# maxjaritz/mvpnet

Hardware: AMD Instinct MI355X
Metric: chunks/sec (8192 pts, 3x160x120 views) fwd+bwd (higher is better)
Workload: dtype f32; 1 GPU; configs[2]: MVPNet lifting (unproject + pixel k-NN + gather) + FeatureAggregation + PN2SSG full train step (fwd+loss+bwd+Adam), 2D CNN replaced by a resident 64-ch feature map; cfg=mvpnet_3d_unet_resnet34_pn2ssg.yaml, chunks_per_gpu=32, points=8192, views=3x160x120, feature_channels=64, k=3, parallelism=dp1 (one process per GPU, 1 grad all-reduce/step), launch=eager, cpu_affinity=32 logical cpus of 256 (0 .. 183)

## Files before the change

include/mvp_hip.h:

```cpp
#ifndef MVP_HIP_H_
#define MVP_HIP_H_

#include <stdint.h>

#ifdef __cplusplus
extern "C" {
#endif

typedef void* mvp_stream_t;

#define MVP_OK 0
#define MVP_EINVAL (-1)
#define MVP_EUNSUPPORTED (-2)
#define MVP_ENULL (-3)

const char* mvp_version(void);
const char* mvp_strerror(int code);

int mvp_set_fps_mode(int mode);

int mvp_fps_f32(const float* points, int64_t B, int64_t N, int64_t D, int64_t M, int64_t* index, mvp_stream_t stream);
int mvp_fps_f64(const double* points, int64_t B, int64_t N, int64_t D, int64_t M, int64_t* index, mvp_stream_t stream);
int mvp_fps_shape_f32(const float* points, int64_t B, int64_t N, int64_t D, int64_t M, int64_t* index, int shape, mvp_stream_t stream);
int mvp_fps_shape_f64(const double* points, int64_t B, int64_t N, int64_t D, int64_t M, int64_t* index, int shape, mvp_stream_t stream);
// ... 232 lines not shown
                                      const float* beta_i, const double* stat_i, float* dgamma_i, float* dbeta_i, int training, int mode,
                                      float drop_p, uint64_t drop_seed, const float* X, int64_t ldx, const float* act_mean,
                                      const float* act_invstd, const float* act_gamma, const float* act_beta, const float* W, int64_t ldw,
                                      int64_t R, int64_t C, int64_t Cp, float* dW, int64_t lddw, float* dZ, double* stat_prev, int* ticket,
                                      float* workspace, int64_t workspace_floats, int precision, int precision_backward, mvp_stream_t stream);
int mvp_mlp_layer_backward_wide_pooled_p_f32(const float* G, const float* Yi, const float* mean_i, const float* invstd_i, const float* gamma_i,
                                             const float* beta_i, const double* stat_i, float* dgamma_i, float* dbeta_i, int training, int mode,
                                             int64_t pool_k, float drop_p, uint64_t drop_seed, const float* X, int64_t ldx, const float* act_mean,
                                             const float* act_invstd, const float* act_gamma, const float* act_beta, const float* W, int64_t ldw,
                                             int64_t R, int64_t C, int64_t Cp, float* dW, int64_t lddw, float* dZ, double* stat_prev, int* ticket,
                                             float* workspace, int64_t workspace_floats, int precision, int precision_backward, mvp_stream_t stream);
int mvp_mlp_weight_grad_finish_p_f32(const float* dZ, const float* Y, const float* mean, const float* invstd, const float* gamma, const double* stat,
                                     int training, const float* X, int64_t R, int64_t Cout, int64_t Cin, int64_t ldx, float* dW, int64_t lddw,
                                     float* workspace, int64_t workspace_floats, int precision, int precision_backward, mvp_stream_t stream);
int mvp_mlp_weight_grad_finish_rel_p_f32(const float* dZ, const float* Y, const float* mean, const float* invstd, const float* gamma, const double* stat,
                                         int training, const float* X, int64_t R, int64_t Cout, int64_t Cin, int64_t ldx, const float* REL, float* dW,
                                         float* dWrel, int64_t lddw, int precision, int precision_backward, mvp_stream_t stream);
int mvp_mlp_weight_grad_finish_act_p_f32(const float* dZ, const float* Y, const float* mean, const float* invstd, const float* gamma, const double* stat,
                                         int training, const float* X, int64_t R, int64_t Cout, int64_t Cin, int64_t ldx, const float* act_mean,
                                         const float* act_invstd, const float* act_gamma, const float* act_beta, float* dW, int64_t lddw,
                                         float* workspace, int64_t workspace_floats, int precision, int precision_backward, mvp_stream_t stream);
int64_t mvp_mlp_input_grad_wide_workspace_bytes(int64_t C, int64_t Cp);
int mvp_mlp_input_grad_wide_p_f32(const float* G, const float* Yi, const float* mean_i, const float* invstd_i, const float* gamma_i,
                                  const double* stat_i, float* dgamma_i, float* dbeta_i, int training, const float* X, int64_t ldx,
                                  const float* act_mean, const float* act_invstd, const float* act_gamma, const float* act_beta, const float* W,
                                  int64_t ldw, int64_t R, int64_t C, int64_t Cp, float* dZ, double* stat_prev, void* workspace,
                                  int64_t workspace_bytes, int precision, int precision_backward, mvp_stream_t stream);
int mvp_mlp_weight_grad_f32(const float* dY, const float* X, int64_t R, int64_t Cout, int64_t Cin, int64_t ldx,
                            const float* act_mean, const float* act_invstd, const float* act_gamma, const float* act_beta,
                            float* dW, int64_t lddw, mvp_stream_t stream);
int64_t mvp_mlp_weight_grad_workspace_floats(void);
int mvp_mlp_weight_grad_ws_f32(const float* dY, const float* X, int64_t R, int64_t Cout, int64_t Cin, int64_t ldx,
                               const float* act_mean, const float* act_invstd, const float* act_gamma, const float* act_beta,
                               float* dW, int64_t lddw, float* workspace, int64_t workspace_floats, mvp_stream_t stream);

int mvp_sa_train_forward_f32(int stage, const float* zf, const float* xyz, const float* centre, const int64_t* index, const float* wxyz,
                             int64_t B, int64_t N, int64_t M, int64_t K, int64_t C1, const float* bn1_mean, const float* bn1_invstd,
                             const float* bn1_gamma, const float* bn1_beta, const float* W2, int64_t C2, const float* bn2_mean,
                             const float* bn2_invstd, const float* bn2_gamma, const float* bn2_beta, const float* W3, int64_t C3,
                             double* stat, float eps, float momentum, float* mean, float* invstd, float* running_mean,
                             float* running_var, int64_t* num_batches_tracked, float* ymax, float* ymin, uint8_t* amax, uint8_t* amin,
                             mvp_stream_t stream);
int mvp_sa_train_backward_f32(int layer, const float* zf, const float* xyz, const float* centre, const int64_t* index, const float* wxyz,
                              int64_t B, int64_t N, int64_t M, int64_t K, int64_t C1, const float* bn1_mean, const float* bn1_invstd,
                              const float* bn1_gamma, const float* bn1_beta, const float* W2, int64_t C2, const float* bn2_mean,
                              const float* bn2_invstd, const float* bn2_gamma, const float* bn2_beta, const float* W3, int64_t C3,
                              const float* mean_i, const float* invstd_i, const float* gamma_i, const double* stat_i, float* dgamma_i,
                              float* dbeta_i, int training, const float* G, const float* pool_dout, const float* pool_out,
                              const uint8_t* pool_arg, float* dW, int64_t lddw, float* dZ, double* stat_prev, float* tsum, mvp_stream_t stream);
int mvp_sa_train_backward1_f32(const float* dz1, const int32_t* offsets, const int32_t* slots, const float* zf, const float* dsum,
                               const float* wxyz, const float* tsum, const double* zsum, const double* gsum, int64_t B, int64_t N, int64_t M,
                               int64_t K, int64_t C1, const float* mean, const float* invstd, const float* gamma, const double* stat,
                               int training, float* dgamma, float* dbeta, float* gz, float* dWxyz, int64_t lddw, mvp_stream_t stream);
int mvp_sa_geom_sums_f32(const int32_t* offsets, const int32_t* slots, const float* xyz, const float* centre, int64_t B, int64_t N, int64_t M,
                         int64_t K, float* dsum, double* gsum, mvp_stream_t stream);
int mvp_sa_train_stats1_f32(const float* zf, const float* dsum, const float* wxyz, const double* gsum, int64_t B, int64_t N, int64_t M, int64_t K,
                            int64_t C1, double* stat, double* zsum, float eps, float momentum, float* mean, float* invstd, float* running_mean,
                            float* running_var, int64_t* num_batches_tracked, mvp_stream_t stream);
int mvp_sa_train_stats1_ws_f32(const float* zf, const float* dsum, const float* wxyz, const double* gsum, int64_t B, int64_t N, int64_t M, int64_t K,
                               int64_t C1, double* stat, double* zsum, float eps, float momentum, float* mean, float* invstd, float* running_mean,
                               float* running_var, int64_t* num_batches_tracked, double* scratch, int64_t scratch_doubles, mvp_stream_t stream);

int mvp_mlp_forward_p_f32(const float* X, int64_t R, int64_t Cin, int64_t ldx, const float* W, int64_t ldw, int64_t Cout, const
    float* act_mean, const float* act_invstd, const float* act_gamma, const float* act_beta, const float* bias, float* Y,
    double* stat, double* partial, int precision, int precision_backward, mvp_stream_t stream);
int mvp_mlp_forward_bn_p_f32(const float* X, int64_t R, int64_t Cin, int64_t ldx, const float* W, int64_t ldw, int64_t Cout,
    const float* act_mean, const float* act_invstd, const float* act_gamma, const float* act_beta, float* Y, double* stat,
    double* partial, float eps, float momentum, float* mean, float* invstd, float* running_mean, float* running_var, int64_t*
    num_batches_tracked, int precision, int precision_backward, mvp_stream_t stream);
int mvp_mlp_forward_rel_bn_p_f32(const float* X, int64_t R, int64_t Cin, int64_t ldx, const float* W, int64_t ldw, int64_t Cout,
    const float* rel, const float* wrel, float* Y, double* stat, double* partial, float eps, float momentum, float* mean, float*
    invstd, float* running_mean, float* running_var, int64_t* num_batches_tracked, int precision, int precision_backward,
    mvp_stream_t stream);
int mvp_mlp_forward_pool_p_f32(const float* X, int64_t R, int64_t Cin, int64_t ldx, const float* W, int64_t ldw, int64_t Cout,
    const float* act_mean, const float* act_invstd, const float* act_gamma, const float* act_beta, float* ymax, float* ymin,
    uint8_t* amax, uint8_t* amin, double* stat, double* partial, float eps, float momentum, float* mean, float* invstd, float*
    running_mean, float* running_var, int64_t* num_batches_tracked, int precision, int precision_backward, mvp_stream_t stream);
int mvp_mlp_input_grad_p_f32(const float* dY, int64_t R, int64_t Cout, const float* W, int64_t Cin, const float* y_prev, const
    float* mean, const float* invstd, const float* gamma, const float* beta, float* dZ, double* stat, double* partial, int
    precision, int precision_backward, mvp_stream_t stream);
int mvp_mlp_input_grad_dropout_p_f32(const float* dY, int64_t R, int64_t Cout, const float* W, int64_t Cin, const float* y_prev, const
    float* mean, const float* invstd, const float* gamma, const float* beta, float drop_p, uint64_t drop_seed, float* dZ, double* stat,
    double* partial, int precision, int precision_backward, mvp_stream_t stream);
int mvp_mlp_weight_grad_p_f32(const float* dY, const float* X, int64_t R, int64_t Cout, int64_t Cin, int64_t ldx, const float*
    act_mean, const float* act_invstd, const float* act_gamma, const float* act_beta, float* dW, int64_t lddw, int precision,
    int precision_backward, mvp_stream_t stream);
int mvp_mlp_weight_grad_ws_p_f32(const float* dY, const float* X, int64_t R, int64_t Cout, int64_t Cin, int64_t ldx, const
    float* act_mean, const float* act_invstd, const float* act_gamma, const float* act_beta, float* dW, int64_t lddw, float*
    workspace, int64_t workspace_floats, int precision, int precision_backward, mvp_stream_t stream);
int mvp_mlp_layer_backward_p_f32(const float* G, const float* Yi, const float* mean_i, const float* invstd_i, const float*
    gamma_i, const double* stat_i, float* dgamma_i, float* dbeta_i, int training, const float* X, int64_t ldx, const float*
    act_mean, const float* act_invstd, const float* act_gamma, const float* act_beta, const float* W, int64_t ldw, int64_t R,
    int64_t C, int64_t Cp, float* dW, int64_t lddw, float* dZ, double* stat_prev, double* partial, const float* pool_dout, const
    float* pool_out, const uint8_t* pool_arg, int precision, int precision_backward, mvp_stream_t stream);
int mvp_mlp_layer_backward_ws_p_f32(const float* G, const float* Yi, const float* mean_i, const float* invstd_i, const float*
    gamma_i, const double* stat_i, float* dgamma_i, float* dbeta_i, int training, const float* X, int64_t ldx, const float*
    act_mean, const float* act_invstd, const float* act_gamma, const float* act_beta, const float* W, int64_t ldw, int64_t R,
    int64_t C, int64_t Cp, float* dW, int64_t lddw, float* dZ, double* stat_prev, double* partial, const float* pool_dout, const
    float* pool_out, const uint8_t* pool_arg, float* workspace, int64_t workspace_floats, int precision, int precision_backward,
    mvp_stream_t stream);
int mvp_sa_fused_forward_p_f32(const float* zf, const float* xyz, const float* centre, const int64_t* index, const float* wxyz,
    int64_t B, int64_t N, int64_t M, int64_t K, int64_t C1, const float* bn1_mean, const float* bn1_invstd, const float*
    bn1_gamma, const float* bn1_beta, const float* W2, int64_t C2, const float* bn2_mean, const float* bn2_invstd, const float*
    bn2_gamma, const float* bn2_beta, const float* W3, int64_t C3, const float* bn3_mean, const float* bn3_invstd, const float*
    bn3_gamma, const float* bn3_beta, float* out, uint8_t* arg, int precision, int precision_backward, mvp_stream_t stream);

int mvp_sa_train_forward_p_f32(int stage, const float* zf, const float* xyz, const float* centre, const int64_t* index, const
    float* wxyz, int64_t B, int64_t N, int64_t M, int64_t K, int64_t C1, const float* bn1_mean, const float* bn1_invstd, const
    float* bn1_gamma, const float* bn1_beta, const float* W2, int64_t C2, const float* bn2_mean, const float* bn2_invstd, const
    float* bn2_gamma, const float* bn2_beta, const float* W3, int64_t C3, double* stat, float eps, float momentum, float* mean,
    float* invstd, float* running_mean, float* running_var, int64_t* num_batches_tracked, float* ymax, float* ymin, uint8_t*
    amax, uint8_t* amin, int precision, int precision_backward, mvp_stream_t stream);
int mvp_sa_train_backward_p_f32(int layer, const float* zf, const float* xyz, const float* centre, const int64_t* index, const
    float* wxyz, int64_t B, int64_t N, int64_t M, int64_t K, int64_t C1, const float* bn1_mean, const float* bn1_invstd, const
    float* bn1_gamma, const float* bn1_beta, const float* W2, int64_t C2, const float* bn2_mean, const float* bn2_invstd, const
    float* bn2_gamma, const float* bn2_beta, const float* W3, int64_t C3, const float* mean_i, const float* invstd_i, const
    float* gamma_i, const double* stat_i, float* dgamma_i, float* dbeta_i, int training, const float* G, const float* pool_dout,
    const float* pool_out, const uint8_t* pool_arg, float* dW, int64_t lddw, float* dZ, double* stat_prev, float* tsum, int precision, int
    precision_backward, mvp_stream_t stream);

int mvp_pn2_plan_f32(const float* xyz, int64_t B, int64_t N, int64_t levels, const int64_t* centroids, const float* radius,
                     const int64_t* neighbours, const int32_t* geom, int fps_shape, int flags, float knn_eps, void* const* buffers,
                     int64_t n_buffers, void* const* events, int* fps_status, mvp_stream_t stream);

int mvp_vote_accumulate_f32(const float* logit, int64_t ld_r, int64_t ld_c, const int64_t* chunk_ind, int64_t n,
                            int64_t C, float* sum, int32_t* count, mvp_stream_t stream);
int mvp_vote_gather_f32(const float* logit, int64_t ld_chunk, int64_t ld_r, int64_t ld_c, const int64_t* chunk_offsets, int64_t num_chunks,
                        const int32_t* point_offsets, const int32_t* point_slots, int64_t n_pts, int64_t C, float* sum, int32_t* count,
                        mvp_stream_t stream);
int mvp_vote_finish_f32(const float* sum, const int32_t* count, int64_t n_pts, int64_t C, float* mean, int64_t* label,
                        mvp_stream_t stream);

int mvp_seg_loss_f32(const float* logit, int64_t B, int64_t C, int64_t N, int64_t ld_b, int64_t ld_c, int64_t ld_n,
                     const int64_t* label, const float* weight, int64_t ignore_index, double* acc, float* loss, mvp_stream_t stream);
int mvp_seg_loss_backward_f32(const float* logit, int64_t B, int64_t C, int64_t N, int64_t ld_b, int64_t ld_c, int64_t ld_n,
                              const int64_t* label, const float* weight, int64_t ignore_index, const double* acc,
                              const float* grad_out, float* grad_logit, int64_t gld_b, int64_t gld_c, int64_t gld_n,
                              mvp_stream_t stream);
int mvp_seg_confusion_f32(const float* logit, int64_t B, int64_t C, int64_t N, int64_t ld_b, int64_t ld_c, int64_t ld_n,
                          const int64_t* label, int64_t ignore_index, int64_t* mat, mvp_stream_t stream);

#ifdef __cplusplus
}
#endif
#endif
```

mvpnet_amd/_lib.py:

```python
import ctypes
import os

import torch

_HERE = os.path.dirname(os.path.abspath(__file__))
LIB_PATH = os.environ.get('MVP_LIBRARY') or os.path.join(_HERE, 'libmvp_hip.so')
_lib = None
MLP_PRECISIONS = {'fp32': 0, 'bf16': 1, 'bf16x3': 3, 'bf16x6': 6}

_i64 = ctypes.c_int64
_ptr = ctypes.c_void_p
_f32 = ctypes.c_float

_SIGNATURES = {
    'mvp_fps_f32': [_ptr, _i64, _i64, _i64, _i64, _ptr, _ptr],
    'mvp_fps_f64': [_ptr, _i64, _i64, _i64, _i64, _ptr, _ptr],
    'mvp_fps_shape_f32': [_ptr, _i64, _i64, _i64, _i64, _ptr, ctypes.c_int, _ptr],
    'mvp_fps_shape_f64': [_ptr, _i64, _i64, _i64, _i64, _ptr, ctypes.c_int, _ptr],
    'mvp_fps_checked_f32': [_ptr, _i64, _i64, _i64, _i64, _ptr, ctypes.c_int, _ptr, _ptr],
    'mvp_fps_centroid_levels_f32': [_ptr, _ptr, _i64, _i64, _i64, _i64, _i64, _ptr, _ptr, _ptr],
    'mvp_ball_query_f32': [_ptr, _ptr, _i64, _i64, _i64, _f32, _i64, _ptr, _ptr],
    'mvp_ball_query_f64': [_ptr, _ptr, _i64, _i64, _i64, _f32, _i64, _ptr, _ptr],
    'mvp_ball_query_distance_f32': [_ptr, _ptr, _i64, _i64, _i64, _f32, _i64, _ptr, _ptr, _ptr],
    'mvp_ball_query_distance_f64': [_ptr, _ptr, _i64, _i64, _i64, _f32, _i64, _ptr, _ptr, _ptr],
# ... 25 lines not shown
    'mvp_interpolate_forward_bf16': [_ptr, _ptr, _ptr, _i64, _i64, _i64, _i64, _ptr, _ptr],
    'mvp_interpolate_backward_f32': [_ptr, _ptr, _ptr, _i64, _i64, _i64, _i64, _ptr, _ptr],
    'mvp_interpolate_backward_f64': [_ptr, _ptr, _ptr, _i64, _i64, _i64, _i64, _ptr, _ptr],
    'mvp_interpolate_backward_bf16': [_ptr, _ptr, _ptr, _i64, _i64, _i64, _i64, _ptr, _ptr],
    'mvp_unproject_f32': [_ptr, _ptr, _ptr, _ptr, _i64, _i64, _i64, _i64, _ptr, _ptr, _ptr],
    'mvp_unproject_u16': [_ptr, _ptr, _ptr, _ptr, _i64, _i64, _i64, _i64, _ptr, _ptr, _ptr],
    'mvp_pixel_knn_bruteforce_f32': [_ptr, _ptr, _ptr, _i64, _i64, _i64, _i64, _ptr, _ptr, _ptr],
    'mvp_pixel_knn_projective_f32': [_ptr, _ptr, _ptr, _ptr, _ptr, _i64, _i64, _i64, _i64, _i64, _i64, _ptr, _ptr, _ptr],
    'mvp_lift_gather_f32': [_ptr, _ptr, _ptr, _i64, _i64, _i64, _i64, _i64, _ptr, _ptr, _ptr],
    'mvp_lift_gather_backward_f32': [_ptr, _ptr, _i64, _i64, _i64, _i64, _i64, _ptr, _ptr],
    'mvp_lift_f32': [_ptr, ctypes.c_int, _ptr, _ptr, _ptr, _ptr, _ptr, _ptr, _i64, _i64, _i64, _i64, _i64, _i64, _i64, _ptr,
                     _ptr, _ptr, _ptr, _ptr, _ptr, _ptr],
    'mvp_lift_aug_f32': [_ptr, ctypes.c_int, _ptr, _ptr, _ptr, _ptr, _ptr, _ptr, _i64, _i64, _i64, _i64, _i64, _i64, _i64, _ptr,
                         _ptr, _ptr, _ptr, _ptr, _ptr, _ptr, _ptr, _ptr, _ptr],
    'mvp_rotate_rows_f32': [_ptr, _ptr, _i64, _i64, _ptr, _ptr],
    'mvp_copy_slices_f32': [_ptr, _i64, _ptr],
    'mvp_group_rows_f32': [_ptr, _ptr, _ptr, _ptr, _i64, _i64, _i64, _i64, _i64, _i64, _ptr, _ptr],
    'mvp_group_rows_backward_f32': [_ptr, _ptr, _i64, _i64, _i64, _i64, _i64, _i64, _ptr, _ptr],
    'mvp_group_lin_rows_f32': [_ptr, _ptr, _ptr, _ptr, _ptr, _i64, _i64, _i64, _i64, _i64, _ptr, _ptr, _ptr, _ptr, _ptr],
    'mvp_group_lin_rows_bn_f32': [_ptr, _ptr, _ptr, _ptr, _ptr, _i64, _i64, _i64, _i64, _i64, _ptr, _ptr, _ptr, _ptr, _f32, _f32, _ptr, _ptr, _ptr, _ptr, _ptr, _ptr],
    'mvp_colstats_f32': [_ptr, _i64, _i64, _ptr, _ptr, _ptr],
    'mvp_relation_rows_f32': [_ptr, _ptr, _ptr, _i64, _i64, _i64, _ptr, _ptr],
    'mvp_interp_rows_f32': [_ptr, _ptr, _ptr, _i64, _i64, _i64, _i64, _i64, _ptr, _ptr],
    'mvp_mlp_forward_bf16': [_ptr, _i64, _i64, _i64, _ptr, _i64, _i64, _ptr, _ptr, _ptr, ctypes.c_int, _ptr, _i64, _ptr],
    'mvp_adam_step_f32': [_ptr, _ptr, _ptr, _ptr, _ptr, _i64] + [ctypes.c_double] * 6 + [_ptr],
    'mvp_csr_build_i64': [_ptr, _i64, _i64, _i64, _ptr, _ptr, _ptr, _ptr],
    'mvp_csr_build_sorted_i64': [_ptr, _i64, _i64, _i64, _ptr, _ptr, _ptr, _ptr],
    'mvp_gather_rows_backward_csr_f32': [_ptr, _ptr, _ptr, _ptr, _i64, _i64, _i64, _i64, _i64, _i64, _ptr, _ptr],
    'mvp_gather_rows_backward_csr_finish_f32': [_ptr, _ptr, _ptr, _ptr, _ptr, _ptr, ctypes.c_int, _ptr, _ptr, _ptr, _i64, _i64, _i64, _i64, _i64, _i64, _ptr, _ptr],
    'mvp_interp_add_rows_f32': [_ptr, _ptr, _ptr, _ptr, _i64, _i64, _i64, _i64, _ptr, _ptr, _ptr, _ptr],
    'mvp_interp_add_rows_bn_f32': [_ptr, _ptr, _ptr, _ptr, _i64, _i64, _i64, _i64, _ptr, _ptr, _ptr, _f32, _f32, _ptr, _ptr, _ptr, _ptr, _ptr, _ptr],
    'mvp_interp_rows_backward_f32': [_ptr, _ptr, _ptr, _i64, _i64, _i64, _i64, _i64, _ptr, _ptr],
    'mvp_bn_rows_forward_f32': [_ptr, _ptr, _ptr, _i64, _i64, _i64, ctypes.c_int, _f32, _f32, ctypes.c_int, _ptr, _ptr, _ptr, _ptr,
                                _ptr, _ptr, _ptr, _ptr, _ptr],
    'mvp_bn_rows_backward_f32': [_ptr, _ptr, _ptr, _ptr, _ptr, _ptr, _ptr, _ptr, _i64, _i64, _i64, ctypes.c_int, ctypes.c_int, _ptr,
                                 _ptr, _ptr, _ptr, _ptr, _ptr],
    'mvp_bn_rows_forward_dropout_f32': [_ptr, _ptr, _ptr, _i64, _i64, ctypes.c_int, _f32, _f32, ctypes.c_int, _ptr, _ptr, _ptr, _ptr, _ptr, _ptr,
                                        _ptr, _f32, ctypes.c_uint64, _ptr],
    'mvp_bn_rows_backward_dropout_f32': [_ptr, _ptr, _ptr, _ptr, _ptr, _ptr, _i64, _i64, ctypes.c_int, ctypes.c_int, _ptr, _ptr, _ptr, _ptr,
                                         _ptr, _f32, ctypes.c_uint64, _ptr],
    'mvp_bn_rows_backward_finish_f32': [_ptr, _ptr, _ptr, _ptr, _ptr, _ptr, _i64, _i64, ctypes.c_int, _ptr, _ptr, _ptr, _ptr, _ptr],
    'mvp_bn_finalize_f32': [_ptr, _i64, _i64, _f32, _f32, _ptr, _ptr, _ptr, _ptr, _ptr, _ptr],
    'mvp_mlp_weight_grad_f32': [_ptr, _ptr, _i64, _i64, _i64, _i64, _ptr, _ptr, _ptr, _ptr, _ptr, _i64, _ptr],
    'mvp_mlp_weight_grad_ws_f32': [_ptr, _ptr, _i64, _i64, _i64, _i64, _ptr, _ptr, _ptr, _ptr, _ptr, _i64, _ptr, _i64, _ptr],
    'mvp_mlp_input_grad_f32': [_ptr, _i64, _i64, _ptr, _i64, _ptr, _ptr, _ptr, _ptr, _ptr, _ptr, _ptr, _ptr, _ptr],
    'mvp_mlp_input_grad_dropout_f32': [_ptr, _i64, _i64, _ptr, _i64, _ptr, _ptr, _ptr, _ptr, _ptr, _f32, ctypes.c_uint64, _ptr, _ptr, _ptr, _ptr],
    'mvp_mlp_layer_backward_f32': [_ptr, _ptr, _ptr, _ptr, _ptr, _ptr, _ptr, _ptr, ctypes.c_int, _ptr, _i64, _ptr, _ptr, _ptr, _ptr, _ptr, _i64,
                                   _i64, _i64, _i64, _ptr, _i64, _ptr, _ptr, _ptr, _ptr, _ptr, _ptr, _ptr],
    'mvp_mlp_layer_backward_ws_f32': [_ptr, _ptr, _ptr, _ptr, _ptr, _ptr, _ptr, _ptr, ctypes.c_int, _ptr, _i64, _ptr, _ptr, _ptr, _ptr, _ptr, _i64,
                                   _i64, _i64, _i64, _ptr, _i64, _ptr, _ptr, _ptr, _ptr, _ptr, _ptr, _ptr, _i64, _ptr],
    'mvp_mlp_forward_pool_f32': [_ptr, _i64, _i64, _i64, _ptr, _i64, _i64, _ptr, _ptr, _ptr, _ptr, _ptr, _ptr, _ptr, _ptr, _ptr, _ptr, _f32, _f32,
                                 _ptr, _ptr, _ptr, _ptr, _ptr, _ptr],
    'mvp_pool_finalize_f32': [_ptr, _ptr, _ptr, _ptr, _ptr, _ptr, _ptr, _ptr, _i64, _i64, ctypes.c_int, _ptr, _ptr, _ptr, _ptr],
    'mvp_pool_backward_stats_f32': [_ptr, _ptr, _ptr, _ptr, _ptr, _i64, _i64, ctypes.c_int, _ptr, _ptr, _ptr],
    'mvp_sa_fused_forward_f32': [_ptr, _ptr, _ptr, _ptr, _ptr, _i64, _i64, _i64, _i64, _i64, _ptr, _ptr, _ptr, _ptr, _ptr, _i64, _ptr, _ptr, _ptr,
                                 _ptr, _ptr, _i64, _ptr, _ptr, _ptr, _ptr, _ptr, _ptr, _ptr],
    'mvp_sa_train_forward_f32': [ctypes.c_int, _ptr, _ptr, _ptr, _ptr, _ptr, _i64, _i64, _i64, _i64, _i64, _ptr, _ptr, _ptr, _ptr, _ptr, _i64, _ptr, _ptr,
                                 _ptr, _ptr, _ptr, _i64, _ptr, _f32, _f32, _ptr, _ptr, _ptr, _ptr, _ptr, _ptr, _ptr, _ptr, _ptr, _ptr],
    'mvp_sa_train_backward_f32': [ctypes.c_int, _ptr, _ptr, _ptr, _ptr, _ptr, _i64, _i64, _i64, _i64, _i64, _ptr, _ptr, _ptr, _ptr, _ptr, _i64, _ptr, _ptr,
                                  _ptr, _ptr, _ptr, _i64, _ptr, _ptr, _ptr, _ptr, _ptr, _ptr, ctypes.c_int, _ptr, _ptr, _ptr, _ptr, _ptr, _i64, _ptr, _ptr,
                                  _ptr, _ptr],
    'mvp_sa_train_backward1_f32': [_ptr, _ptr, _ptr, _ptr, _ptr, _ptr, _ptr, _ptr, _ptr, _i64, _i64, _i64, _i64, _i64, _ptr, _ptr, _ptr, _ptr,
                                   ctypes.c_int, _ptr, _ptr, _ptr, _ptr, _i64, _ptr],
    'mvp_pn2_plan_f32': [_ptr, _i64, _i64, _i64, _ptr, _ptr, _ptr, _ptr, ctypes.c_int, ctypes.c_int, _f32, _ptr, _i64, _ptr, _ptr, _ptr],
    'mvp_sa_geom_sums_f32': [_ptr, _ptr, _ptr, _ptr, _i64, _i64, _i64, _i64, _ptr, _ptr, _ptr],
    'mvp_sa_train_stats1_f32': [_ptr, _ptr, _ptr, _ptr, _i64, _i64, _i64, _i64, _i64, _ptr, _ptr, _f32, _f32, _ptr, _ptr, _ptr, _ptr, _ptr, _ptr],
    'mvp_sa_train_stats1_ws_f32': [_ptr, _ptr, _ptr, _ptr, _i64, _i64, _i64, _i64, _i64, _ptr, _ptr, _f32, _f32, _ptr, _ptr, _ptr, _ptr, _ptr, _ptr, _i64, _ptr],
    'mvp_mlp_forward_bn_f32': [_ptr, _i64, _i64, _i64, _ptr, _i64, _i64, _ptr, _ptr, _ptr, _ptr, _ptr, _ptr, _ptr, _f32, _f32, _ptr, _ptr, _ptr,
                               _ptr, _ptr, _ptr],
    'mvp_mlp_forward_rel_bn_f32': [_ptr, _i64, _i64, _i64, _ptr, _i64, _i64, _ptr, _ptr, _ptr, _ptr, _ptr, _f32, _f32, _ptr, _ptr, _ptr, _ptr, _ptr, _ptr],
    'mvp_relation4_rows_f32': [_ptr, _ptr, _i64, _i64, _ptr, _ptr],
    'mvp_mlp_forward_f32': [_ptr, _i64, _i64, _i64, _ptr, _i64, _i64, _ptr, _ptr, _ptr, _ptr, _ptr, _ptr, _ptr, _ptr, _ptr],
    'mvp_vote_accumulate_f32': [_ptr, _i64, _i64, _ptr, _i64, _i64, _ptr, _ptr, _ptr],
    'mvp_vote_gather_f32': [_ptr, _i64, _i64, _i64, _ptr, _i64, _ptr, _ptr, _i64, _i64, _ptr, _ptr, _ptr],
    'mvp_vote_finish_f32': [_ptr, _ptr, _i64, _i64, _ptr, _ptr, _ptr],
    'mvp_seg_loss_f32': [_ptr, _i64, _i64, _i64, _i64, _i64, _i64, _ptr, _ptr, _i64, _ptr, _ptr, _ptr],
    'mvp_seg_loss_backward_f32': [_ptr, _i64, _i64, _i64, _i64, _i64, _i64, _ptr, _ptr, _i64, _ptr, _ptr, _ptr, _i64, _i64, _i64, _ptr],
    'mvp_seg_confusion_f32': [_ptr, _i64, _i64, _i64, _i64, _i64, _i64, _ptr, _i64, _ptr, _ptr],
}
for _n in ['mvp_mlp_forward_f32', 'mvp_mlp_forward_bn_f32', 'mvp_mlp_forward_rel_bn_f32', 'mvp_mlp_forward_pool_f32', 'mvp_mlp_input_grad_f32', 'mvp_mlp_input_grad_dropout_f32',
           'mvp_mlp_weight_grad_f32', 'mvp_mlp_weight_grad_ws_f32', 'mvp_mlp_layer_backward_f32', 'mvp_mlp_layer_backward_ws_f32',
           'mvp_sa_fused_forward_f32', 'mvp_sa_train_forward_f32', 'mvp_sa_train_backward_f32']:
    _SIGNATURES[_n[:-4] + '_p_f32'] = _SIGNATURES[_n][:-1] + [ctypes.c_int, ctypes.c_int, _ptr]
_SIGNATURES['mvp_mlp_layer_backward_wide_p_f32'] = [_ptr] * 9 + [ctypes.c_int, ctypes.c_int, _f32, ctypes.c_uint64, _ptr, _i64, _ptr, _ptr, _ptr, _ptr, _ptr, _i64,
                                                    _i64, _i64, _i64, _ptr, _i64, _ptr, _ptr, _ptr, _ptr, _i64, ctypes.c_int, ctypes.c_int, _ptr]
_SIGNATURES['mvp_mlp_layer_backward_wide_pooled_p_f32'] = [_ptr] * 9 + [ctypes.c_int, ctypes.c_int, _i64, _f32, ctypes.c_uint64, _ptr, _i64, _ptr, _ptr, _ptr, _ptr, _ptr, _i64,
                                                           _i64, _i64, _i64, _ptr, _i64, _ptr, _ptr, _ptr, _ptr, _i64, ctypes.c_int, ctypes.c_int, _ptr]
_SIGNATURES['mvp_mlp_weight_grad_finish_p_f32'] = [_ptr] * 6 + [ctypes.c_int, _ptr, _i64, _i64, _i64, _i64, _ptr, _i64, _ptr, _i64, ctypes.c_int, ctypes.c_int, _ptr]
_SIGNATURES['mvp_mlp_weight_grad_finish_rel_p_f32'] = [_ptr] * 6 + [ctypes.c_int, _ptr, _i64, _i64, _i64, _i64, _ptr, _ptr, _ptr, _i64, ctypes.c_int, ctypes.c_int, _ptr]
_SIGNATURES['mvp_mlp_weight_grad_finish_act_p_f32'] = [_ptr] * 6 + [ctypes.c_int, _ptr, _i64, _i64, _i64, _i64, _ptr, _ptr, _ptr, _ptr, _ptr, _i64, _ptr, _i64, ctypes.c_int,
                                                        ctypes.c_int, _ptr]
_SIGNATURES['mvp_mlp_input_grad_wide_p_f32'] = [_ptr] * 8 + [ctypes.c_int, _ptr, _i64, _ptr, _ptr, _ptr, _ptr, _ptr, _i64, _i64, _i64, _i64, _ptr, _ptr, _ptr, _i64,
                                                 ctypes.c_int, ctypes.c_int, _ptr]
EXPORTS = ['mvp_version', 'mvp_strerror', 'mvp_lift_workspace_bytes', 'mvp_ball_query_grid_workspace', 'mvp_knn3_grid_workspace', 'mvp_mlp_weight_grad_workspace_floats', 'mvp_mlp_input_grad_wide_workspace_bytes', 'mvp_group_lin_partial_count', 'mvp_colstats_partial_count',
           'mvp_set_mlp_precision', 'mvp_get_mlp_precision', 'mvp_mlp_layer_backward_partial_count', 'mvp_set_mlp_stream', 'mvp_set_mlp_precision_backward', 'mvp_get_mlp_precision_backward', 'mvp_mlp_precision_scope', 'mvp_set_fps_mode', 'mvp_fps_debug_spin_limit', 'mvp_fps_last_kernel'] + sorted(_SIGNATURES)


def lib():
    global _lib
    if _lib is None:
        if not os.path.exists(LIB_PATH):
            raise RuntimeError('libmvp_hip.so is not built: run `python -c "import __graft_entry__ as g; g.build()"` '
                               'or `make -C mvpnet_amd/csrc` ({})'.format(LIB_PATH))
        handle = ctypes.CDLL(LIB_PATH)
        handle.mvp_version.restype = ctypes.c_char_p
        handle.mvp_strerror.restype = ctypes.c_char_p
        handle.mvp_strerror.argtypes = [ctypes.c_int]
        handle.mvp_lift_workspace_bytes.restype = ctypes.c_int64
        handle.mvp_lift_workspace_bytes.argtypes = [_i64, _i64, _i64, _i64, _i64]
        handle.mvp_ball_query_grid_workspace.restype = ctypes.c_int64
        handle.mvp_ball_query_grid_workspace.argtypes = [_i64, _i64, _i64]
        handle.mvp_knn3_grid_workspace.restype = ctypes.c_int64
        handle.mvp_knn3_grid_workspace.argtypes = [_i64, _i64, _i64]
        handle.mvp_group_lin_partial_count.restype = ctypes.c_int64
        handle.mvp_group_lin_partial_count.argtypes = [_i64, _i64, _i64, _i64]
        handle.mvp_mlp_weight_grad_workspace_floats.restype = ctypes.c_int64
        handle.mvp_mlp_weight_grad_workspace_floats.argtypes = []
        handle.mvp_mlp_input_grad_wide_workspace_bytes.restype = ctypes.c_int64
        handle.mvp_mlp_input_grad_wide_workspace_bytes.argtypes = [ctypes.c_int64, ctypes.c_int64]
        handle.mvp_colstats_partial_count.restype = ctypes.c_int64
        handle.mvp_colstats_partial_count.argtypes = [_i64, _i64]
        handle.mvp_set_mlp_precision.restype = ctypes.c_int
        handle.mvp_set_mlp_precision.argtypes = [ctypes.c_int, ctypes.c_int]
        handle.mvp_get_mlp_precision.restype = ctypes.c_int
        handle.mvp_get_mlp_precision.argtypes = []
        handle.mvp_mlp_layer_backward_partial_count.restype = ctypes.c_int64
        handle.mvp_mlp_layer_backward_partial_count.argtypes = [_i64, _i64]
        for name, argtypes in _SIGNATURES.items():
            fn = getattr(handle, name)
            fn.argtypes = argtypes
            fn.restype = ctypes.c_int
        _lib = handle
        handle.mvp_set_mlp_stream.restype = ctypes.c_int
        handle.mvp_set_mlp_stream.argtypes = [ctypes.c_int]
        handle.mvp_set_fps_mode.restype = ctypes.c_int
        handle.mvp_set_fps_mode.argtypes = [ctypes.c_int]
        handle.mvp_fps_debug_spin_limit.restype = ctypes.c_int
        handle.mvp_fps_debug_spin_limit.argtypes = [ctypes.c_int]
        handle.mvp_fps_last_kernel.restype = ctypes.c_int
        handle.mvp_fps_last_kernel.argtypes = []
        if os.environ.get('MVP_MLP_STREAM') is not None:
            handle.mvp_set_mlp_stream(int(os.environ['MVP_MLP_STREAM']))
        handle.mvp_set_mlp_precision_backward.restype = ctypes.c_int
        handle.mvp_set_mlp_precision_backward.argtypes = [ctypes.c_int]
        handle.mvp_get_mlp_precision_backward.restype = ctypes.c_int
        handle.mvp_get_mlp_precision_backward.argtypes = []
        handle.mvp_mlp_precision_scope.restype = ctypes.c_int
        handle.mvp_mlp_precision_scope.argtypes = [ctypes.c_int, ctypes.c_int]
        if os.environ.get('MVP_MLP_PRECISION_BWD'):
            check(handle.mvp_set_mlp_precision_backward(MLP_PRECISIONS[os.environ['MVP_MLP_PRECISION_BWD']]), 'mvp_set_mlp_precision_backward')
        env = os.environ.get('MVP_MLP_PRECISION')
        if env:
            set_mlp_precision(env, int(os.environ.get('MVP_MLP_MIN_WIDTH', '0')))
    return _lib




def set_mlp_precision(name, min_width=0):
    if name not in MLP_PRECISIONS:
        raise ValueError('mlp precision must be one of {}'.format(sorted(MLP_PRECISIONS)))
    check(lib().mvp_set_mlp_precision(MLP_PRECISIONS[name], int(min_width)), 'mvp_set_mlp_precision')
    global _mlp_min_width
    _mlp_min_width = int(min_width)


_mlp_min_width = 0


def mlp_min_width():
    return _mlp_min_width


def set_mlp_precision_backward(name):
    if name not in ('bf16', 'bf16x3', 'bf16x6'):
        raise ValueError("backward mlp precision must be 'bf16', 'bf16x3' or 'bf16x6'")
    check(lib().mvp_set_mlp_precision_backward(MLP_PRECISIONS[name]), 'mvp_set_mlp_precision_backward')


class mlp_precision:

    def __init__(self, forward=None, backward=None):
        self.terms = -1 if forward is None else MLP_PRECISIONS[forward]
        self.bwd = -1 if backward is None else MLP_PRECISIONS[backward]
        if self.bwd == 0:
            raise ValueError("backward mlp precision must be 'bf16', 'bf16x3' or 'bf16x6'")

    def __enter__(self):
        old = lib().mvp_mlp_precision_scope(self.terms, self.bwd)
        if old < 0:
            check(old, 'mvp_mlp_precision_scope')
        self.old = (old // 16 - 1, old % 16 - 1)
        return self

    def __exit__(self, *exc):
        lib().mvp_mlp_precision_scope(*self.old)


def current_precision():
    h = lib()
    return (h.mvp_get_mlp_precision(), h.mvp_get_mlp_precision_backward())

# ... 30 lines not shown


def stream_of(t):
    return ctypes.c_void_p(torch.cuda.current_stream(t.device).cuda_stream)


def ptr(t):
    return None if t is None else t.data_ptr()


def ptr_at(t, element_offset):
    return t.data_ptr() + int(element_offset) * t.element_size()


def require_gpu(*tensors):
    for t in tensors:
        if t is None:
            continue
        if not t.is_cuda:
            raise RuntimeError('mvpnet_amd ops run on the GPU only (got a {} tensor); there is no CPU fallback'.format(t.device))
        if not t.is_contiguous():
            raise RuntimeError('tensor must be contiguous')


def suffix(t):
    if t.dtype == torch.float32:
        return 'f32'
    if t.dtype == torch.float64:
        return 'f64'
    raise RuntimeError('expected a float32 or float64 tensor, got {}'.format(t.dtype))


def value_suffix(t):
    return 'bf16' if t.dtype == torch.bfloat16 else suffix(t)


_FN = {}
_raw_stream = getattr(torch._C, '_cuda_getCurrentRawStream', None)
_raw_device = getattr(torch._C, '_cuda_getDevice', None)


def _fn(name):
    f = _FN.get(name)
    if f is None:
        f = _FN[name] = getattr(_lib if _lib is not None else lib(), name)
    return f


DW_WORKSPACE = os.environ.get('MVP_DETERMINISTIC', '0') == '1'


def set_deterministic(flag):
    global DW_WORKSPACE
    old, DW_WORKSPACE = DW_WORKSPACE, bool(flag)
    return old


_DW_WS = {}
_DW_WS_NAMES = {'mvp_mlp_weight_grad_f32': 'mvp_mlp_weight_grad_ws_f32', 'mvp_mlp_layer_backward_f32': 'mvp_mlp_layer_backward_ws_f32'}


def dw_workspace(index, stream_handle):
    ws = _DW_WS.get((index, stream_handle))
    if ws is None:
        ws = _DW_WS[(index, stream_handle)] = torch.empty(lib().mvp_mlp_weight_grad_workspace_floats(), dtype=torch.float32,
                                                          device=torch.device('cuda', index))
    return ws


def current_dw_workspace(device):
    if not DW_WORKSPACE:
        return None, 0
    index = device.index
    handle = _raw_stream(index) if (_raw_stream is not None and index == _raw_device()) else torch.cuda.current_stream(device).cuda_stream
    ws = dw_workspace(index, handle)
    return ws.data_ptr(), ws.numel()


def _with_dw_workspace(index, stream_handle, args):
    ws = dw_workspace(index, stream_handle)
    return args + (ws.data_ptr(), ws.numel())


def call_on(stream, name, *args, prec=None):
    if DW_WORKSPACE and name in _DW_WS_NAMES:
        name, args = _DW_WS_NAMES[name], _with_dw_workspace(stream.device.index, stream.cuda_stream, args)
    if prec is not None:
        name, args = name[:-4] + '_p_f32', args + prec
    code = _fn(name)(*args, stream.cuda_stream)
    if code != 0:
        check(code, name)


def call(name, tensor_for_device, *args, prec=None):
    index = tensor_for_device.device.index
    if DW_WORKSPACE and name in _DW_WS_NAMES:
        handle = _raw_stream(index) if _raw_stream is not None else torch.cuda.current_stream(tensor_for_device.device).cuda_stream
        name, args = _DW_WS_NAMES[name], _with_dw_workspace(index, handle, args)
    if prec is not None:
        name, args = name[:-4] + '_p_f32', args + prec
    if _raw_stream is not None and index == _raw_device():
        code = _fn(name)(*args, _raw_stream(index))
    elif index == torch.cuda.current_device():
        code = _fn(name)(*args, torch.cuda.current_stream(tensor_for_device.device).cuda_stream)
    else:
        with torch.cuda.device(tensor_for_device.device):
            code = _fn(name)(*args, stream_of(tensor_for_device))
    if code != 0:
        check(code, name)
```

mvpnet_amd/csrc/mlp.hip:

```cpp
#include "common.h"
#include "stats_reduce.h"
#include "mlp_common.h"
#include "dropout.h"
#include <algorithm>

int mvp_mlp_stream_forward(const float* X, int64_t R, int Cin, int ldx, const float* W, int ldw, int Cout, const float* act_mean,
                           const float* act_invstd, const float* act_gamma, const float* act_beta, const float* bias, float* Y,
                           double* stat, double* partial, int ns, float bn_eps, float bn_momentum, float* bn_mean, float* bn_invstd,
                           float* bn_running_mean, float* bn_running_var, int64_t* bn_num_batches, float* ymax, float* ymin,
                           uint8_t* amax, uint8_t* amin, hipStream_t s);

int g_mlp_terms = 6;
int g_mlp_terms_bwd = 3;
int g_mlp_min_width = 0;
thread_local int tl_mlp_terms = -1;
thread_local int tl_mlp_terms_bwd = -1;
int g_mlp_stream = 1;

namespace {


constexpr int kMT = 256;
constexpr int kBM = 128;


struct EpiBwd {
  const float* y;
  const float* mean;
  const float* invstd;
  const float* gamma;
  const float* beta;
  const float* rel;
  const float* wrel;
  Dropout drop;
};

#ifndef MVP_MFMA_PRIO
#define MVP_MFMA_PRIO 2
#endif
#ifndef MVP_DW_PRIO
#define MVP_DW_PRIO 2
#endif
constexpr int kMaxActCin = 512;

#ifndef MVP_MLP_WAVES128
#define MVP_MLP_WAVES128 3
#endif
template <int BN, int BK, bool WT, bool VEC, int ACT, int NS>
__global__ __launch_bounds__(kMT, (BN == 128 && VEC && WT && NS == 0) ? MVP_MLP_WAVES128 : (NS != 0 && BN == 128) ? 2 : 1) void mlp_fwd_kernel(const float* __restrict__ X, int64_t R, int Cin, int ldx,
                                                      const float* __restrict__ W, int ldw, int Cout,
                                                      InAct act, const float* __restrict__ bias, EpiBwd epi,
                                                      float* __restrict__ Y , double* __restrict__ stat,
                                                      double* __restrict__ partial) {
  static_assert(NS == 0 || (VEC && BK == 32), "split-bf16 needs the vector path and 32-wide slabs");
  constexpr int kLdB = BK + 4;
  constexpr int NT = BK / 8;
  constexpr int kColB = 80;
  constexpr int kPieceB = BN * kColB;
  constexpr int kBufB = NS == 0 ? BN * kLdB * 4 : NS * kPieceB;
  __shared__ __attribute__((aligned(16))) unsigned char BsRaw[2 * kBufB];
  float* const Bs0 = reinterpret_cast<float*>(BsRaw);
  __shared__ __attribute__((aligned(16))) float Ps[4][kMaxActCin];
  constexpr int kLdS = 36;
  constexpr int kSsFloats = 4 * 32 * kLdS;
  constexpr bool kAliasS = sizeof(float) * kSsFloats + sizeof(double) * 2 * 4 * BN <= (size_t)2 * kBufB;
  __shared__ __attribute__((aligned(16))) float Ss_own[kAliasS ? 4 : kSsFloats];
  float (*Ss)[32 * kLdS] = reinterpret_cast<float (*)[32 * kLdS]>(kAliasS ? Bs0 : &Ss_own[0]);
  static_assert(sizeof(double) * 2 * 4 * BN <= (size_t)2 * kBufB, "sred must fit in Bs");
  double (*sred)[4][BN] = reinterpret_cast<double (*)[4][BN]>(Bs0 + (kAliasS ? kSsFloats : 0));
  constexpr int NB = BN / 32;
  const int tid = threadIdx.x, lane = tid & 63, wave = tid >> 6;
  const int64_t row0 = (int64_t)blockIdx.x * kBM;
  const int col0 = blockIdx.y * BN;
  const int li = lane & 31, lh = lane >> 5;

  f32x16 acc[NB];
#pragma unroll
  for (int j = 0; j < NB; ++j)
#pragma unroll
    for (int i = 0; i < 16; ++i) acc[j][i] = 0.f;

  constexpr bool has_act = ACT != 0;
  constexpr bool act_lds = ACT == 1;
  if constexpr (act_lds) {
    for (int k = tid; k < min(kMaxActCin, (Cin + BK - 1) / BK * BK); k += kMT) {
      const int kc = min(k, Cin - 1);
      Ps[0][k] = act.mean[kc];
      Ps[1][k] = act.invstd[kc];
      Ps[2][k] = act.gamma[kc];
      Ps[3][k] = act.beta[kc];
    }
  }

  const int64_t arow = row0 + wave * 32 + li;
  const bool arow_ok = arow < R;
  const float* xrow = X + (size_t)(arow_ok ? arow : 0) * ldx;
  float4 an[NT];
  auto load_a = [&](int k0) {
#pragma unroll
    for (int t = 0; t < NT; ++t) {
      const int k = k0 + 8 * t + 4 * lh;
      if constexpr (VEC) {
        an[t] = *reinterpret_cast<const float4*>(xrow + min(k, Cin - 4));
      } else {
        an[t].x = xrow[min(k + 0, Cin - 1)];
        an[t].y = xrow[min(k + 1, Cin - 1)];
        an[t].z = xrow[min(k + 2, Cin - 1)];
        an[t].w = xrow[min(k + 3, Cin - 1)];
      }
    }
  };
  float ac[NT][4];
  auto activate = [&](int k0) {
#pragma unroll
    for (int t = 0; t < NT; ++t) {
      const int k = k0 + 8 * t + 4 * lh;
      float v[4] = {an[t].x, an[t].y, an[t].z, an[t].w};
      if constexpr (has_act) {
        float pm[4], pi[4], pg[4], pb[4];
        if constexpr (act_lds) {
          const float4 m4 = *reinterpret_cast<const float4*>(&Ps[0][k]), i4 = *reinterpret_cast<const float4*>(&Ps[1][k]);
          const float4 g4 = *reinterpret_cast<const float4*>(&Ps[2][k]), b4 = *reinterpret_cast<const float4*>(&Ps[3][k]);
          pm[0] = m4.x; pm[1] = m4.y; pm[2] = m4.z; pm[3] = m4.w;
          pi[0] = i4.x; pi[1] = i4.y; pi[2] = i4.z; pi[3] = i4.w;
          pg[0] = g4.x; pg[1] = g4.y; pg[2] = g4.z; pg[3] = g4.w;
          pb[0] = b4.x; pb[1] = b4.y; pb[2] = b4.z; pb[3] = b4.w;
        } else {
#pragma unroll
          for (int e = 0; e < 4; ++e) {
            const int kc = min(k + e, Cin - 1);
            pm[e] = act.mean[kc];
            pi[e] = act.invstd[kc];
            pg[e] = act.gamma[kc];
            pb[e] = act.beta[kc];
          }
        }
#pragma unroll
        for (int e = 0; e < 4; ++e) {
          const float a = ((v[e] - pm[e]) * pi[e]) * pg[e] + pb[e];
          v[e] = a > 0.f ? a : 0.f;
        }
      }
#pragma unroll
      for (int e = 0; e < 4; ++e) ac[t][e] = v[e];
    }
  };

  constexpr int LPC = BK / 4;
  constexpr int CPP = kMT / LPC;
  constexpr int NV = BN / CPP;
  constexpr int KH = BK / 32;
  float4 bn[WT ? NB * KH : NV];
  auto load_b = [&](int k0) {
    if constexpr (WT && NS != 0) {
      const int c = tid & 31, kq = (tid >> 5) * 4;
#pragma unroll
      for (int u = 0; u < NB; ++u) {
        const int co = min(col0 + u * 32 + c, Cout - 1);
        bn[u].x = W[(size_t)min(k0 + kq + 0, Cin - 1) * ldw + co];
        bn[u].y = W[(size_t)min(k0 + kq + 1, Cin - 1) * ldw + co];
        bn[u].z = W[(size_t)min(k0 + kq + 2, Cin - 1) * ldw + co];
        bn[u].w = W[(size_t)min(k0 + kq + 3, Cin - 1) * ldw + co];
      }
    } else if constexpr (!WT) {
      const int c = tid / LPC, k = k0 + (tid % LPC) * 4;
#pragma unroll
      for (int u = 0; u < NV; ++u) {
        const float* src = W + (size_t)min(col0 + u * CPP + c, Cout - 1) * ldw;
        if constexpr (VEC) {
          bn[u] = *reinterpret_cast<const float4*>(src + min(k, Cin - 4));
        } else {
          bn[u].x = src[min(k + 0, Cin - 1)];
          bn[u].y = src[min(k + 1, Cin - 1)];
          bn[u].z = src[min(k + 2, Cin - 1)];
          bn[u].w = src[min(k + 3, Cin - 1)];
        }
      }
    } else {
#pragma unroll
      for (int g = 0; g < KH; ++g) {
        const float* src = W + (size_t)min(k0 + 32 * g + (tid & 31), Cin - 1) * ldw;
#pragma unroll
        for (int p = 0; p < NB; ++p) {
          const int co = col0 + p * 32 + (tid >> 5) * 4;
          if constexpr (VEC) {
            bn[g * NB + p] = *reinterpret_cast<const float4*>(src + min(co, Cout - 4));
          } else {
            bn[g * NB + p].x = src[min(co + 0, Cout - 1)];
            bn[g * NB + p].y = src[min(co + 1, Cout - 1)];
            bn[g * NB + p].z = src[min(co + 2, Cout - 1)];
            bn[g * NB + p].w = src[min(co + 3, Cout - 1)];
          }
        }
      }
    }
  };
  auto store_b = [&](int buf, int k0) {
    if constexpr (NS != 0) {
      const int c = WT ? (tid & 31) : (tid / LPC), kq = WT ? (tid >> 5) * 4 : (tid % LPC) * 4;
      const int t = kq >> 3, unit = 2 * (t >> 1) + ((kq >> 2) & 1);
      unsigned char* base = BsRaw + (size_t)buf * kBufB + unit * 16 + (t & 1) * 8;
      const int k = k0 + kq;
      constexpr int PASSES = WT ? NB : NV;
#pragma unroll
      for (int u = 0; u < PASSES; ++u) {
        const int cl = u * 32 + c;
        const bool cok = col0 + cl < Cout;
        float4 v = bn[u];
        v.x = (cok && k + 0 < Cin) ? v.x : 0.f;
        v.y = (cok && k + 1 < Cin) ? v.y : 0.f;
        v.z = (cok && k + 2 < Cin) ? v.z : 0.f;
        v.w = (cok && k + 3 < Cin) ? v.w : 0.f;
        unsigned lo[NS], hi[NS];
        split_pair<NS>(v.x, v.y, lo);
        split_pair<NS>(v.z, v.w, hi);
#pragma unroll
        for (int pc = 0; pc < NS; ++pc)
          *reinterpret_cast<uint2*>(base + (size_t)pc * kPieceB + (size_t)cl * kColB) = make_uint2(lo[pc], hi[pc]);
      }
      return;
    }
    float* dst = Bs0 + (size_t)buf * (kBufB / 4);
    if constexpr (!WT) {
      const int c = tid / LPC, kq = (tid % LPC) * 4, k = k0 + kq;
#pragma unroll
      for (int u = 0; u < NV; ++u) {
        const bool cok = col0 + u * CPP + c < Cout;
        float4 v = bn[u];
        v.x = (cok && k + 0 < Cin) ? v.x : 0.f;
        v.y = (cok && k + 1 < Cin) ? v.y : 0.f;
        v.z = (cok && k + 2 < Cin) ? v.z : 0.f;
        v.w = (cok && k + 3 < Cin) ? v.w : 0.f;
        *reinterpret_cast<float4*>(dst + (u * CPP + c) * kLdB + kq) = v;
      }
    } else {
#pragma unroll
      for (int g = 0; g < KH; ++g) {
        const int kl = 32 * g + (tid & 31);
        const bool kok = k0 + kl < Cin;
#pragma unroll
        for (int p = 0; p < NB; ++p) {
          const int c = p * 32 + (tid >> 5) * 4;
          const int co = col0 + c;
          dst[(c + 0) * kLdB + kl] = (kok && co + 0 < Cout) ? bn[g * NB + p].x : 0.f;
          dst[(c + 1) * kLdB + kl] = (kok && co + 1 < Cout) ? bn[g * NB + p].y : 0.f;
          dst[(c + 2) * kLdB + kl] = (kok && co + 2 < Cout) ? bn[g * NB + p].z : 0.f;
          dst[(c + 3) * kLdB + kl] = (kok && co + 3 < Cout) ? bn[g * NB + p].w : 0.f;
        }
      }
    }
  };

  u32x4 af[NS == 0 ? 1 : 2][NS == 0 ? 1 : NS];
  auto split_a = [&]() {
    if constexpr (NS != 0) {
#pragma unroll
      for (int sI = 0; sI < 2; ++sI) {
        unsigned q0[NS], q1[NS], q2[NS], q3[NS];
        split_pair<NS>(ac[2 * sI][0], ac[2 * sI][1], q0);
        split_pair<NS>(ac[2 * sI][2], ac[2 * sI][3], q1);
        split_pair<NS>(ac[2 * sI + 1][0], ac[2 * sI + 1][1], q2);
        split_pair<NS>(ac[2 * sI + 1][2], ac[2 * sI + 1][3], q3);
#pragma unroll
        for (int pc = 0; pc < NS; ++pc) af[sI][pc] = u32x4{q0[pc], q1[pc], q2[pc], q3[pc]};
      }
    }
  };
  f32x16 acc1;
#pragma unroll
  for (int i = 0; i < 16; ++i) acc1[i] = 0.f;

  load_a(0);
  load_b(0);
  __syncthreads();
  store_b(0, 0);
  activate(0);
  split_a();
  __syncthreads();
  int buf = 0;
  for (int k0 = 0; k0 < Cin; k0 += BK) {
    const bool more = k0 + BK < Cin;
    if (more) {
      load_a(k0 + BK);
      load_b(k0 + BK);
    }
    __builtin_amdgcn_sched_barrier(0);
    __builtin_amdgcn_s_setprio(MVP_MFMA_PRIO);
    if constexpr (NS == 0) {
      const float* bp = Bs0 + (size_t)buf * (kBufB / 4) + li * kLdB + 4 * lh;
#pragma unroll
      for (int t = 0; t < NT; ++t) {
        float4 bf[NB];
#pragma unroll
        for (int j = 0; j < NB; ++j) bf[j] = *reinterpret_cast<const float4*>(bp + j * 32 * kLdB + 8 * t);
#pragma unroll
        for (int j = 0; j < NB; ++j) acc[j] = __builtin_amdgcn_mfma_f32_32x32x2f32(ac[t][0], bf[j].x, acc[j], 0, 0, 0);
#pragma unroll
        for (int j = 0; j < NB; ++j) acc[j] = __builtin_amdgcn_mfma_f32_32x32x2f32(ac[t][1], bf[j].y, acc[j], 0, 0, 0);
#pragma unroll
        for (int j = 0; j < NB; ++j) acc[j] = __builtin_amdgcn_mfma_f32_32x32x2f32(ac[t][2], bf[j].z, acc[j], 0, 0, 0);
#pragma unroll
        for (int j = 0; j < NB; ++j) acc[j] = __builtin_amdgcn_mfma_f32_32x32x2f32(ac[t][3], bf[j].w, acc[j], 0, 0, 0);
      }
    } else {
      using SP = SplitPairs<NS == 0 ? 2 : NS>;
      const unsigned char* bp = BsRaw + (size_t)buf * kBufB + (size_t)li * kColB + lh * 16;
      constexpr int JG = NB >= 2 ? 2 : 1;
#pragma unroll
      for (int sI = 0; sI < 2; ++sI) {
#pragma unroll
        for (int j0 = 0; j0 < NB; j0 += JG) {
          u32x4 bfr[JG][NS == 0 ? 1 : NS];
#pragma unroll
          for (int jj = 0; jj < JG; ++jj)
#pragma unroll
            for (int pc = 0; pc < NS; ++pc)
              bfr[jj][pc] = *reinterpret_cast<const u32x4*>(bp + (size_t)pc * kPieceB + (size_t)(j0 + jj) * 32 * kColB + sI * 32);
#pragma unroll
          for (int q = 0; q < SP::N; ++q)
#pragma unroll
            for (int jj = 0; jj < JG; ++jj) {
              const bf16x8 a8 = __builtin_bit_cast(bf16x8, af[sI][SP::A[q]]);
              const bf16x8 b8 = __builtin_bit_cast(bf16x8, bfr[jj][SP::B[q]]);
              if (NB == 1 && sI == 1)
                acc1 = __builtin_amdgcn_mfma_f32_32x32x16_bf16(a8, b8, acc1, 0, 0, 0);
              else
                acc[j0 + jj] = __builtin_amdgcn_mfma_f32_32x32x16_bf16(a8, b8, acc[j0 + jj], 0, 0, 0);
            }
        }
      }
    }
    __builtin_amdgcn_s_setprio(0);
    __builtin_amdgcn_sched_barrier(0);
    if (more) {
      store_b(buf ^ 1, k0 + BK);
      activate(k0 + BK);
      split_a();
    }
    __syncthreads();
    buf ^= 1;
  }
  if constexpr (NS != 0 && NB == 1) {
#pragma unroll
    for (int i = 0; i < 16; ++i) acc[0][i] += acc1[i];
  }

  const int cl = lane & 31, rh = (lane >> 5) * 4;
  const bool has_rel = VEC && !WT && epi.rel != nullptr;
  if constexpr (VEC && !WT) {
    if (has_rel) {
      if (lane < 32) {
        const int64_t r = row0 + wave * 32 + lane;
        f32x4 v = {0.f, 0.f, 0.f, 0.f};
        if (r < R) v = *reinterpret_cast<const f32x4*>(epi.rel + (size_t)r * 4);
        *reinterpret_cast<f32x4*>(Ss[wave] + lane * kLdS + 32) = v;
      }
      __builtin_amdgcn_wave_barrier();
    }
  }
  f32x4 ypv[VEC ? NB : 1][4];
  if constexpr (VEC) {
    if (epi.y) {
#pragma unroll
      for (int j = 0; j < NB; ++j)
#pragma unroll
        for (int pp = 0; pp < 4; ++pp) {
          const int row = pp * 8 + (lane >> 3), c4 = (lane & 7) * 4;
// ... 20 lines not shown
    if (has_rel && co < Cout) wr = *reinterpret_cast<const f32x4*>(epi.wrel + (size_t)co * 4);
    float yst[16];
    if constexpr (VEC) {
      if (epi.y) {
        float* st = Ss[wave];
#pragma unroll
        for (int pp = 0; pp < 4; ++pp) {
          const int row = pp * 8 + (lane >> 3), c4 = (lane & 7) * 4;
          *reinterpret_cast<f32x4*>(st + row * kLdS + c4) = ypv[j][pp];
        }
        __builtin_amdgcn_wave_barrier();
      }
    }
#pragma unroll
    for (int i = 0; i < 16; ++i) {
      const int m = wave * 32 + (i & 3) + 8 * (i >> 2) + rh;
      const int64_t r = row0 + m;
      yst[i] = 0.f;
      if (r < R && co < Cout) {
        float y = acc[j][i] + bv;
        if constexpr (VEC && !WT) {
          if (has_rel) {
            const f32x4 rv = *reinterpret_cast<const f32x4*>(Ss[wave] + ((i & 3) + 8 * (i >> 2) + rh) * kLdS + 32);
            y += (rv[0] * wr[0] + rv[1] * wr[1]) + (rv[2] * wr[2] + rv[3] * wr[3]);
          }
        }
        if (epi.y) {
          const float yp = VEC ? Ss[wave][((i & 3) + 8 * (i >> 2) + rh) * kLdS + cl] : epi.y[(size_t)r * Cout + co];
          const float xh = (yp - em) * ei;
          if (epi.drop.thresh) y *= epi.drop.factor((unsigned)((size_t)r * Cout + co));
          y = (xh * eg + eb > 0.f) ? y : 0.f;
          s += y;
          q += y * xh;
        } else {
          s += y;
          q += y * y;
        }
        if constexpr (!VEC) __builtin_nontemporal_store(y, Y + (size_t)r * Cout + co);
        yst[i] = y;
      }
    }
    if constexpr (VEC) {
      if (epi.y) __builtin_amdgcn_wave_barrier();
      float* st = Ss[wave];
#pragma unroll
      for (int i = 0; i < 16; ++i) st[((i & 3) + 8 * (i >> 2) + rh) * kLdS + cl] = yst[i];
      __builtin_amdgcn_wave_barrier();
#pragma unroll
      for (int pp = 0; pp < 4; ++pp) {
        const int row = pp * 8 + (lane >> 3), c4 = (lane & 7) * 4;
        const f32x4 v = *reinterpret_cast<const f32x4*>(st + row * kLdS + c4);
        const int64_t r = row0 + wave * 32 + row;
        const int cc = col0 + j * 32 + c4;
        if (r < R && cc < Cout)
          __builtin_nontemporal_store(v, reinterpret_cast<f32x4*>(Y + (size_t)r * Cout + cc));
      }
      __builtin_amdgcn_wave_barrier();
    }
    if (stat) {
      s += __shfl_xor(s, 32, kWave);
      q += __shfl_xor(q, 32, kWave);
      if (lane < 32) {
        sred[0][wave][j * 32 + cl] = (double)s;
        sred[1][wave][j * 32 + cl] = (double)q;
      }
    }
  }
  if (stat) {
    __syncthreads();
    for (int c = tid; c < BN; c += kMT) {
      const int co = col0 + c;
      if (co < Cout) {
        const double s0 = sred[0][0][c] + sred[0][1][c] + sred[0][2][c] + sred[0][3][c];
        const double s1 = sred[1][0][c] + sred[1][1][c] + sred[1][2][c] + sred[1][3][c];
        if (partial) {
          partial[((size_t)blockIdx.x * 2 + 0) * Cout + co] = s0;
          partial[((size_t)blockIdx.x * 2 + 1) * Cout + co] = s1;
        } else {
          atomicAdd(stat + co, s0);
          atomicAdd(stat + Cout + co, s1);
        }
      }
    }
  }
}

template <int TM, int TN, bool VEC, bool FIN = false>
__global__ __launch_bounds__(kMT) void mlp_dw_kernel(const float* __restrict__ dY, const float* __restrict__ X, int64_t R,
                                                     int Cout, int Cin, int ldx, InAct act, int64_t rows_per_block,
                                                     float* __restrict__ dW, int lddw, float* __restrict__ ws, DyFinish fin = DyFinish{}) {
  static_assert(!FIN || VEC, "the finish on load takes whole quadruples");
  constexpr int NBLK = (TM / 32) * (TN / 32);
  constexpr int RS = 4 / NBLK;
  constexpr int BR = 32 * RS;
  __shared__ __attribute__((aligned(16))) float Ds[2][BR * TM];
  __shared__ __attribute__((aligned(16))) float As[2][BR * TN];
  const int tid = threadIdx.x, lane = tid & 63, wave = tid >> 6;
  const int co0 = blockIdx.x * TM, ci0 = blockIdx.y * TN;
  const int64_t r_begin = (int64_t)blockIdx.z * rows_per_block;
  const int64_t r_end = min(R, r_begin + rows_per_block);
  const int blk = wave % NBLK, rs = wave / NBLK;
  const int wco = (blk / (TN / 32)) * 32, wci = (blk % (TN / 32)) * 32;
  f32x16 acc;
#pragma unroll
  for (int i = 0; i < 16; ++i) acc[i] = 0.f;

  constexpr int LD = TM / 4, RD = kMT / LD, PD = BR / RD;
  constexpr int LA = TN / 4, RA = kMT / LA, PA = BR / RA;
  const int dq = (tid % LD) * 4, dr = tid / LD;
  const int aq = (tid % LA) * 4, ar = tid / LA;
  float pm[4], pi[4], pg[4], pb[4];
  const bool has_act = act.mean != nullptr;
  if (has_act) {
#pragma unroll
    for (int i = 0; i < 4; ++i) {
      const int k = min(ci0 + aq + i, Cin - 1);
      pm[i] = act.mean[k];
      pi[i] = act.invstd[k];
      pg[i] = act.gamma[k];
      pb[i] = act.beta[k];
    }
  }
  float4 dn[PD], an[PA];
  float4 yn[FIN ? PD : 1];
  float fmu[4], fis[4], fsc[4], fdb[4], fdg[4];
  if constexpr (FIN) {
#pragma unroll
    for (int i = 0; i < 4; ++i) {
      const int k = min(co0 + dq, Cout - 4) + i;
      fmu[i] = fin.mean[k];
      fis[i] = fin.invstd[k];
      fsc[i] = fin.gamma[k] * fis[i];
      fdb[i] = (float)fin.stat[k] * fin.inv_rows;
      fdg[i] = (float)fin.stat[Cout + k] * fin.inv_rows;
    }
  }
  auto load = [&](int64_t r0) {
#pragma unroll
    for (int p = 0; p < PD; ++p) {
      const float* src = dY + (size_t)min(r0 + dr + p * RD, R - 1) * Cout;
      const int c = co0 + dq;
      if constexpr (FIN) yn[p] = *reinterpret_cast<const float4*>(fin.Y + (size_t)min(r0 + dr + p * RD, R - 1) * Cout + min(c, Cout - 4));
      if constexpr (VEC) {
        dn[p] = *reinterpret_cast<const float4*>(src + min(c, Cout - 4));
      } else {
        dn[p].x = src[min(c + 0, Cout - 1)];
        dn[p].y = src[min(c + 1, Cout - 1)];
        dn[p].z = src[min(c + 2, Cout - 1)];
        dn[p].w = src[min(c + 3, Cout - 1)];
      }
    }
#pragma unroll
    for (int p = 0; p < PA; ++p) {
      const float* src = X + (size_t)min(r0 + ar + p * RA, R - 1) * ldx;
      const int c = ci0 + aq;
      if constexpr (VEC) {
        an[p] = *reinterpret_cast<const float4*>(src + min(c, Cin - 4));
      } else {
        an[p].x = src[min(c + 0, Cin - 1)];
        an[p].y = src[min(c + 1, Cin - 1)];
        an[p].z = src[min(c + 2, Cin - 1)];
        an[p].w = src[min(c + 3, Cin - 1)];
      }
    }
  };
  auto store = [&](int buf, int64_t r0) {
// ... 243 lines not shown
                                                           accr[a], 0, 0, 0);
    }
    __builtin_amdgcn_s_setprio(0);
    __builtin_amdgcn_sched_barrier(0);
  }
  constexpr int NBLK = TMB * TNB;
  auto publish = [&](int slot) {
#pragma unroll
    for (int a = 0; a < TMB; ++a)
#pragma unroll
      for (int b = 0; b < TNB; ++b)
#pragma unroll
        for (int i = 0; i < 16; ++i) red[slot][((a * TNB + b) * 16 + i) * 64 + lane] = acc[a][b][i];
    if constexpr (REL) {
#pragma unroll
      for (int a = 0; a < TMB; ++a)
#pragma unroll
        for (int i = 0; i < 16; ++i) red[slot][((TMB * TNB + a) * 16 + i) * 64 + lane] = accr[a][i];
    }
  };
  auto absorb = [&](int slot) {
#pragma unroll
    for (int a = 0; a < TMB; ++a)
#pragma unroll
      for (int b = 0; b < TNB; ++b)
#pragma unroll
        for (int i = 0; i < 16; ++i) acc[a][b][i] += red[slot][((a * TNB + b) * 16 + i) * 64 + lane];
    if constexpr (REL) {
#pragma unroll
      for (int a = 0; a < TMB; ++a)
#pragma unroll
        for (int i = 0; i < 16; ++i) accr[a][i] += red[slot][((TMB * TNB + a) * 16 + i) * 64 + lane];
    }
  };
  static_assert(NBLK <= 4, "tile");
  static_assert(!REL || sizeof(red) <= 64 * 1024, "LDS");
  if (wave >= 2) publish(wave - 2);
  __syncthreads();
  if (wave < 2) absorb(wave);
  __syncthreads();
  if (wave == 1) publish(0);
  __syncthreads();
  if (wave == 0) {
    absorb(0);
    if (ws) {
      float* t = ws + (((size_t)blockIdx.z * gridDim.x + blockIdx.x) * gridDim.y + blockIdx.y) * (size_t)(NBLK * 1024);
#pragma unroll
      for (int a = 0; a < TMB; ++a)
#pragma unroll
        for (int b = 0; b < TNB; ++b)
#pragma unroll
          for (int i = 0; i < 16; ++i) __builtin_nontemporal_store(acc[a][b][i], t + ((a * TNB + b) * 16 + i) * 64 + lane);
      return;
    }
#pragma unroll
    for (int a = 0; a < TMB; ++a)
#pragma unroll
      for (int b = 0; b < TNB; ++b) {
        const int ci = ci0 + 32 * b + c;
#pragma unroll
        for (int i = 0; i < 16; ++i) {
          const int co = co0 + 32 * a + (i & 3) + 8 * (i >> 2) + 4 * g;
#ifdef MVP_EXP_DW_STORE
          if (co < Cout && ci < Cin) *(dW + (size_t)co * lddw + ci) = acc[a][b][i];
#else
          if (co < Cout && ci < Cin) atomicAdd(dW + (size_t)co * lddw + ci, acc[a][b][i]);
#endif
        }
      }
    if constexpr (REL) {
#pragma unroll
      for (int a = 0; a < TMB; ++a)
#pragma unroll
        for (int i = 0; i < 16; ++i) {
          const int co = co0 + 32 * a + (i & 3) + 8 * (i >> 2) + 4 * g;
          if (co < Cout && c < 4) atomicAdd(dW2 + (size_t)co * lddw + c, accr[a][i]);
        }
    }
  }
}

template <bool WT>
void launch_mlp(const float* X, int64_t R, int K, int ldx, const float* W, int ldw, int N, InAct act, const float* bias, EpiBwd epi,
                float* Y, double* stat, double* partial, hipStream_t s) {
  const unsigned gx = (unsigned)cdiv(R, kBM);
  const bool vec = ldx % 4 == 0 && ldw % 4 == 0 && K % 4 == 0 && N % 4 == 0 && ((uintptr_t)X) % 16 == 0 && ((uintptr_t)W) % 16 == 0 &&
                   K >= 4 && N >= 4;
#define MVP_MLP_LAUNCH(BN, VEC, NS_)                                                                                              \
                                  \
  do {                                                                                                                             \
    if (WT || act.mean == nullptr)                                                                                                 \
      hipLaunchKernelGGL((mlp_fwd_kernel<BN, 32, WT, VEC, 0, NS_>), dim3(gx, (unsigned)cdiv(N, BN)), dim3(kMT), 0, s, X, R, K, ldx, W, ldw, N, \
                         act, bias, epi, Y, stat, partial);                                                                        \
    else if (K <= kMaxActCin)                                                                                                      \
      hipLaunchKernelGGL((mlp_fwd_kernel<BN, 32, WT, VEC, WT ? 0 : 1, NS_>), dim3(gx, (unsigned)cdiv(N, BN)), dim3(kMT), 0, s, X, R, K, ldx, W, \
                         ldw, N, act, bias, epi, Y, stat, partial);                                                                \
    else                                                                                                                           \
      hipLaunchKernelGGL((mlp_fwd_kernel<BN, 32, WT, VEC, WT ? 0 : 2, NS_>), dim3(gx, (unsigned)cdiv(N, BN)), dim3(kMT), 0, s, X, R, K, ldx, W, \
                         ldw, N, act, bias, epi, Y, stat, partial);                                                                \
  } while (0)
  int bn = N <= 32 ? 32 : N <= 64 ? 64 : 128;
  while (bn > 32 && (int64_t)gx * cdiv(N, bn) < 256) bn >>= 1;
  const int fwd_pieces = mlp_fwd_pieces();
  const int ns = (vec && std::max(K, N) >= g_mlp_min_width) ? (WT ? mlp_bwd_pieces() : fwd_pieces) : 0;
#define MVP_MLP_BY_NS(BN)                                                                                                          \
  do {                                                                                                                             \
    if (!vec) MVP_MLP_LAUNCH(BN, false, 0);                                                                                        \
    else if (ns == 1) MVP_MLP_LAUNCH(BN, true, 1);                                                                                 \
    else if (ns == 2) MVP_MLP_LAUNCH(BN, true, 2);                                                                                 \
    else if (ns == 3) MVP_MLP_LAUNCH(BN, true, 3);                                                                                 \
    else MVP_MLP_LAUNCH(BN, true, 0);                                                                                              \
  } while (0)
  if (bn == 32) MVP_MLP_BY_NS(32);
  else if (bn == 64) MVP_MLP_BY_NS(64);
  else MVP_MLP_BY_NS(128);
#undef MVP_MLP_BY_NS
#undef MVP_MLP_LAUNCH
}

}

namespace {
int mlp_forward_impl(const float* X, int64_t R, int64_t Cin, int64_t ldx, const float* W, int64_t ldw, int64_t Cout, const float* act_mean,
                     const float* act_invstd, const float* act_gamma, const float* act_beta, const float* bias, float* Y, double* stat,
                     double* partial, float bn_eps, float bn_momentum, float* bn_mean, float* bn_invstd, float* bn_running_mean,
                     float* bn_running_var, int64_t* bn_num_batches, hipStream_t s, const float* rel = nullptr, const float* wrel = nullptr) {
  InAct act{act_mean, act_invstd, act_gamma, act_beta};
  const unsigned gx = (unsigned)cdiv(R, kBM);
  const BnFinalize fin{R, bn_eps, bn_momentum, bn_mean, bn_invstd, bn_running_mean, bn_running_var, bn_num_batches};
  if (g_mlp_stream && !rel && std::max(Cin, Cout) >= g_mlp_min_width) {
    const int rc = mvp_mlp_stream_forward(X, R, (int)Cin, (int)ldx, W, (int)ldw, (int)Cout, act_mean, act_invstd, act_gamma, act_beta, bias, Y,
                                          stat, partial, mlp_fwd_pieces(), bn_eps, bn_momentum, bn_mean,
                                          bn_invstd, bn_running_mean, bn_running_var, bn_num_batches, nullptr, nullptr, nullptr, nullptr, s);
    if (rc != MVP_EUNSUPPORTED) return rc;
  }
  launch_mlp<false>(X, R, (int)Cin, (int)ldx, W, (int)ldw, (int)Cout, act, bias, EpiBwd{nullptr, nullptr, nullptr, nullptr, nullptr, rel, wrel}, Y, stat,
                    stat ? partial : nullptr, s);
  if (stat && bn_mean)
    launch_stats_reduce_finalize(partial, partial ? (int64_t)gx : 0, (int)(2 * Cout), stat, fin, s);
  else if (stat && partial)
    launch_stats_reduce(partial, (int64_t)gx, (int)(2 * Cout), stat, s);
  return mvp_launch_status();
}
}

MVP_API int mvp_mlp_forward_f32(const float* X, int64_t R, int64_t Cin, int64_t ldx, const float* W, int64_t ldw,
                                int64_t Cout, const float* act_mean, const float* act_invstd, const float* act_gamma,
                                const float* act_beta, const float* bias, float* Y, double* stat, double* partial,
                                mvp_stream_t stream) {
  MVP_NONNULL(X);
  MVP_NONNULL(W);
  MVP_NONNULL(Y);
  MVP_REQUIRE(R >= 0 && Cin > 0 && Cout > 0 && ldx >= Cin && ldw >= Cin && Cin < (1 << 20) && Cout < (1 << 20));
  if (act_mean) {
    MVP_NONNULL(act_invstd);
    MVP_NONNULL(act_gamma);
    MVP_NONNULL(act_beta);
  }
  if (R == 0) return MVP_OK;
  return mlp_forward_impl(X, R, Cin, ldx, W, ldw, Cout, act_mean, act_invstd, act_gamma, act_beta, bias, Y, stat, partial, 0.f, 0.f, nullptr,
                          nullptr, nullptr, nullptr, nullptr, static_cast<hipStream_t>(stream));
}

MVP_API int mvp_mlp_forward_bn_f32(const float* X, int64_t R, int64_t Cin, int64_t ldx, const float* W, int64_t ldw, int64_t Cout,
                                   const float* act_mean, const float* act_invstd, const float* act_gamma, const float* act_beta, float* Y,
                                   double* stat, double* partial, float eps, float momentum, float* mean, float* invstd,
                                   float* running_mean, float* running_var, int64_t* num_batches_tracked, mvp_stream_t stream) {
  MVP_NONNULL(X);
  MVP_NONNULL(W);
  MVP_NONNULL(Y);
  MVP_NONNULL(stat);
  MVP_NONNULL(mean);
  MVP_NONNULL(invstd);
  MVP_REQUIRE(R > 0 && Cin > 0 && Cout > 0 && ldx >= Cin && ldw >= Cin && Cin < (1 << 20) && Cout < (1 << 20));
  if (act_mean) {
    MVP_NONNULL(act_invstd);
    MVP_NONNULL(act_gamma);
    MVP_NONNULL(act_beta);
  }
  if (running_mean) MVP_NONNULL(running_var);
  return mlp_forward_impl(X, R, Cin, ldx, W, ldw, Cout, act_mean, act_invstd, act_gamma, act_beta, nullptr, Y, stat, partial, eps, momentum,
                          mean, invstd, running_mean, running_var, num_batches_tracked, static_cast<hipStream_t>(stream));
}

MVP_API int mvp_mlp_forward_rel_bn_f32(const float* X, int64_t R, int64_t Cin, int64_t ldx, const float* W, int64_t ldw, int64_t Cout,
                                       const float* rel, const float* wrel, float* Y, double* stat, double* partial, float eps, float momentum,
                                       float* mean, float* invstd, float* running_mean, float* running_var, int64_t* num_batches_tracked,
                                       mvp_stream_t stream) {
  MVP_NONNULL(X);
  MVP_NONNULL(W);
  MVP_NONNULL(Y);
  MVP_NONNULL(rel);
  MVP_NONNULL(wrel);
  MVP_REQUIRE(R > 0 && Cin >= 4 && Cout >= 4 && ldx >= Cin && ldw >= Cin && Cin < (1 << 20) && Cout < (1 << 20));
  MVP_REQUIRE(ldx % 4 == 0 && ldw % 4 == 0 && Cin % 4 == 0 && Cout % 4 == 0 && ((uintptr_t)X) % 16 == 0 && ((uintptr_t)W) % 16 == 0 &&
              ((uintptr_t)rel) % 16 == 0 && ((uintptr_t)wrel) % 16 == 0);
  if (mean) {
    MVP_NONNULL(stat);
    MVP_NONNULL(invstd);
  }
  if (running_mean) MVP_NONNULL(running_var);
  return mlp_forward_impl(X, R, Cin, ldx, W, ldw, Cout, nullptr, nullptr, nullptr, nullptr, nullptr, Y, stat, partial, eps, momentum, mean, invstd,
                          running_mean, running_var, num_batches_tracked, static_cast<hipStream_t>(stream), rel, wrel);
}

MVP_API int mvp_mlp_forward_pool_f32(const float* X, int64_t R, int64_t Cin, int64_t ldx, const float* W, int64_t ldw, int64_t Cout,
                                     const float* act_mean, const float* act_invstd, const float* act_gamma, const float* act_beta,
                                     float* ymax, float* ymin, uint8_t* amax, uint8_t* amin, double* stat, double* partial, float eps,
                                     float momentum, float* mean, float* invstd, float* running_mean, float* running_var,
                                     int64_t* num_batches_tracked, mvp_stream_t stream) {
  MVP_NONNULL(X);
  MVP_NONNULL(W);
  MVP_NONNULL(ymax);
  MVP_NONNULL(ymin);
  MVP_NONNULL(amax);
  MVP_NONNULL(amin);
  MVP_NONNULL(stat);
  MVP_NONNULL(partial);
  MVP_NONNULL(mean);
  MVP_NONNULL(invstd);
// ... 158 lines not shown
                                                 const float* REL, float* dW, float* dWrel, int64_t lddw, int precision, int precision_backward,
                                                 mvp_stream_t stream) {
  MVP_NONNULL(dZ);
  MVP_NONNULL(Y);
  MVP_NONNULL(mean);
  MVP_NONNULL(invstd);
  MVP_NONNULL(gamma);
  MVP_NONNULL(stat);
  MVP_NONNULL(X);
  MVP_NONNULL(REL);
  MVP_NONNULL(dW);
  MVP_NONNULL(dWrel);
  MVP_REQUIRE(R >= 0 && Cin > 0 && Cout > 0 && ldx >= Cin && lddw >= Cin && lddw >= 4 && lddw < (1 << 24) && Cout < (1 << 20));
  MVP_REQUIRE((precision == -1 || precision == 0 || precision == 1 || precision == 3 || precision == 6) &&
              (precision_backward == -1 || precision_backward == 1 || precision_backward == 3 || precision_backward == 6));
  const int terms = precision >= 0 ? precision : mlp_terms();
  const int bwd = precision_backward >= 0 ? precision_backward : mlp_terms_bwd();
  const int ns = terms == 0 ? 0 : (bwd == 6 ? 3 : bwd == 1 ? 1 : 2);
  if ((ns != 1 && ns != 2) || Cout <= 32 || Cin <= 32 || Cin > 64 || std::max(Cin, Cout) < g_mlp_min_width) return MVP_EUNSUPPORTED;
  if (R == 0) return MVP_OK;
  hipStream_t s = static_cast<hipStream_t>(stream);
  static const int64_t wg_target = []() { const char* e = getenv("MVP_DW_WORKGROUPS"); return e ? (int64_t)atoi(e) : (int64_t)1024; }();
  const int64_t tiles = cdiv(Cout, 64);
  int64_t splits = std::min<int64_t>(cdiv(wg_target, tiles), 512);
  int64_t rows_per_block = cdiv(cdiv(R, splits), 64) * 64;
  if (rows_per_block < 256) rows_per_block = 256;
  splits = cdiv(R, rows_per_block);
  const DyFinish fin{Y, mean, invstd, gamma, stat, training ? 1.0f / (float)R : 0.f};
  const InAct act{nullptr, nullptr, nullptr, nullptr};
  dim3 grid((unsigned)tiles, 1, (unsigned)splits);
  if (ns == 1)
    hipLaunchKernelGGL((mlp_dw_bf_kernel<2, 2, 1, true, true>), grid, dim3(kMT), 0, s, dZ, X, R, (int)Cout, (int)Cin, (int)ldx, act, rows_per_block, dW,
                       (int)lddw, nullptr, fin, REL, dWrel);
  else
    hipLaunchKernelGGL((mlp_dw_bf_kernel<2, 2, 2, true, true>), grid, dim3(kMT), 0, s, dZ, X, R, (int)Cout, (int)Cin, (int)ldx, act, rows_per_block, dW,
                       (int)lddw, nullptr, fin, REL, dWrel);
  return mvp_launch_status();
}

MVP_API int mvp_mlp_weight_grad_finish_act_p_f32(const float* dZ, const float* Y, const float* mean, const float* invstd, const float* gamma,
                                                 const double* stat, int training, const float* X, int64_t R, int64_t Cout, int64_t Cin, int64_t ldx,
                                                 const float* act_mean, const float* act_invstd, const float* act_gamma, const float* act_beta,
                                                 float* dW, int64_t lddw, float* workspace, int64_t workspace_floats, int precision,
                                                 int precision_backward, mvp_stream_t stream) {
  MVP_NONNULL(Y);
  MVP_NONNULL(mean);
  MVP_NONNULL(invstd);
  MVP_NONNULL(gamma);
  MVP_NONNULL(stat);
  MVP_REQUIRE((precision == -1 || precision == 0 || precision == 1 || precision == 3 || precision == 6) &&
              (precision_backward == -1 || precision_backward == 1 || precision_backward == 3 || precision_backward == 6));
  if (Cout % 4 != 0 || Cout <= 32 || ((uintptr_t)dZ | (uintptr_t)Y) % 16 != 0 || (act_mean && Cin <= 32)) return MVP_EUNSUPPORTED;
  const int old_terms = tl_mlp_terms, old_bwd = tl_mlp_terms_bwd;
  if (precision >= 0) tl_mlp_terms = precision;
  if (precision_backward >= 0) tl_mlp_terms_bwd = precision_backward;
  const DyFinish fin{Y, mean, invstd, gamma, stat, (training && R > 0) ? 1.0f / (float)R : 0.f};
  const int rc = weight_grad_impl(dZ, X, R, Cout, Cin, ldx, act_mean, act_invstd, act_gamma, act_beta, dW, lddw, workspace, workspace_floats, stream, &fin);
  tl_mlp_terms = old_terms;
  tl_mlp_terms_bwd = old_bwd;
  return rc;
}

namespace {
int input_grad_impl(const float* dY, int64_t R, int64_t Cout, const float* W, int64_t Cin, const float* y_prev, const float* mean, const float* invstd,
                    const float* gamma, const float* beta, float drop_p, uint64_t drop_seed, float* dZ, double* stat, double* partial, mvp_stream_t stream) {
  MVP_NONNULL(dY);
  MVP_NONNULL(W);
  MVP_NONNULL(dZ);
  MVP_REQUIRE(R >= 0 && Cin > 0 && Cout > 0 && Cin < (1 << 20) && Cout < (1 << 20));
  if (y_prev) {
    MVP_NONNULL(mean);
    MVP_NONNULL(invstd);
    MVP_NONNULL(gamma);
    MVP_NONNULL(beta);
    MVP_NONNULL(stat);
  }
  hipStream_t s = static_cast<hipStream_t>(stream);
  if (R == 0) return MVP_OK;
  InAct act{nullptr, nullptr, nullptr, nullptr};
  EpiBwd epi{y_prev, mean, invstd, gamma, beta};
  if (make_dropout(y_prev ? drop_p : 0.f, drop_seed, R, Cin, 1, &epi.drop) != MVP_OK) return MVP_EINVAL;
  double* st = y_prev ? stat : nullptr;
  const unsigned gx = (unsigned)cdiv(R, kBM);
  launch_mlp<true>(dY, R, (int)Cout, (int)Cout, W, (int)Cin, (int)Cin, act, nullptr, epi, dZ, st, st ? partial : nullptr, s);
  if (st && partial)
    launch_stats_reduce(partial, (int64_t)gx, (int)(2 * Cin), stat, s);
  return mvp_launch_status();
}
}

MVP_API int mvp_mlp_input_grad_f32(const float* dY, int64_t R, int64_t Cout, const float* W, int64_t Cin,
                                   const float* y_prev, const float* mean, const float* invstd, const float* gamma,
                                   const float* beta, float* dZ, double* stat, double* partial, mvp_stream_t stream) {
  return input_grad_impl(dY, R, Cout, W, Cin, y_prev, mean, invstd, gamma, beta, 0.f, 0, dZ, stat, partial, stream);
}

MVP_API int mvp_mlp_input_grad_dropout_f32(const float* dY, int64_t R, int64_t Cout, const float* W, int64_t Cin, const float* y_prev, const float* mean,
                                           const float* invstd, const float* gamma, const float* beta, float drop_p, uint64_t drop_seed, float* dZ,
                                           double* stat, double* partial, mvp_stream_t stream) {
  MVP_NONNULL(y_prev);
  return input_grad_impl(dY, R, Cout, W, Cin, y_prev, mean, invstd, gamma, beta, drop_p, drop_seed, dZ, stat, partial, stream);
}

MVP_API int mvp_set_mlp_precision(int terms, int min_width) {
  MVP_REQUIRE(terms == 0 || terms == 1 || terms == 3 || terms == 6);
  MVP_REQUIRE(min_width >= 0);
  g_mlp_terms = terms;
  g_mlp_min_width = min_width;
  return MVP_OK;
}
MVP_API int mvp_get_mlp_precision(void) { return mlp_terms(); }
MVP_API int mvp_set_mlp_precision_backward(int terms) {
  MVP_REQUIRE(terms == 1 || terms == 3 || terms == 6);
  g_mlp_terms_bwd = terms;
  return MVP_OK;
}
MVP_API int mvp_get_mlp_precision_backward(void) { return mlp_terms_bwd(); }
MVP_API int mvp_mlp_precision_scope(int terms, int terms_backward) {
  if (!(terms == -1 || terms == 0 || terms == 1 || terms == 3 || terms == 6) ||
      !(terms_backward == -1 || terms_backward == 1 || terms_backward == 3 || terms_backward == 6))
    return MVP_EINVAL;
  const int old = (tl_mlp_terms + 1) * 16 + (tl_mlp_terms_bwd + 1);
  tl_mlp_terms = terms;
  tl_mlp_terms_bwd = terms_backward;
  return old;
}
MVP_API int mvp_set_mlp_stream(int on) {
  const int old = g_mlp_stream;
  g_mlp_stream = on ? 1 : 0;
  return old;
}
```

mvpnet_amd/csrc/mlp_common.h:

```cpp
#pragma once
#include "common.h"

extern int g_mlp_terms;
extern int g_mlp_terms_bwd;
extern int g_mlp_min_width;

extern thread_local int tl_mlp_terms;
extern thread_local int tl_mlp_terms_bwd;
static inline int mlp_terms() { return tl_mlp_terms >= 0 ? tl_mlp_terms : g_mlp_terms; }
static inline int mlp_terms_bwd() { return tl_mlp_terms_bwd >= 0 ? tl_mlp_terms_bwd : g_mlp_terms_bwd; }
static inline int mlp_fwd_pieces() { return mlp_terms() == 1 ? 1 : mlp_terms() == 3 ? 2 : mlp_terms() == 6 ? 3 : 0; }
static inline int mlp_bwd_pieces() { return mlp_terms() == 0 ? 0 : (mlp_terms_bwd() == 6 ? 3 : mlp_terms_bwd() == 1 ? 1 : 2); }

int mlp_dw_wide_launch(const float* G, const float* Yi, const float* mean_i, const float* invstd_i, const float* gamma_i, const double* stat_i,
                       float inv_rows, const float* X, int64_t ldx, const float* act_mean, const float* act_invstd, const float* act_gamma,
                       const float* act_beta, int64_t R, int64_t C, int64_t Cp, float* dW, int64_t lddw, int ns, hipStream_t s);

namespace {

struct InAct {
  const float* mean;
  const float* invstd;
  const float* gamma;
  const float* beta;
};

struct DyFinish {
  const float* Y;
  const float* mean;
  const float* invstd;
  const float* gamma;
  const double* stat;
  float inv_rows;
};

typedef float f32x16 __attribute__((ext_vector_type(16)));
typedef float f32x4 __attribute__((ext_vector_type(4)));
typedef __bf16 bf16x8 __attribute__((ext_vector_type(8)));
typedef __bf16 bf16x2 __attribute__((ext_vector_type(2)));
typedef unsigned u32x4 __attribute__((ext_vector_type(4)));

__device__ __forceinline__ unsigned pack_bf16(float x, float y) {
  bf16x2 p = {(__bf16)x, (__bf16)y};
  return __builtin_bit_cast(unsigned, p);
}
template <int NS>
__device__ __forceinline__ void split_pair(float x, float y, unsigned (&pc)[NS]) {
  pc[0] = pack_bf16(x, y);
  if constexpr (NS == 1) return;
  float rx = x - __uint_as_float(pc[0] << 16), ry = y - __uint_as_float(pc[0] & 0xffff0000u);
  pc[1] = pack_bf16(rx, ry);
  if constexpr (NS == 3) {
    rx -= __uint_as_float(pc[1] << 16);
    ry -= __uint_as_float(pc[1] & 0xffff0000u);
    pc[2] = pack_bf16(rx, ry);
  }
}
template <int NS> struct SplitPairs;
template <> struct SplitPairs<1> { static constexpr int N = 1; static constexpr int A[1] = {0}; static constexpr int B[1] = {0}; };
template <> struct SplitPairs<2> { static constexpr int N = 3; static constexpr int A[3] = {1, 0, 0}; static constexpr int B[3] = {0, 1, 0}; };
template <> struct SplitPairs<3> { static constexpr int N = 6; static constexpr int A[6] = {2, 0, 1, 1, 0, 0}; static constexpr int B[6] = {0, 2, 1, 0, 1, 0}; };


template <int TMB, int TNB>
__global__ __launch_bounds__(256) void dw_reduce_kernel(const float* __restrict__ ws, int splits, int tiles_x, int tiles_y, int Cout, int Cin,
                                                        float* __restrict__ dW, int lddw) {
  constexpr int NBLK = TMB * TNB;
  __shared__ float part[4][64];
  const int lane = threadIdx.x & 63, wave = threadIdx.x >> 6;
  const int e = blockIdx.x;
  const int i = e & 15, ab = (e >> 4) % NBLK, tile = (e >> 4) / NBLK;
  const int a = ab / TNB, b = ab % TNB;
  const int tx = tile / tiles_y, ty = tile % tiles_y;
  const size_t stride = (size_t)tiles_x * tiles_y * NBLK * 1024;
  const float* p = ws + (size_t)tile * (NBLK * 1024) + (size_t)(ab * 16 + i) * 64 + lane;
  float v0 = 0.f, v1 = 0.f, v2 = 0.f, v3 = 0.f;
  int sI = wave;
  for (; sI + 12 < splits; sI += 16) {
    v0 += p[(size_t)sI * stride];
    v1 += p[(size_t)(sI + 4) * stride];
    v2 += p[(size_t)(sI + 8) * stride];
    v3 += p[(size_t)(sI + 12) * stride];
  }
  for (; sI < splits; sI += 4) v0 += p[(size_t)sI * stride];
  part[wave][lane] = (v0 + v1) + (v2 + v3);
  __syncthreads();
  if (wave == 0) {
    const float sum = (part[0][lane] + part[1][lane]) + (part[2][lane] + part[3][lane]);
    const int co = tx * (32 * TMB) + 32 * a + (i & 3) + 8 * (i >> 2) + 4 * (lane >> 5);
    const int ci = ty * (32 * TNB) + 32 * b + (lane & 31);
    if (co < Cout && ci < Cin) dW[(size_t)co * lddw + ci] += sum;
// ... 6 lines not shown
```

mvpnet_amd/csrc/mlp_prec.hip:

```cpp
#include "mlp_common.h"

namespace {
struct PrecisionArg {
  int old_terms, old_bwd;
  bool ok;
  PrecisionArg(int terms, int bwd) : old_terms(tl_mlp_terms), old_bwd(tl_mlp_terms_bwd) {
    ok = (terms == -1 || terms == 0 || terms == 1 || terms == 3 || terms == 6) && (bwd == -1 || bwd == 1 || bwd == 3 || bwd == 6);
    if (ok && terms >= 0) tl_mlp_terms = terms;
    if (ok && bwd >= 0) tl_mlp_terms_bwd = bwd;
  }
  ~PrecisionArg() {
    tl_mlp_terms = old_terms;
    tl_mlp_terms_bwd = old_bwd;
  }
};
}

#define MVP_WITH_PRECISION(call)             \
  PrecisionArg scope(precision, precision_backward); \
  if (!scope.ok) return MVP_EINVAL;          \
  return call

MVP_API int mvp_mlp_forward_p_f32(const float* X, int64_t R, int64_t Cin, int64_t ldx, const float* W, int64_t ldw, int64_t Cout,
                                  const float* act_mean, const float* act_invstd, const float* act_gamma, const float* act_beta,
                                  const float* bias, float* Y, double* stat, double* partial, int precision, int precision_backward,
                                  mvp_stream_t stream) {
  MVP_WITH_PRECISION(mvp_mlp_forward_f32(X, R, Cin, ldx, W, ldw, Cout, act_mean, act_invstd, act_gamma, act_beta, bias, Y, stat, partial, stream));
}
MVP_API int mvp_mlp_forward_bn_p_f32(const float* X, int64_t R, int64_t Cin, int64_t ldx, const float* W, int64_t ldw, int64_t Cout,
                                     const float* act_mean, const float* act_invstd, const float* act_gamma, const float* act_beta, float* Y,
                                     double* stat, double* partial, float eps, float momentum, float* mean, float* invstd,
                                     float* running_mean, float* running_var, int64_t* num_batches_tracked, int precision,
                                     int precision_backward, mvp_stream_t stream) {
  MVP_WITH_PRECISION(mvp_mlp_forward_bn_f32(X, R, Cin, ldx, W, ldw, Cout, act_mean, act_invstd, act_gamma, act_beta, Y, stat, partial, eps, momentum,
                                            mean, invstd, running_mean, running_var, num_batches_tracked, stream));
}
MVP_API int mvp_mlp_forward_rel_bn_p_f32(const float* X, int64_t R, int64_t Cin, int64_t ldx, const float* W, int64_t ldw, int64_t Cout,
                                         const float* rel, const float* wrel, float* Y, double* stat, double* partial, float eps, float momentum,
                                         float* mean, float* invstd, float* running_mean, float* running_var, int64_t* num_batches_tracked,
                                         int precision, int precision_backward, mvp_stream_t stream) {
  MVP_WITH_PRECISION(mvp_mlp_forward_rel_bn_f32(X, R, Cin, ldx, W, ldw, Cout, rel, wrel, Y, stat, partial, eps, momentum, mean, invstd, running_mean,
                                                running_var, num_batches_tracked, stream));
}
MVP_API int mvp_mlp_forward_pool_p_f32(const float* X, int64_t R, int64_t Cin, int64_t ldx, const float* W, int64_t ldw, int64_t Cout,
                                       const float* act_mean, const float* act_invstd, const float* act_gamma, const float* act_beta,
                                       float* ymax, float* ymin, uint8_t* amax, uint8_t* amin, double* stat, double* partial, float eps,
                                       float momentum, float* mean, float* invstd, float* running_mean, float* running_var,
                                       int64_t* num_batches_tracked, int precision, int precision_backward, mvp_stream_t stream) {
  MVP_WITH_PRECISION(mvp_mlp_forward_pool_f32(X, R, Cin, ldx, W, ldw, Cout, act_mean, act_invstd, act_gamma, act_beta, ymax, ymin, amax, amin, stat,
                                              partial, eps, momentum, mean, invstd, running_mean, running_var, num_batches_tracked, stream));
}
MVP_API int mvp_mlp_input_grad_p_f32(const float* dY, int64_t R, int64_t Cout, const float* W, int64_t Cin, const float* y_prev,
                                     const float* mean, const float* invstd, const float* gamma, const float* beta, float* dZ, double* stat,
                                     double* partial, int precision, int precision_backward, mvp_stream_t stream) {
  MVP_WITH_PRECISION(mvp_mlp_input_grad_f32(dY, R, Cout, W, Cin, y_prev, mean, invstd, gamma, beta, dZ, stat, partial, stream));
}
MVP_API int mvp_mlp_input_grad_dropout_p_f32(const float* dY, int64_t R, int64_t Cout, const float* W, int64_t Cin, const float* y_prev,
                                             const float* mean, const float* invstd, const float* gamma, const float* beta, float drop_p,
                                             uint64_t drop_seed, float* dZ, double* stat, double* partial, int precision, int precision_backward,
                                             mvp_stream_t stream) {
  MVP_WITH_PRECISION(mvp_mlp_input_grad_dropout_f32(dY, R, Cout, W, Cin, y_prev, mean, invstd, gamma, beta, drop_p, drop_seed, dZ, stat, partial, stream));
}
MVP_API int mvp_mlp_weight_grad_p_f32(const float* dY, const float* X, int64_t R, int64_t Cout, int64_t Cin, int64_t ldx,
                                      const float* act_mean, const float* act_invstd, const float* act_gamma, const float* act_beta,
                                      float* dW, int64_t lddw, int precision, int precision_backward, mvp_stream_t stream) {
  MVP_WITH_PRECISION(mvp_mlp_weight_grad_f32(dY, X, R, Cout, Cin, ldx, act_mean, act_invstd, act_gamma, act_beta, dW, lddw, stream));
}
MVP_API int mvp_mlp_weight_grad_ws_p_f32(const float* dY, const float* X, int64_t R, int64_t Cout, int64_t Cin, int64_t ldx,
                                         const float* act_mean, const float* act_invstd, const float* act_gamma, const float* act_beta,
                                         float* dW, int64_t lddw, float* workspace, int64_t workspace_floats, int precision,
                                         int precision_backward, mvp_stream_t stream) {
  MVP_WITH_PRECISION(mvp_mlp_weight_grad_ws_f32(dY, X, R, Cout, Cin, ldx, act_mean, act_invstd, act_gamma, act_beta, dW, lddw, workspace,
                                                workspace_floats, stream));
}
MVP_API int mvp_mlp_layer_backward_p_f32(const float* G, const float* Yi, const float* mean_i, const float* invstd_i, const float* gamma_i,
                                         const double* stat_i, float* dgamma_i, float* dbeta_i, int training, const float* X, int64_t ldx,
                                         const float* act_mean, const float* act_invstd, const float* act_gamma, const float* act_beta,
                                         const float* W, int64_t ldw, int64_t R, int64_t C, int64_t Cp, float* dW, int64_t lddw, float* dZ,
                                         double* stat_prev, double* partial, const float* pool_dout, const float* pool_out,
                                         const uint8_t* pool_arg, int precision, int precision_backward, mvp_stream_t stream) {
  MVP_WITH_PRECISION(mvp_mlp_layer_backward_f32(G, Yi, mean_i, invstd_i, gamma_i, stat_i, dgamma_i, dbeta_i, training, X, ldx, act_mean, act_invstd,
                                                act_gamma, act_beta, W, ldw, R, C, Cp, dW, lddw, dZ, stat_prev, partial, pool_dout,
                                                    pool_out, pool_arg,
                                                stream));
}
MVP_API int mvp_mlp_layer_backward_ws_p_f32(const float* G, const float* Yi, const float* mean_i, const float* invstd_i, const float* gamma_i,
                                            const double* stat_i, float* dgamma_i, float* dbeta_i, int training, const float* X, int64_t ldx,
                                            const float* act_mean, const float* act_invstd, const float* act_gamma, const float* act_beta,
                                            const float* W, int64_t ldw, int64_t R, int64_t C, int64_t Cp, float* dW, int64_t lddw, float* dZ,
                                            double* stat_prev, double* partial, const float* pool_dout, const float* pool_out,
                                            const uint8_t* pool_arg, float* workspace, int64_t workspace_floats, int precision,
                                            int precision_backward, mvp_stream_t stream) {
  MVP_WITH_PRECISION(mvp_mlp_layer_backward_ws_f32(G, Yi, mean_i, invstd_i, gamma_i, stat_i, dgamma_i, dbeta_i, training, X, ldx, act_mean,
      act_invstd,
                                                   act_gamma, act_beta, W, ldw, R, C, Cp, dW, lddw, dZ, stat_prev, partial, pool_dout, pool_out,
                                                   pool_arg, workspace, workspace_floats, stream));
}
MVP_API int mvp_sa_fused_forward_p_f32(const float* zf, const float* xyz, const float* centre, const int64_t* index, const float* wxyz,
                                       int64_t B, int64_t N, int64_t M, int64_t K, int64_t C1, const float* bn1_mean, const float* bn1_invstd,
                                       const float* bn1_gamma, const float* bn1_beta, const float* W2, int64_t C2, const float* bn2_mean,
                                       const float* bn2_invstd, const float* bn2_gamma, const float* bn2_beta, const float* W3, int64_t C3,
                                       const float* bn3_mean, const float* bn3_invstd, const float* bn3_gamma, const float* bn3_beta,
                                       float* out, uint8_t* arg, int precision, int precision_backward, mvp_stream_t stream) {
  MVP_WITH_PRECISION(mvp_sa_fused_forward_f32(zf, xyz, centre, index, wxyz, B, N, M, K, C1, bn1_mean, bn1_invstd, bn1_gamma, bn1_beta, W2,
      C2, bn2_mean,
                                              bn2_invstd, bn2_gamma, bn2_beta, W3, C3, bn3_mean, bn3_invstd, bn3_gamma, bn3_beta, out, arg, stream));
}
MVP_API int mvp_sa_train_forward_p_f32(int stage, const float* zf, const float* xyz, const float* centre, const int64_t* index, const float*
    wxyz, int64_t B, int64_t N, int64_t M, int64_t K, int64_t C1, const float* bn1_mean, const float* bn1_invstd, const float* bn1_gamma,
    const float* bn1_beta, const float* W2, int64_t C2, const float* bn2_mean, const float* bn2_invstd, const float* bn2_gamma, const float*
    bn2_beta, const float* W3, int64_t C3, double* stat, float eps, float momentum, float* mean, float* invstd, float* running_mean, float*
    running_var, int64_t* num_batches_tracked, float* ymax, float* ymin, uint8_t* amax, uint8_t* amin, int precision, int
    precision_backward, mvp_stream_t stream) {
  MVP_WITH_PRECISION(mvp_sa_train_forward_f32(stage, zf, xyz, centre, index, wxyz, B, N, M, K, C1, bn1_mean, bn1_invstd, bn1_gamma,
      bn1_beta, W2, C2, bn2_mean, bn2_invstd, bn2_gamma, bn2_beta, W3, C3, stat, eps, momentum, mean, invstd, running_mean, running_var,
      num_batches_tracked, ymax, ymin, amax, amin, stream));
}

MVP_API int mvp_sa_train_backward_p_f32(int layer, const float* zf, const float* xyz, const float* centre, const int64_t* index, const
    float* wxyz, int64_t B, int64_t N, int64_t M, int64_t K, int64_t C1, const float* bn1_mean, const float* bn1_invstd, const float*
    bn1_gamma, const float* bn1_beta, const float* W2, int64_t C2, const float* bn2_mean, const float* bn2_invstd, const float* bn2_gamma,
    const float* bn2_beta, const float* W3, int64_t C3, const float* mean_i, const float* invstd_i, const float* gamma_i, const double*
    stat_i, float* dgamma_i, float* dbeta_i, int training, const float* G, const float* pool_dout, const float* pool_out, const uint8_t*
    pool_arg, float* dW, int64_t lddw, float* dZ, double* stat_prev, float* tsum, int precision, int precision_backward, mvp_stream_t stream) {
  MVP_WITH_PRECISION(mvp_sa_train_backward_f32(layer, zf, xyz, centre, index, wxyz, B, N, M, K, C1, bn1_mean, bn1_invstd, bn1_gamma,
      bn1_beta, W2, C2, bn2_mean, bn2_invstd, bn2_gamma, bn2_beta, W3, C3, mean_i, invstd_i, gamma_i, stat_i, dgamma_i, dbeta_i, training,
      G, pool_dout, pool_out, pool_arg, dW, lddw, dZ, stat_prev, tsum, stream));
}
```

mvpnet_amd/optim.py:

```python
import ctypes

import torch

from . import _lib as L


class FusedAdam(torch.optim.Adam):
    def __init__(self, params, lr=1e-3, betas=(0.9, 0.999), eps=1e-8, weight_decay=0.0, amsgrad=False, **kwargs):
        if amsgrad or kwargs.get('maximize') or kwargs.get('capturable') or kwargs.get('differentiable'):
            raise ValueError('FusedAdam covers plain Adam (no amsgrad / maximize / capturable / differentiable)')
        kwargs.pop('fused', None)
        kwargs.pop('foreach', None)
        super().__init__(params, lr=lr, betas=betas, eps=eps, weight_decay=weight_decay, amsgrad=False, foreach=False, fused=False, **kwargs)
        self._plans = {}
        self._step_bufs = {}

    def _plan(self, gi, plist):
        key = tuple(id(p) for p in plist)
        plan = self._plans.get(gi)
        if plan is not None and plan['key'] == key and all(p.data_ptr() == q for p, q in zip(plist, plan['pptr'])) \
                and all(self.state[p]['exp_avg'] is m and self.state[p]['exp_avg_sq'] is v for p, m, v in zip(plist, *plan['keep'])):
            return plan
        n = len(plist)
        arr = lambda vals: (ctypes.c_void_p * n)(*vals)
        moments1 = [self.state[p]['exp_avg'] for p in plist]
        moments2 = [self.state[p]['exp_avg_sq'] for p in plist]
        plan = {'key': key, 'pptr': [p.data_ptr() for p in plist], 'p': arr([p.data_ptr() for p in plist]),
                'm': arr([t.data_ptr() for t in moments1]), 'v': arr([t.data_ptr() for t in moments2]), 'g': (ctypes.c_void_p * n)(),
                'numel': (ctypes.c_int64 * n)(*[p.numel() for p in plist]), 'keep': (moments1, moments2)}
        self._plans[gi] = plan
        return plan

    def _advance_steps(self, gi, plist):
        cache = self._step_bufs.get(gi)
        state = self.state
        if cache is None or len(cache[1]) != len(plist) or any(state[p]['step'] is not v for p, v in zip(plist, cache[1])):
            base = torch.tensor([float(state[p]['step']) for p in plist], dtype=torch.float32)
            views = [base[i] for i in range(len(plist))]
            for p, v in zip(plist, views):
                state[p]['step'] = v
            cache = self._step_bufs[gi] = (base, views)
        cache[0].add_(1.0)
        return cache[0].tolist()

    @torch.no_grad()
    def step(self, closure=None):
        loss = None
        if closure is not None:
            with torch.enable_grad():
                loss = closure()
        for gi, group in enumerate(self.param_groups):
            plist = [p for p in group['params'] if p.grad is not None]
            if not plist:
                continue
            for p in plist:
                if not (p.is_cuda and p.dtype == torch.float32 and p.is_contiguous()) or p.grad.is_sparse:
                    raise RuntimeError('FusedAdam: parameters must be dense contiguous float32 tensors on the GPU (use torch.optim.Adam otherwise)')
                st = self.state[p]
                if len(st) == 0:
                    st['step'] = torch.tensor(0.0, dtype=torch.float32)
                    st['exp_avg'] = torch.zeros_like(p, memory_format=torch.preserve_format)
                    st['exp_avg_sq'] = torch.zeros_like(p, memory_format=torch.preserve_format)
            counts = self._advance_steps(gi, plist)
            plan = self._plan(gi, plist)
            grads = []
            g_arr = plan['g']
            for i, p in enumerate(plist):
                g = p.grad
                if g.dtype != torch.float32 or not g.is_contiguous():
                    g = g.float().contiguous()
                grads.append(g)
                g_arr[i] = g.data_ptr()
            beta1, beta2 = group['betas']
            dev = plist[0].device
            if any(p.device != dev for p in plist):
                raise RuntimeError('FusedAdam: the parameters of a group must live on one device')
            if all(c == counts[0] for c in counts):
                buckets = [(counts[0], plan['p'], g_arr, plan['m'], plan['v'], plan['numel'], len(plist))]
            else:
                buckets = []
                for c in sorted(set(counts)):
                    ids = [i for i, ci in enumerate(counts) if ci == c]
                    sub = lambda arr, typ: (typ * len(ids))(*[arr[i] for i in ids])
                    buckets.append((c, sub(plan['p'], ctypes.c_void_p), sub(g_arr, ctypes.c_void_p), sub(plan['m'], ctypes.c_void_p),
                                    sub(plan['v'], ctypes.c_void_p), sub(plan['numel'], ctypes.c_int64), len(ids)))
            with torch.cuda.device(dev):
                for count, p_arr, gg_arr, m_arr, v_arr, n_arr, n in buckets:
                    code = L._fn('mvp_adam_step_f32')(p_arr, gg_arr, m_arr, v_arr, n_arr, n, float(group['lr']), float(beta1), float(beta2),
                                                      float(group['eps']), float(group['weight_decay']), count,
                                                      torch.cuda.current_stream(dev).cuda_stream)
                    if code != 0:
                        L.check(code, 'mvp_adam_step_f32')
            del grads
        return loss
```

mvpnet_amd/rows.py:

```python
import os
import weakref

import torch
import torch.nn.functional as F
from torch.autograd.function import once_differentiable

from . import _lib as L


FUSE_BWD_MAX_COUT = int(os.environ.get('MVP_BWD_FUSE_MAXC', '64'))
FUSE_BWD_MAX_CIN = int(os.environ.get('MVP_BWD_FUSE_MAXCIN', '96'))
PARTIAL_MIN_ROWS = int(os.environ.get('MVP_PARTIAL_MIN_ROWS', '65536'))
WIDE_BWD = os.environ.get('MVP_BWD_WIDE', '1') != '0'
WIDE_BWD_MIN_ROWS = int(os.environ.get('MVP_BWD_WIDE_MIN_ROWS', '16384'))


WIDE_BWD_64 = os.environ.get('MVP_BWD_WIDE64', '1') != '0'
WIDE_BWD_POOLED = os.environ.get('MVP_BWD_WIDE_POOLED', '1') != '0'
WIDE_BWD_64_MIN_ROWS = int(os.environ.get('MVP_BWD_WIDE64_MIN_ROWS', '262144'))


DX_WIDE = os.environ.get('MVP_DX_WIDE', '0') == '1'
DX_WIDE_MIN_ROWS = int(os.environ.get('MVP_DX_WIDE_MIN_ROWS', '16384'))
DX_WIDE_MAX_COUT = int(os.environ.get('MVP_DX_WIDE_MAXC', '512'))
# ... 93 lines not shown
        self.demand = 0
        self.capacity = 0
        self.depth = 0

    class _Step:
        def __init__(self, pool, dev):
            self.pool, self.dev = pool, dev

        def __enter__(self):
            p = self.pool
            if p.depth == 0:
                p.capacity = max(p.demand, p.cursor)
                p.buf = torch.zeros(p.capacity // 8, dtype=torch.float64, device=self.dev) if p.capacity else None
                p.cursor = p.demand = 0
                if self.dev.type == 'cuda':
                    weight_slices.refresh(self.dev)
            p.depth += 1

        def __exit__(self, *exc):
            self.pool.depth -= 1

    def step(self, dev):
        return ZeroPool._Step(self, dev)

    def zeros(self, shape, dtype, dev):
        if isinstance(shape, int):
            shape = (shape,)
        numel = 1
        for d in shape:
            numel *= int(d)
        nbytes = (numel * torch.empty(0, dtype=dtype).element_size() + 255) // 256 * 256
        self.demand += nbytes
        buf = self.buf
        if buf is None or buf.device != dev or self.cursor + nbytes > self.capacity or numel == 0:
            return torch.zeros(shape, dtype=dtype, device=dev)
        view = buf[self.cursor // 8:(self.cursor + nbytes) // 8].view(dtype)[:numel].view(shape)
        self.cursor += nbytes
        return view


zero_pool = ZeroPool()


class WeightSlices:

    ENABLED = os.environ.get('MVP_WEIGHT_SLICES', '1') != '0'

    class Entry:
        __slots__ = ('weight', 'c0', 'cols', 'bufs', 'cur', 'version', 'ptr')

    def __init__(self):
        self.entries = {}
        self.tables = {}
        self.retired = []

    @staticmethod
    def _src(e):
        return e.weight.detach().reshape(e.weight.size(0), -1)[:, e.c0:e.c0 + e.cols]

    def get(self, weight, c0, c1, ld):
        if not WeightSlices.ENABLED:
            w = weight.detach().reshape(weight.size(0), -1)[:, c0:c1]
            return (F.pad(w, (0, ld - (c1 - c0))) if ld != c1 - c0 else w).contiguous()
        key = (id(weight), c0, c1, ld)
        e = self.entries.get(key)
        if e is None or e.weight is not weight or e.bufs[0].device != weight.device:
            e = WeightSlices.Entry()
            e.weight, e.c0, e.cols, e.cur, e.version, e.ptr = weight, c0, c1 - c0, 0, None, None
            e.bufs = [torch.zeros((weight.size(0), ld), dtype=torch.float32, device=weight.device) for _ in range(2)]
            if not torch.cuda.is_current_stream_capturing():
                self.entries[key] = e
                old = self.tables.pop(weight.device, None)
                if old is not None:
                    self.retired.append(old[0])
        if e.version != weight._version or e.ptr != weight.data_ptr():
            e.cur ^= 1
            e.bufs[e.cur][:, :e.cols].copy_(self._src(e))
            e.version, e.ptr = weight._version, weight.data_ptr()
        return e.bufs[e.cur]

    def invalidate(self):
        for e in self.entries.values():
            e.version = None

    def refresh(self, dev):
        if not WeightSlices.ENABLED:
            return
        mine = [e for e in self.entries.values() if e.bufs[0].device == dev]
        if not mine:
            return
        capturing = torch.cuda.is_current_stream_capturing()
        tab = self.tables.get(dev)
        if (tab is None or any(e.weight.data_ptr() != p for e, p in zip(tab[1], tab[2]))) and not capturing:
            rows = [[], []]
            for e in mine:
                w2 = e.weight.detach().reshape(e.weight.size(0), -1)
                for par in (0, 1):
                    rows[par].append([w2.data_ptr() + 4 * e.c0, e.bufs[par].data_ptr(), w2.stride(0), e.bufs[par].stride(0), w2.size(0), e.cols])
            if tab is not None:
                self.retired.append(tab[0])
            tab = self.tables[dev] = ([torch.tensor(r, dtype=torch.int64).to(dev) for r in rows], mine, [e.weight.data_ptr() for e in mine])
        if tab is None:
            return
        stale = [e.version != e.weight._version or e.ptr != e.weight.data_ptr() for e in tab[1]]
        if not capturing and not any(stale):
            return
        par = tab[1][0].cur ^ 1
        L.call('mvp_copy_slices_f32', tab[0][par], L.ptr(tab[0][par]), len(tab[1]))
        for e in tab[1]:
            e.cur, e.version, e.ptr = par, e.weight._version, e.weight.data_ptr()


weight_slices = WeightSlices()


DW_SIDE_STREAM = os.environ.get('MVP_DW_SIDE_STREAM', '1') != '0'
LINEAR_ASIDE = os.environ.get('MVP_LINEAR_ASIDE', '1') != '0'
DW_FINISH_ON_LOAD = os.environ.get('MVP_DW_FINISH_ON_LOAD', '1') != '0'
REL_DW_FUSED = os.environ.get('MVP_REL_DW_FUSED', '1') != '0'
REL_DW_SPLIT = os.environ.get('MVP_REL_DW_SPLIT', '1') != '0'
_EXP_SKIP_DW = os.environ.get('MVP_EXP_SKIP_DW', '0') == '1'


class WeightUse:
    __slots__ = ('weights', 'shared', 'done', '__weakref__')

    def __init__(self, weights):
        self.weights = list(weights)
        self.shared = False
        self.done = False
        me = weakref.ref(self)
        for w in self.weights:
            live = [r for r in w.__dict__.get('_mvp_uses', ()) if r() is not None and not r().done]
            for r in live:
                r().shared = True
            if live:
                self.shared = True
            live.append(me)
            w.__dict__['_mvp_uses'] = live

    def aside_ok(self):
        return not self.shared and all(w.is_leaf and w.grad is None and not w._backward_hooks and not w._post_accumulate_grad_hooks
                                       for w in self.weights)


class SideStream:
    def __init__(self):
        self.streams = {}
        self.open = set()
        self.keep = []
        self.task = None

    def _join(self):
        for dev in list(self.open):
            torch.cuda.current_stream(dev).wait_stream(self.streams[dev][0])
        self.open.clear()
        self.keep.clear()

    def run(self, dev, name, args, tensors, prec=None):
        st = self.streams.get(dev)
        if st is None:
            st = self.streams[dev] = (torch.cuda.Stream(device=dev), torch.cuda.Event())
        task = torch._C._current_graph_task_id()
        if task != self.task or not self.open:
            torch.autograd.Variable._execution_engine.queue_callback(self._join)
            self.task = task
        self.open.add(dev)
        side, fork = st
        fork.record(torch.cuda.current_stream(dev))
        side.wait_event(fork)
        if dev.index == torch.cuda.current_device():
            L.call_on(side, name, *args, prec=prec)
        else:
            with torch.cuda.stream(side):
                L.call(name, tensors[0], *args, prec=prec)
        self.keep.extend(tensors)


side_stream = SideStream()


class WeightGradSink:

    def __init__(self, weight, users):
        self.shape = tuple(weight.shape)
        self.numel = weight.numel()
        self.users = self.left = users
        self.buf = None
        self.use = WeightUse([weight]) if DW_SIDE_STREAM else None
        self.aside = None

    def buffer(self, dev):
        if self.buf is None:
            self.buf = zero_pool.zeros(self.numel + 4, torch.float32, dev)
        return self.buf

# ... 336 lines not shown
        if not training:
            scale = gamma * invstd
            z = ((y - mean) * invstd) * gamma + beta
            if K > 1:
                z = z.view(G, K, C)
                mask = torch.zeros_like(z)
                mask.scatter_(1, arg.long().unsqueeze(1), 1.0)
                dz = g.unsqueeze(1) * mask
                if relu:
                    dz = dz * (out.unsqueeze(1) > 0)
                dz = dz.reshape(G * K, C)
            else:
                dz = g * (z > 0) if relu else g
            xhat = (y - mean) * invstd
            return dz * scale, (dz * xhat).sum(0), dz.sum(0), None, None, None, None, None, None, None
        stat = torch.empty(2 * C, dtype=torch.float64, device=y.device)
        dy = torch.empty_like(y)
        dgb = torch.empty((2, C), dtype=torch.float32, device=y.device)
        L.call('mvp_bn_rows_backward_f32', y, L.ptr(g), L.ptr(out), L.ptr(arg), L.ptr(y), L.ptr(mean), L.ptr(invstd),
               L.ptr(gamma), L.ptr(beta), G, K, C, int(relu), 1, L.ptr(stat), L.ptr(dy), L.ptr(dgb[0]), L.ptr(dgb[1]),
               L.ptr(_cs_partial(G * K, C, y.device)))
        return dy, dgb[0], dgb[1], None, None, None, None, None, None, None


def bn_act_rows(y, bn, relu=True, K=1):
    if y.dtype != torch.float32 or y.dim() != 2:
        raise RuntimeError('bn_act_rows: (rows, C) float32 expected')
    training = bn.training or bn.running_mean is None
    if bn.training and bn.num_batches_tracked is not None:
        bn.num_batches_tracked.add_(1)
    if bn.momentum is not None:
        momentum = bn.momentum
    elif bn.training and bn.num_batches_tracked is not None:
        momentum = 1.0 / float(bn.num_batches_tracked)
    else:
        momentum = 0.0
    return BNActRows.apply(y.contiguous(), bn.weight, bn.bias, bn.running_mean, bn.running_var, training, momentum, bn.eps,
                           relu, K)


def _partial(R, cols, device):
    if R < PARTIAL_MIN_ROWS:
        return None
    return torch.empty(((R + 127) // 128) * 2 * cols, dtype=torch.float64, device=device)


def _cs_partial(R, C, device):
    return torch.empty(L.lib().mvp_colstats_partial_count(R, C), dtype=torch.float64, device=device)


def _bn_backward(dsrc, out, arg, y, mean, invstd, gamma, beta, G, K, C, relu, training):
    stat = torch.empty(2 * C, dtype=torch.float64, device=y.device)
    dy = torch.empty_like(y)
    dgb = torch.empty((2, C), dtype=torch.float32, device=y.device)
    L.call('mvp_bn_rows_backward_f32', y, L.ptr(dsrc), L.ptr(out), L.ptr(arg), L.ptr(y), L.ptr(mean), L.ptr(invstd),
           L.ptr(gamma), L.ptr(beta), G, K, C, int(relu), int(training), L.ptr(stat), L.ptr(dy), L.ptr(dgb[0]), L.ptr(dgb[1]),
           L.ptr(_cs_partial(G * K, C, y.device)))
    return dy, dgb[0], dgb[1]


def _bn_apply(y, mean, invstd, gamma, beta, G, K, C, relu, pool_sum=False):
    out = torch.empty((G, C), dtype=torch.float32, device=y.device)
    arg = torch.empty((G, C), dtype=torch.uint8, device=y.device) if (K > 1 and not pool_sum) else None
    L.call('mvp_bn_rows_forward_f32', y, L.ptr(y), L.ptr(gamma), L.ptr(beta), G, K, C, 0, 0.0, 0.0, int(relu), None, None, None,
           L.ptr(mean), L.ptr(invstd), L.ptr(out), L.ptr(arg), None)
    return out, arg


class MLPChainRows(torch.autograd.Function):

    @staticmethod
    def forward(ctx, x0, training, K, eps_mom, bn_buffers, first_stat, pool_sum, *params):
        nl = len(params) // 3
        R = x0.size(0)
        dev = x0.device
        prec = ctx.prec = L.current_precision()
        opts = pool_sum if isinstance(pool_sum, dict) else {'sum': bool(pool_sum)}
        drop_p, drop_seed = opts.get('drop_p', 0.0), opts.get('drop_seed', 0)
        ctx.dw_use = opts.get('use')
        ctx.defer = opts.get('defer')
        pool_sum = bool(opts.get('sum', False))
        rel, w0_param = opts.get('rel', (None, None))
        ctx.rel = (rel, w0_param)
        ctx.dropout = (float(drop_p), int(drop_seed))
        ys, means, invstds = [], [], []
        act = (None, None, None, None)
        x = x0
        couts = [x0.size(1) if params[3 * i] is None else params[3 * i].size(0) for i in range(nl)]
        arena = zero_pool.zeros(2 * sum(couts) + nl, torch.float64, dev) if training else None
        wl = params[3 * (nl - 1)]
        pooled = bool(POOL_WITHOUT_Y and training and K == 32 and not pool_sum and nl >= 2 and wl is not None and R % 32 == 0 and R >= 32768 and
                      prec[0] != 0 and wl.size(0) <= min(64, FUSE_BWD_MAX_COUT) and wl.size(1) <= 64 and
                      wl.size(0) % 4 == 0 and wl.size(1) % 4 == 0)
        off = 0
        for i in range(nl):
            w, gamma, beta = params[3 * i], params[3 * i + 1], params[3 * i + 2]
            eps, mom = eps_mom[i]
            stat = arena[off:off + 2 * couts[i] + 1] if training else None
            off += 2 * couts[i] + 1
            if w is None:
                assert i == 0
                cout = x0.size(1)
                y = x0
                if training and isinstance(first_stat, tuple):
                    first_mi = first_stat[1]
                    ys.append(y)
                    means.append(first_mi[:cout])
                    invstds.append(first_mi[cout:])
                    act = (means[-1], invstds[-1], gamma, beta)
                    x = y
                    continue
                if training and first_stat is not None:
                    stat = first_stat
                elif training:
                    L.call('mvp_colstats_f32', y, L.ptr(y), R, cout, L.ptr(stat), L.ptr(_cs_partial(R, cout, dev)))
            else:
                cout, cin = w.size(0), w.size(1)
                if i == 0 and rel is not None:
                    cin_f = x0.size(1)
                    assert cin == cin_f + 4 and act[0] is None
                    wrel = weight_slices.get(w0_param, cin_f, cin, 4)
                    rm, rv, nbt = bn_buffers[i]
                    y = torch.empty((R, cout), dtype=torch.float32, device=dev)
                    if training:
                        mean = torch.empty(cout, dtype=torch.float32, device=dev)
                        invstd = torch.empty(cout, dtype=torch.float32, device=dev)
                        L.call('mvp_mlp_forward_rel_bn_f32', x, L.ptr(x), R, cin_f, cin_f, L.ptr(w), cin, cout, L.ptr(rel), L.ptr(wrel), L.ptr(y),
                               L.ptr(stat), L.ptr(_partial(R, cout, dev)), float(eps), float(mom), L.ptr(mean), L.ptr(invstd), L.ptr(rm), L.ptr(rv),
                               L.ptr(nbt), prec=prec)
                    else:
                        L.call('mvp_mlp_forward_rel_bn_f32', x, L.ptr(x), R, cin_f, cin_f, L.ptr(w), cin, cout, L.ptr(rel), L.ptr(wrel), L.ptr(y),
                               None, None, 0.0, 0.0, None, None, None, None, None, prec=prec)
                        mean, invstd = rm, eval_invstd.get(rv, eps)
                    ys.append(y)
                    means.append(mean)
                    invstds.append(invstd)
                    act = (mean, invstd, gamma, beta)
                    x = y
                    continue
                if pooled and i == nl - 1:
                    G = R // K
                    rm, rv, nbt = bn_buffers[i]
                    mean = torch.empty(cout, dtype=torch.float32, device=dev)
                    invstd = torch.empty(cout, dtype=torch.float32, device=dev)
                    ymax = torch.empty((G, cout), dtype=torch.float32, device=dev)
                    ymin = torch.empty((G, cout), dtype=torch.float32, device=dev)
                    amax = torch.empty((G, cout), dtype=torch.uint8, device=dev)
                    amin = torch.empty((G, cout), dtype=torch.uint8, device=dev)
                    L.call('mvp_mlp_forward_pool_f32', x, L.ptr(x), R, cin, x.size(1), L.ptr(w), cin, cout, L.ptr(act[0]), L.ptr(act[1]),
                           L.ptr(act[2]), L.ptr(act[3]), L.ptr(ymax), L.ptr(ymin), L.ptr(amax), L.ptr(amin), L.ptr(stat),
                           L.ptr(torch.empty(((R + 127) // 128) * 2 * cout, dtype=torch.float64, device=dev)), float(eps), float(mom),
                           L.ptr(mean), L.ptr(invstd), L.ptr(rm), L.ptr(rv), L.ptr(nbt), prec=prec)
                    out = torch.empty((G, cout), dtype=torch.float32, device=dev)
                    arg = torch.empty((G, cout), dtype=torch.uint8, device=dev)
                    ysel = torch.empty((G, cout), dtype=torch.float32, device=dev)
                    L.call('mvp_pool_finalize_f32', ymax, L.ptr(ymax), L.ptr(ymin), L.ptr(amax), L.ptr(amin), L.ptr(mean), L.ptr(invstd),
                           L.ptr(gamma), L.ptr(beta), G, cout, 1, L.ptr(out), L.ptr(arg), L.ptr(ysel))
                    ys.append(ysel)
                    means.append(mean)
                    invstds.append(invstd)
                    break
                y = torch.empty((R, cout), dtype=torch.float32, device=dev)
                if training and R > 0:
                    rm, rv, nbt = bn_buffers[i]
                    mean = torch.empty(cout, dtype=torch.float32, device=dev)
                    invstd = torch.empty(cout, dtype=torch.float32, device=dev)
                    L.call('mvp_mlp_forward_bn_f32', x, L.ptr(x), R, cin, x.size(1), L.ptr(w), cin, cout, L.ptr(act[0]), L.ptr(act[1]),
                           L.ptr(act[2]), L.ptr(act[3]), L.ptr(y), L.ptr(stat), L.ptr(_partial(R, cout, dev)), float(eps), float(mom),
                           L.ptr(mean), L.ptr(invstd), L.ptr(rm), L.ptr(rv), L.ptr(nbt), prec=prec)
                    ys.append(y)
                    means.append(mean)
                    invstds.append(invstd)
                    act = (mean, invstd, gamma, beta)
                    x = y
                    continue
                L.call('mvp_mlp_forward_f32', x, L.ptr(x), R, cin, x.size(1), L.ptr(w), cin, cout, L.ptr(act[0]), L.ptr(act[1]),
                       L.ptr(act[2]), L.ptr(act[3]), None, L.ptr(y), L.ptr(stat), L.ptr(_partial(R, cout, dev) if training else None), prec=prec)
            rm, rv, nbt = bn_buffers[i]
            if training:
                mean = torch.empty(cout, dtype=torch.float32, device=dev)
                invstd = torch.empty(cout, dtype=torch.float32, device=dev)
                L.call('mvp_bn_finalize_f32', y, L.ptr(stat), R, cout, float(eps), float(mom), L.ptr(mean), L.ptr(invstd),
                       L.ptr(rm), L.ptr(rv), L.ptr(nbt))
            else:
                mean, invstd = rm, eval_invstd.get(rv, eps)
            ys.append(y)
            means.append(mean)
            invstds.append(invstd)
            act = (mean, invstd, gamma, beta)
            x = y
        cl = ys[-1].size(1)
        G = R // K
        if not pooled and drop_p > 0:
            assert K == 1
            out, arg = torch.empty((R, cl), dtype=torch.float32, device=dev), None
            L.call('mvp_bn_rows_forward_dropout_f32', x0, L.ptr(ys[-1]), L.ptr(params[-2]), L.ptr(params[-1]), R, cl, 0, 0.0, 0.0, 1, None, None,
                   None, L.ptr(means[-1]), L.ptr(invstds[-1]), L.ptr(out), None, float(drop_p), int(drop_seed))
        elif not pooled:
            out, arg = _bn_apply(ys[-1], means[-1], invstds[-1], params[-2], params[-1], G, K, cl, True, pool_sum)
        ao = opts.get('act_out')
        ctx.act_out = None
        if ao is not None and ActivationHandOver.ENABLED and not pooled and K == 1 and training is not None:
            ao.info, ao.stat = (ys[-1], means[-1], invstds[-1], params[-2], params[-1], float(drop_p), int(drop_seed)), None
            ctx.act_out = ao
        ctx.first_linear = params[0] is not None
        ctx.pooled = pooled
        ctx.save_for_backward(x0, out, arg, *ys, *means, *invstds, *[p for p in params if p is not None])
        ctx.cfg = (nl, training, K, R)
        return out

    @staticmethod
    @once_differentiable
    def backward(ctx, grad_out):
        nl, training, K, R = ctx.cfg
        saved = ctx.saved_tensors
        x0, out, arg = saved[0], saved[1], saved[2]
        ys = saved[3:3 + nl]
        means = saved[3 + nl:3 + 2 * nl]
        invstds = saved[3 + 2 * nl:3 + 3 * nl]
        params = list(saved[3 + 3 * nl:])
        if not ctx.first_linear:
            params.insert(0, None)
        grads = [None] * (3 * nl)
        g = grad_out.contiguous()
        G = R // K
        cl = ys[-1].size(1)
        pool = None
        wl = params[3 * (nl - 1)]
        handed = None
        if ctx.act_out is not None and ctx.act_out.stat is not None:
            handed, ctx.act_out.stat = ctx.act_out.stat, None
        last_wide = bool(handed is None and not ctx.pooled and K == 1 and nl >= 2 and wl is not None and g.is_cuda and
                         wide_backward_ok(ctx.prec, R, wl.size(0), wl.size(1), ys[nl - 2].size(1)) and R * cl < 2 ** 32 and
                         aligned16(g, ys[-1], ys[nl - 2]))
        last_wide_sum = bool(WIDE_BWD_POOLED and not ctx.pooled and K > 1 and arg is None and ctx.dropout[0] == 0 and nl >= 2 and wl is not None and
                             g.is_cuda and wide_backward_ok(ctx.prec, R, wl.size(0), wl.size(1), ys[nl - 2].size(1)) and R * cl < 2 ** 32 and
                             aligned16(g, ys[-1], ys[nl - 2]))
        if handed is not None:
            dy, dgam, dbet = None, None, None
        elif ctx.pooled:
            ysel = ys[-1]
            stat_l = torch.empty(2 * cl, dtype=torch.float64, device=g.device)
            L.call('mvp_pool_backward_stats_f32', g, L.ptr(g), L.ptr(out), L.ptr(ysel), L.ptr(means[-1]), L.ptr(invstds[-1]), G, cl, 1,
                   L.ptr(stat_l), L.ptr(_cs_partial(G, cl, g.device)))
            pool = (g, out, arg)
            dy, dgam, dbet = None, None, None
        elif last_wide_sum:
            stat_d = torch.empty(2 * cl, dtype=torch.float64, device=g.device)
            L.call('mvp_bn_rows_backward_f32', g, L.ptr(g), None, None, L.ptr(ys[-1]), L.ptr(means[-1]), L.ptr(invstds[-1]), L.ptr(params[-2]),
                   L.ptr(params[-1]), G, K, cl, 1, int(training), L.ptr(stat_d), None, None, None, L.ptr(_cs_partial(R, cl, g.device)))
            dy, dgam, dbet = None, None, None
        elif last_wide:
            stat_d = torch.empty(2 * cl, dtype=torch.float64, device=g.device)
            L.call('mvp_bn_rows_backward_dropout_f32', g, L.ptr(g), L.ptr(ys[-1]), L.ptr(means[-1]), L.ptr(invstds[-1]), L.ptr(params[-2]),
                   L.ptr(params[-1]), R, cl, 1, int(training), L.ptr(stat_d), None, None, None, L.ptr(_cs_partial(R, cl, g.device)),
                   ctx.dropout[0], ctx.dropout[1])
            dy, dgam, dbet = None, None, None
        elif ctx.dropout[0] > 0:
            stat_d = torch.empty(2 * cl, dtype=torch.float64, device=g.device)
            dy = torch.empty_like(ys[-1])
# ... 50 lines not shown
                grads[0] = dw
                dgb0 = pending.view(2, cout).to(torch.float32)
                grads[1], grads[2] = dgb0[1], dgb0[0]
                ws_ptr, ws_floats = L.current_dw_workspace(dev)
                if REL_DW_FUSED and ws_ptr is None and 32 < cin_f <= 64 and aligned16(src, rel):
                    L.call('mvp_mlp_weight_grad_finish_rel_p_f32', gcur, L.ptr(gcur), L.ptr(ys[0]), L.ptr(means[0]), L.ptr(invstds[0]), L.ptr(params[1]),
                           L.ptr(pending), int(training), L.ptr(src), R, cout, cin_f, cin_f, L.ptr(rel), L.ptr(dw), L.ptr_at(dw, cin_f), cin, *ctx.prec)
                    break
                for xs, ncol, c0 in ((src, cin_f, 0), (rel, 4, cin_f)):
                    fargs = (L.ptr(gcur), L.ptr(ys[0]), L.ptr(means[0]), L.ptr(invstds[0]), L.ptr(params[1]), L.ptr(pending), int(training), L.ptr(xs), R,
                             cout, ncol, ncol, L.ptr_at(dw, c0), cin)
                    if dw_aside and xs is not rel and ws_ptr is None:
                        side_stream.run(dev, 'mvp_mlp_weight_grad_finish_p_f32', fargs + (None, 0) + tuple(ctx.prec),
                                        (gcur, ys[0], xs, dw, pending, means[0], invstds[0], params[1]))
                    else:
                        L.call('mvp_mlp_weight_grad_finish_p_f32', gcur, *(fargs + (ws_ptr, ws_floats) + tuple(ctx.prec)))
                break
            if pending is not None and not fuse and not dxw:
                dyi = torch.empty((R, cout), dtype=torch.float32, device=dev)
                dgb = torch.empty((2, cout), dtype=torch.float32, device=dev)
                L.call('mvp_bn_rows_backward_finish_f32', gcur, L.ptr(gcur), L.ptr(ys[i]), L.ptr(means[i]), L.ptr(invstds[i]), L.ptr(params[3 * i + 1]),
                       L.ptr(params[3 * i + 2]), R, cout, int(training), L.ptr(pending), L.ptr(dyi), L.ptr(dgb[0]), L.ptr(dgb[1]))
                gcur, pending = dyi, None
                dgam, dbet = dgb[0], dgb[1]
            if pending is None:
                grads[3 * i + 1], grads[3 * i + 2] = dgam, dbet
            if dxw:
                act = (means[i - 1], invstds[i - 1], params[3 * i - 2], params[3 * i - 1])
                dw = dw_arena[dw_off:dw_off + cout * cin].view(cout, cin)
                dw_off += cout * cin
                grads[3 * i] = dw
                stat = st_arena[st_off:st_off + 2 * cin]
                st_off += 2 * cin
                dz = torch.empty((R, cin), dtype=torch.float32, device=dev)
                fin = pending is not None
                dgb = torch.empty((2, cout), dtype=torch.float32, device=dev) if fin else None
                if fin:
                    wg_name = 'mvp_mlp_weight_grad_finish_act_p_f32'
                    wg_args = (L.ptr(gcur), L.ptr(ys[i]), L.ptr(means[i]), L.ptr(invstds[i]), L.ptr(params[3 * i + 1]), L.ptr(pending), int(training), L.ptr(src),
                               R, cout, cin, src.size(1), L.ptr(act[0]), L.ptr(act[1]), L.ptr(act[2]), L.ptr(act[3]), L.ptr(dw), cin, None, 0) + tuple(ctx.prec)
                    wg_keep = (gcur, ys[i], means[i], invstds[i], params[3 * i + 1], pending, src, dw) + act
                    if dw_aside:
                        side_stream.run(dev, wg_name, wg_args, wg_keep)
                    else:
                        L.call(wg_name, gcur, *wg_args)
                else:
                    wg_args = (L.ptr(gcur), L.ptr(src), R, cout, cin, src.size(1), L.ptr(act[0]), L.ptr(act[1]), L.ptr(act[2]), L.ptr(act[3]), L.ptr(dw), cin)
                    if dw_aside:
                        side_stream.run(dev, 'mvp_mlp_weight_grad_f32', wg_args, (gcur, src, dw) + act, prec=ctx.prec)
                    else:
                        L.call('mvp_mlp_weight_grad_f32', gcur, *wg_args, prec=ctx.prec)
                nbytes = int(L.lib().mvp_mlp_input_grad_wide_workspace_bytes(cout, cin))
                wimg = torch.empty(nbytes, dtype=torch.uint8, device=dev)
                L.call('mvp_mlp_input_grad_wide_f32', gcur, L.ptr(gcur), L.ptr(ys[i]) if fin else None, L.ptr(means[i]) if fin else None,
                       L.ptr(invstds[i]) if fin else None, L.ptr(params[3 * i + 1]) if fin else None, L.ptr(pending), L.ptr(None if dgb is None else dgb[0]),
                       L.ptr(None if dgb is None else dgb[1]), int(training), L.ptr(src), src.size(1), L.ptr(act[0]), L.ptr(act[1]), L.ptr(act[2]), L.ptr(act[3]),
                       L.ptr(w), cin, R, cout, cin, L.ptr(dz), L.ptr(stat), L.ptr(wimg), nbytes, prec=ctx.prec)
                if fin:
                    grads[3 * i + 1], grads[3 * i + 2] = dgb[0], dgb[1]
                gcur, pending = dz, stat
                continue
            if w is None:
                dx0 = gcur
                break
            act = none4 if i == 0 else (means[i - 1], invstds[i - 1], params[3 * i - 2], params[3 * i - 1])
            dw = dw_arena[dw_off:dw_off + cout * cin].view(cout, cin)
            dw_off += cout * cin
            grads[3 * i] = dw
            stat = None
            if i > 0:
                stat = st_arena[st_off:st_off + 2 * cin]
                st_off += 2 * cin
            dz = torch.empty((R, cin if rel is None else src.size(1)), dtype=torch.float32, device=dev) if need_dz else None
            if rel is not None:
                cin_f = src.size(1)
                for xs, ncol, c0 in ((src, cin_f, 0), (rel, 4, cin_f)):
                    wg_args = (L.ptr(gcur), L.ptr(xs), R, cout, ncol, ncol, None, None, None, None, L.ptr_at(dw, c0), cin)
                    if dw_aside and not (REL_DW_SPLIT and xs is rel and not need_dz):
                        side_stream.run(dev, 'mvp_mlp_weight_grad_f32', wg_args, (gcur, xs, dw), prec=ctx.prec)
                    else:
                        L.call('mvp_mlp_weight_grad_f32', gcur, *wg_args, prec=ctx.prec)
                if need_dz:
                    wf = weight_slices.get(w0_param, 0, cin_f, cin_f)
                    L.call('mvp_mlp_input_grad_f32', gcur, L.ptr(gcur), R, cout, L.ptr(wf), cin_f, None, None, None, None, None, L.ptr(dz), None, None, prec=ctx.prec)
                    dx0 = dz
                break
            if wide:
                mode = 0 if pending is None else (2 if ((last_wide or last_wide_sum) and i == nl - 1) else 1)
                pool_k = K if (last_wide_sum and i == nl - 1) else 1
                dgb = torch.empty((2, cout), dtype=torch.float32, device=dev) if pending is not None else None
                ticket = zero_pool.zeros(2, torch.int32, dev)
                ws_ptr, ws_floats = L.current_dw_workspace(dev)
                fin = pending is not None
                L.call('mvp_mlp_layer_backward_wide_pooled_f32', src, L.ptr(gcur), L.ptr(ys[i]) if fin else None, L.ptr(means[i]) if fin else None,
                       L.ptr(invstds[i]) if fin else None, L.ptr(params[3 * i + 1]) if fin else None, L.ptr(params[3 * i + 2]) if mode == 2 else None,
                       L.ptr(pending), L.ptr(None if dgb is None else dgb[0]), L.ptr(None if dgb is None else dgb[1]), int(training), mode, pool_k,
                       float(ctx.dropout[0]) if mode == 2 else 0.0, int(ctx.dropout[1]) if mode == 2 else 0, L.ptr(src), src.size(1), L.ptr(act[0]),
                       L.ptr(act[1]), L.ptr(act[2]), L.ptr(act[3]), L.ptr(w), cin, R, cout, cin, L.ptr(dw), cin, L.ptr(dz), L.ptr(stat), L.ptr(ticket),
                       ws_ptr, ws_floats, prec=ctx.prec)
                if pending is not None:
                    grads[3 * i + 1], grads[3 * i + 2] = dgb[0], dgb[1]
            elif fuse:
                dgb = torch.empty((2, cout), dtype=torch.float32, device=dev) if pending is not None else None
                part = torch.empty(L.lib().mvp_mlp_layer_backward_partial_count(R, cin), dtype=torch.float64, device=dev) if (i > 0 and need_dz) else None
                L.call('mvp_mlp_layer_backward_f32', src, L.ptr(gcur), L.ptr(ys[i]) if (pending is not None and not pool_here) else None,
                       L.ptr(means[i]) if pending is not None else None, L.ptr(invstds[i]) if pending is not None else None,
                       L.ptr(params[3 * i + 1]) if pending is not None else None, L.ptr(pending), L.ptr(None if dgb is None else dgb[0]),
                       L.ptr(None if dgb is None else dgb[1]), int(training), L.ptr(src), src.size(1), L.ptr(act[0]), L.ptr(act[1]), L.ptr(act[2]),
                       L.ptr(act[3]), L.ptr(w), cin, R, cout, cin, L.ptr(dw), cin, L.ptr(dz), L.ptr(stat), L.ptr(part),
                       L.ptr(pool[0]) if pool_here else None, L.ptr(pool[1]) if pool_here else None, L.ptr(pool[2]) if pool_here else None, prec=ctx.prec)
                if pending is not None:
                    grads[3 * i + 1], grads[3 * i + 2] = dgb[0], dgb[1]
            else:
                wg_args = (L.ptr(gcur), L.ptr(src), R, cout, cin, src.size(1), L.ptr(act[0]), L.ptr(act[1]), L.ptr(act[2]), L.ptr(act[3]),
                           L.ptr(dw), cin)
                if _EXP_SKIP_DW:
                    pass
                elif dw_aside:
                    side_stream.run(dev, 'mvp_mlp_weight_grad_f32', wg_args, (gcur, src, dw) + tuple(t for t in act if t is not None), prec=ctx.prec)
                else:
                    L.call('mvp_mlp_weight_grad_f32', gcur, *wg_args, prec=ctx.prec)
                if need_dz and i > 0:
                    pm, pi, pg, pb = act
                    L.call('mvp_mlp_input_grad_f32', gcur, L.ptr(gcur), R, cout, L.ptr(w), cin, L.ptr(ys[i - 1]), L.ptr(pm), L.ptr(pi),
                           L.ptr(pg), L.ptr(pb), L.ptr(dz), L.ptr(stat), L.ptr(_partial(R, cin, dev)), prec=ctx.prec)
                elif need_dz:
                    L.call('mvp_mlp_input_grad_f32', gcur, L.ptr(gcur), R, cout, L.ptr(w), cin, None, None, None, None, None, L.ptr(dz), None, None, prec=ctx.prec)
            if i > 0:
                gcur, pending = dz, stat
            elif need_dz:
                dx0 = dz if x0.size(1) == cin else F.pad(dz, (0, x0.size(1) - cin))
        if ctx.dw_use is not None:
            ctx.dw_use.done = True
        return (dx0, None, None, None, None, None, None) + tuple(grads)


class RelationRows(torch.autograd.Function):

    @staticmethod
    def forward(ctx, feature, src_xyz, tgt_xyz):
        L.require_gpu(feature, src_xyz, tgt_xyz)
        B, N, k, C = feature.shape
        out = torch.empty((B, N, k, C + 4), dtype=torch.float32, device=feature.device)
        L.call('mvp_relation_rows_f32', feature, L.ptr(feature), L.ptr(src_xyz), L.ptr(tgt_xyz), B * N, k, C, L.ptr(out))
        ctx.C = C
        return out

    @staticmethod
    @once_differentiable
    def backward(ctx, g):
        return g[..., :ctx.C].contiguous(), None, None


def relation_rows(feature, src_xyz, tgt_xyz):
    return RelationRows.apply(feature.contiguous(), src_xyz.contiguous(), tgt_xyz.contiguous())


class LinearRows(torch.autograd.Function):

    @staticmethod
    def forward(ctx, x, w_full, bias, c0=0, c1=None, sink=None, act_src=None):
        ctx.sink = sink
        info = None if act_src is None else act_src.info
        ctx.act_src = act_src if (info is not None and ActivationHandOver.ENABLED and x.is_cuda and tuple(info[0].shape) == tuple(x.shape)) else None
        prec = ctx.prec = L.current_precision()
        w2 = w_full.detach().reshape(w_full.size(0), -1)
        c1 = w2.size(1) if c1 is None else c1
        R, ldx = x.shape
        cin = c1 - c0
        if w2.is_cuda and w2.dtype == torch.float32:
            w = weight_slices.get(w_full, c0, c1, ldx)
        else:
            w = w2[:, c0:c1]
            if ldx != cin:
                w = torch.nn.functional.pad(w, (0, ldx - cin))
            w = w.contiguous()
        L.require_gpu(x, w, bias)
        cout = w.size(0)
        y = torch.empty((R, cout), dtype=torch.float32, device=x.device)
        L.call('mvp_mlp_forward_f32', x, L.ptr(x), R, ldx, ldx, L.ptr(w), ldx, cout, None, None, None, None, L.ptr(bias), L.ptr(y), None, None, prec=prec)
        ctx.save_for_backward(x, w)
        ctx.has_bias = bias is not None
        ctx.slice = (c0, cin, tuple(w_full.shape))
        ctx.bias_param = bias if (bias is not None and bias.is_leaf) else None
        ctx.dw_use = WeightUse([w_full]) if (DW_SIDE_STREAM and LINEAR_ASIDE and sink is None and c0 == 0 and c1 == w2.size(1) and ctx.needs_input_grad[1]) else None
        return y

    @staticmethod
    @once_differentiable
    def backward(ctx, gy):
        x, w = ctx.saved_tensors
        R, cin = x.shape
        cout = w.size(0)
        gy = gy.contiguous()
        gx = gw = gb = None
        aside = False
        if ctx.needs_input_grad[0]:
            gx = torch.empty_like(x)
            src = ctx.act_src
            if src is not None and src.info is not None:
                yp, pm, pi, pg, pb, drop_p, drop_seed = src.info
                stat = zero_pool.zeros(2 * cin, torch.float64, gy.device)
                part = L.ptr(_partial(R, cin, gy.device) if R > 65536 else None)
                if drop_p > 0:
                    L.call('mvp_mlp_input_grad_dropout_f32', gy, L.ptr(gy), R, cout, L.ptr(w), cin, L.ptr(yp), L.ptr(pm), L.ptr(pi), L.ptr(pg), L.ptr(pb),
                           drop_p, drop_seed, L.ptr(gx), L.ptr(stat), part, prec=ctx.prec)
                else:
                    L.call('mvp_mlp_input_grad_f32', gy, L.ptr(gy), R, cout, L.ptr(w), cin, L.ptr(yp), L.ptr(pm), L.ptr(pi), L.ptr(pg), L.ptr(pb), L.ptr(gx),
                           L.ptr(stat), part, prec=ctx.prec)
                src.stat = stat
            else:
                L.call('mvp_mlp_input_grad_f32', gy, L.ptr(gy), R, cout, L.ptr(w), cin, None, None, None, None, None, L.ptr(gx), None, None, prec=ctx.prec)
        if ctx.needs_input_grad[1]:
            c0, ncol, shape = ctx.slice
            sink = ctx.sink
            if sink is not None:
                buf = sink.buffer(gy.device)
                sink.run(gy.device, 'mvp_mlp_weight_grad_f32', (L.ptr(gy), L.ptr(x), R, cout, ncol, cin, None, None, None, None,
                                                                L.ptr_at(buf, c0), sink.numel // cout), (gy, x), prec=ctx.prec)
                gw = sink.done()
            else:
                gw = zero_pool.zeros(shape, torch.float32, w.device)
                wg_args = (L.ptr(gy), L.ptr(x), R, cout, ncol, cin, None, None, None, None, L.ptr_at(gw, c0), gw.numel() // cout)
                use = ctx.dw_use
                aside = use is not None and DW_SIDE_STREAM and use.aside_ok()
                if aside:
                    side_stream.run(gy.device, 'mvp_mlp_weight_grad_f32', wg_args, (gy, x), prec=ctx.prec)
                else:
                    L.call('mvp_mlp_weight_grad_f32', gy, *wg_args, prec=ctx.prec)
                if use is not None:
                    use.done = True
        if ctx.has_bias and ctx.needs_input_grad[2]:
            st = side_stream.streams.get(gy.device)
            bp = ctx.bias_param
            if (aside and st is not None and gy.device in side_stream.open and bp is not None and bp.grad is None and not bp._backward_hooks
                    and not bp._post_accumulate_grad_hooks):
                gb = torch.empty(cout, dtype=gy.dtype, device=gy.device)
                with torch.cuda.stream(st[0]):
                    torch.sum(gy, 0, out=gb)
            else:
                gb = gy.sum(0)
        return gx, gw, gb, None, None, None, None


def linear_rows(x, weight, bias=None, cols=None, sink=None, act_src=None):
    c0, c1 = (0, None) if cols is None else cols
    return LinearRows.apply(x.contiguous(), weight, bias, c0, c1, sink, act_src)


def linear_rows_bf16(x, weight, bias=None, scale=None, shift=None, relu=False):
    if not (x.is_cuda and weight.is_cuda):
        raise RuntimeError('mvpnet_amd ops run on the GPU only; there is no CPU fallback')
    if x.dtype != torch.bfloat16 or x.dim() != 2 or x.stride(1) != 1:
        raise RuntimeError('linear_rows_bf16: x must be a (R, C_in) bfloat16 tensor with unit column stride')
    w = weight.detach().reshape(weight.size(0), -1)
    if w.dtype != torch.float32 or not w.is_contiguous() or w.size(1) != x.size(1):
        raise RuntimeError('linear_rows_bf16: weight must be contiguous float32 (C_out, C_in)')
    R, cin = x.shape
    cout = w.size(0)
    f = lambda t: None if t is None else t.detach().float().contiguous()
    bias, scale, shift = f(bias), f(scale), f(shift)
    y = torch.empty((R, cout), dtype=torch.bfloat16, device=x.device)
    L.call('mvp_mlp_forward_bf16', x, L.ptr(x), R, cin, x.stride(0), L.ptr(w), cin, cout, L.ptr(bias), L.ptr(scale), L.ptr(shift), int(bool(relu)),
           L.ptr(y), cout)
    return y


SA_TRAIN_FUSED = os.environ.get('MVP_SA_TRAIN', '1') != '0'


STATS1_REPLICAS = int(os.environ.get('MVP_SA_STATS1_REPLICAS', '16'))


def sa_level_train_widths_ok(c1, c2, c3):
    return c1 >= 4 and max(c1, c2) <= 64 and (c3 <= 64 or (c3 <= 128 and min(c1, c2) > 32))


def sa_level_train_ok(zf, mlp, K):
    if not (SA_TRAIN_FUSED and zf is not None and zf.is_cuda and zf.dtype == torch.float32 and len(mlp) == 3 and K == 32 and mlp_chain_is_fused(mlp)):
        return False
    if L.DW_WORKSPACE:
        return False
    ps = parts(mlp)
    c1, c2, c3 = (q.w.size(0) for q in ps)
    return sa_level_train_widths_ok(c1, c2, c3) and all(q.bn.training for q in ps) and L.current_precision()[0] != 0 and \
        all(q.w.is_contiguous() for q in ps)


class SALevelTrain(torch.autograd.Function):

    @staticmethod
    def forward(ctx, zf, xyz, centre, index, offsets, slots, dsum, gsum, w1_full, sink, bns, W2, W3, g1, b1, g2, b2, g3, b3):
        L.require_gpu(zf, xyz, centre, index, W2, W3)
        prec = ctx.prec = L.current_precision()
        ctx.sink = sink
# ... 209 lines not shown
```

Baseline: 5032 chunks/s.

## Precompute split-bf16 weight images once per step and stream them into LDS

Adds a per-step weight refresh kernel that pre-splits each MLP weight into three bf16 pieces in the tile-ready layout (weight images), rebuilt only when the parameter version changes. The MLP forward and input-grad kernels gain an IMG variant that loads these pre-split slabs straight into LDS via global_load_lds instead of splitting fp32 weights in every tile. This removes redundant per-block weight conversion and shuffle work, at the cost of extra image memory, one refresh launch per step, and version-tracking complexity in Python.

```diff
diff --git a/include/mvp_hip.h b/include/mvp_hip.h
--- a/include/mvp_hip.h
+++ b/include/mvp_hip.h
@@ -338,6 +338,25 @@
 int mvp_mlp_input_grad_dropout_p_f32(const float* dY, int64_t R, int64_t Cout, const float* W, int64_t Cin, const float* y_prev, const
     float* mean, const float* invstd, const float* gamma, const float* beta, float drop_p, uint64_t drop_seed, float* dZ, double* stat,
     double* partial, int precision, int precision_backward, mvp_stream_t stream);
+int mvp_refresh_weights_f32(const int64_t* slices, int64_t n_slices, const int64_t* images, int64_t n_images, mvp_stream_t stream);
+int64_t mvp_mlp_weight_image_bytes(int64_t rows, int64_t cols, int across);
+int mvp_mlp_forward_img_p_f32(const float* X, int64_t R, int64_t Cin, int64_t ldx, const float* W, int64_t ldw, int64_t Cout, const
+    float* act_mean, const float* act_invstd, const float* act_gamma, const float* act_beta, const float* bias, float* Y,
+    double* stat, double* partial, const void* image, int precision, int precision_backward, mvp_stream_t stream);
+int mvp_mlp_forward_bn_img_p_f32(const float* X, int64_t R, int64_t Cin, int64_t ldx, const float* W, int64_t ldw, int64_t Cout,
+    const float* act_mean, const float* act_invstd, const float* act_gamma, const float* act_beta, float* Y, double* stat,
+    double* partial, float eps, float momentum, float* mean, float* invstd, float* running_mean, float* running_var, int64_t*
+    num_batches_tracked, const void* image, int precision, int precision_backward, mvp_stream_t stream);
+int mvp_mlp_forward_rel_bn_img_p_f32(const float* X, int64_t R, int64_t Cin, int64_t ldx, const float* W, int64_t ldw, int64_t Cout,
+    const float* rel, const float* wrel, float* Y, double* stat, double* partial, float eps, float momentum, float* mean, float*
+    invstd, float* running_mean, float* running_var, int64_t* num_batches_tracked, const void* image, int precision,
+    int precision_backward, mvp_stream_t stream);
+int mvp_mlp_input_grad_img_p_f32(const float* dY, int64_t R, int64_t Cout, const float* W, int64_t Cin, const float* y_prev, const
+    float* mean, const float* invstd, const float* gamma, const float* beta, float* dZ, double* stat, double* partial, const void*
+    image, int precision, int precision_backward, mvp_stream_t stream);
+int mvp_mlp_input_grad_dropout_img_p_f32(const float* dY, int64_t R, int64_t Cout, const float* W, int64_t Cin, const float* y_prev, const
+    float* mean, const float* invstd, const float* gamma, const float* beta, float drop_p, uint64_t drop_seed, float* dZ, double* stat,
+    double* partial, const void* image, int precision, int precision_backward, mvp_stream_t stream);
 int mvp_mlp_weight_grad_p_f32(const float* dY, const float* X, int64_t R, int64_t Cout, int64_t Cin, int64_t ldx, const float*
     act_mean, const float* act_invstd, const float* act_gamma, const float* act_beta, float* dW, int64_t lddw, int precision,
     int precision_backward, mvp_stream_t stream);
diff --git a/mvpnet_amd/_lib.py b/mvpnet_amd/_lib.py
--- a/mvpnet_amd/_lib.py
+++ b/mvpnet_amd/_lib.py
@@ -131,6 +131,9 @@
            'mvp_mlp_weight_grad_f32', 'mvp_mlp_weight_grad_ws_f32', 'mvp_mlp_layer_backward_f32', 'mvp_mlp_layer_backward_ws_f32',
            'mvp_sa_fused_forward_f32', 'mvp_sa_train_forward_f32', 'mvp_sa_train_backward_f32']:
     _SIGNATURES[_n[:-4] + '_p_f32'] = _SIGNATURES[_n][:-1] + [ctypes.c_int, ctypes.c_int, _ptr]
+for _n in ['mvp_mlp_forward_f32', 'mvp_mlp_forward_bn_f32', 'mvp_mlp_forward_rel_bn_f32', 'mvp_mlp_input_grad_f32', 'mvp_mlp_input_grad_dropout_f32']:
+    _SIGNATURES[_n[:-4] + '_img_p_f32'] = _SIGNATURES[_n][:-1] + [_ptr, ctypes.c_int, ctypes.c_int, _ptr]
+_SIGNATURES['mvp_refresh_weights_f32'] = [_ptr, _i64, _ptr, _i64, _ptr]
 _SIGNATURES['mvp_mlp_layer_backward_wide_p_f32'] = [_ptr] * 9 + [ctypes.c_int, ctypes.c_int, _f32, ctypes.c_uint64, _ptr, _i64, _ptr, _ptr, _ptr, _ptr, _ptr, _i64,
                                                     _i64, _i64, _i64, _ptr, _i64, _ptr, _ptr, _ptr, _ptr, _i64, ctypes.c_int, ctypes.c_int, _ptr]
 _SIGNATURES['mvp_mlp_layer_backward_wide_pooled_p_f32'] = [_ptr] * 9 + [ctypes.c_int, ctypes.c_int, _i64, _f32, ctypes.c_uint64, _ptr, _i64, _ptr, _ptr, _ptr, _ptr, _ptr, _i64,
@@ -141,7 +144,7 @@
                                                         ctypes.c_int, _ptr]
 _SIGNATURES['mvp_mlp_input_grad_wide_p_f32'] = [_ptr] * 8 + [ctypes.c_int, _ptr, _i64, _ptr, _ptr, _ptr, _ptr, _ptr, _i64, _i64, _i64, _i64, _ptr, _ptr, _ptr, _i64,
                                                  ctypes.c_int, ctypes.c_int, _ptr]
-EXPORTS = ['mvp_version', 'mvp_strerror', 'mvp_lift_workspace_bytes', 'mvp_ball_query_grid_workspace', 'mvp_knn3_grid_workspace', 'mvp_mlp_weight_grad_workspace_floats', 'mvp_mlp_input_grad_wide_workspace_bytes', 'mvp_group_lin_partial_count', 'mvp_colstats_partial_count',
+EXPORTS = ['mvp_version', 'mvp_strerror', 'mvp_mlp_weight_image_bytes', 'mvp_lift_workspace_bytes', 'mvp_ball_query_grid_workspace', 'mvp_knn3_grid_workspace', 'mvp_mlp_weight_grad_workspace_floats', 'mvp_mlp_input_grad_wide_workspace_bytes', 'mvp_group_lin_partial_count', 'mvp_colstats_partial_count',
            'mvp_set_mlp_precision', 'mvp_get_mlp_precision', 'mvp_mlp_layer_backward_partial_count', 'mvp_set_mlp_stream', 'mvp_set_mlp_precision_backward', 'mvp_get_mlp_precision_backward', 'mvp_mlp_precision_scope', 'mvp_set_fps_mode', 'mvp_fps_debug_spin_limit', 'mvp_fps_last_kernel'] + sorted(_SIGNATURES)
 
 
@@ -167,6 +170,8 @@
         handle.mvp_mlp_weight_grad_workspace_floats.argtypes = []
         handle.mvp_mlp_input_grad_wide_workspace_bytes.restype = ctypes.c_int64
         handle.mvp_mlp_input_grad_wide_workspace_bytes.argtypes = [ctypes.c_int64, ctypes.c_int64]
+        handle.mvp_mlp_weight_image_bytes.restype = ctypes.c_int64
+        handle.mvp_mlp_weight_image_bytes.argtypes = [_i64, _i64, ctypes.c_int]
         handle.mvp_colstats_partial_count.restype = ctypes.c_int64
         handle.mvp_colstats_partial_count.argtypes = [_i64, _i64]
         handle.mvp_set_mlp_precision.restype = ctypes.c_int
@@ -363,22 +368,26 @@
     return args + (ws.data_ptr(), ws.numel())
 
 
-def call_on(stream, name, *args, prec=None):
+def call_on(stream, name, *args, prec=None, img=None):
     if DW_WORKSPACE and name in _DW_WS_NAMES:
         name, args = _DW_WS_NAMES[name], _with_dw_workspace(stream.device.index, stream.cuda_stream, args)
-    if prec is not None:
+    if img is not None:
+        name, args = name[:-4] + '_img_p_f32', args + (img,) + (prec if prec is not None else (-1, -1))
+    elif prec is not None:
         name, args = name[:-4] + '_p_f32', args + prec
     code = _fn(name)(*args, stream.cuda_stream)
     if code != 0:
         check(code, name)
 
 
-def call(name, tensor_for_device, *args, prec=None):
+def call(name, tensor_for_device, *args, prec=None, img=None):
     index = tensor_for_device.device.index
     if DW_WORKSPACE and name in _DW_WS_NAMES:
         handle = _raw_stream(index) if _raw_stream is not None else torch.cuda.current_stream(tensor_for_device.device).cuda_stream
         name, args = _DW_WS_NAMES[name], _with_dw_workspace(index, handle, args)
-    if prec is not None:
+    if img is not None:
+        name, args = name[:-4] + '_img_p_f32', args + (img,) + (prec if prec is not None else (-1, -1))
+    elif prec is not None:
         name, args = name[:-4] + '_p_f32', args + prec
     if _raw_stream is not None and index == _raw_device():
         code = _fn(name)(*args, _raw_stream(index))
diff --git a/mvpnet_amd/csrc/mlp.hip b/mvpnet_amd/csrc/mlp.hip
--- a/mvpnet_amd/csrc/mlp.hip
+++ b/mvpnet_amd/csrc/mlp.hip
@@ -15,6 +15,7 @@
 int g_mlp_min_width = 0;
 thread_local int tl_mlp_terms = -1;
 thread_local int tl_mlp_terms_bwd = -1;
+thread_local const void* tl_mlp_image = nullptr;
 int g_mlp_stream = 1;
 
 namespace {
@@ -46,13 +47,17 @@
 #ifndef MVP_MLP_WAVES128
 #define MVP_MLP_WAVES128 3
 #endif
-template <int BN, int BK, bool WT, bool VEC, int ACT, int NS>
-__global__ __launch_bounds__(kMT, (BN == 128 && VEC && WT && NS == 0) ? MVP_MLP_WAVES128 : (NS != 0 && BN == 128) ? 2 : 1) void mlp_fwd_kernel(const float* __restrict__ X, int64_t R, int Cin, int ldx,
-                                                      const float* __restrict__ W, int ldw, int Cout,
-                                                      InAct act, const float* __restrict__ bias, EpiBwd epi,
-                                                      float* __restrict__ Y , double* __restrict__ stat,
-                                                      double* __restrict__ partial) {
+#ifndef MVP_IMG_GLDS
+#define MVP_IMG_GLDS 1
+#endif
+template <int BN, int BK, bool WT, bool VEC, int ACT, int NS, bool IMG>
+__device__ __forceinline__ void mlp_tile(const float* __restrict__ X, int64_t R, int Cin, int ldx,
+                                         const float* __restrict__ W, int ldw, int Cout,
+                                         InAct act, const float* __restrict__ bias, EpiBwd epi,
+                                         float* __restrict__ Y , double* __restrict__ stat,
+                                         double* __restrict__ partial, const unsigned char* __restrict__ img, int npad) {
   static_assert(NS == 0 || (VEC && BK == 32), "split-bf16 needs the vector path and 32-wide slabs");
+  static_assert(!IMG || NS != 0, "weight images exist for the split-bf16 contraction only");
   constexpr int kLdB = BK + 4;
   constexpr int NT = BK / 8;
   constexpr int kColB = 80;
@@ -150,9 +155,31 @@
   constexpr int CPP = kMT / LPC;
   constexpr int NV = BN / CPP;
   constexpr int KH = BK / 32;
-  float4 bn[WT ? NB * KH : NV];
-  auto load_b = [&](int k0) {
-    if constexpr (WT && NS != 0) {
+  float4 bn[IMG ? 1 : WT ? NB * KH : NV];
+  constexpr int kUnits = NS * BN * 5;
+  constexpr int NU = (kUnits + kMT - 1) / kMT;
+  constexpr bool kGlds = MVP_IMG_GLDS != 0;
+  u32x4 bi[(IMG && !kGlds) ? NU : 1];
+  auto load_b = [&](int k0, int buf) {
+    if constexpr (IMG) {
+      const unsigned char* slab = img + ((size_t)(k0 / BK) * 3 * npad + col0) * kColB;
+#pragma unroll
+      for (int u = 0; u < NU; ++u) {
+        const int i = u * kMT + tid;
+        if constexpr (kGlds) {
+          if (kUnits % kMT == 0 || u + 1 < NU || i < kUnits) {
+            const int pc = i / (BN * 5), off = i - pc * (BN * 5);
+            const unsigned char* src = slab + (size_t)pc * npad * kColB + (size_t)off * 16;
+            unsigned char* dst = BsRaw + (size_t)buf * kBufB + (size_t)(u * kMT + wave * 64) * 16;
+            __builtin_amdgcn_global_load_lds((const __attribute__((address_space(1))) void*)src, (__attribute__((address_space(3))) void*)dst, 16, 0, 0);
+          }
+        } else {
+          const int ic = min(i, kUnits - 1);
+          const int pc = ic / (BN * 5), off = ic - pc * (BN * 5);
+          bi[u] = *reinterpret_cast<const u32x4*>(slab + (size_t)pc * npad * kColB + (size_t)off * 16);
+        }
+      }
+    } else if constexpr (WT && NS != 0) {
       const int c = tid & 31, kq = (tid >> 5) * 4;
 #pragma unroll
       for (int u = 0; u < NB; ++u) {
@@ -196,7 +223,18 @@
     }
   };
   auto store_b = [&](int buf, int k0) {
-    if constexpr (NS != 0) {
+    if constexpr (IMG) {
+      if constexpr (kGlds) {
+        asm volatile("s_waitcnt vmcnt(0)" ::: "memory");
+      } else {
+#pragma unroll
+        for (int u = 0; u < NU; ++u) {
+          const int i = u * kMT + tid;
+          if (kUnits % kMT == 0 || u + 1 < NU || i < kUnits) *reinterpret_cast<u32x4*>(BsRaw + (size_t)buf * kBufB + (size_t)i * 16) = bi[u];
+        }
+      }
+      return;
+    } else if constexpr (NS != 0) {
       const int c = WT ? (tid & 31) : (tid / LPC), kq = WT ? (tid >> 5) * 4 : (tid % LPC) * 4;
       const int t = kq >> 3, unit = 2 * (t >> 1) + ((kq >> 2) & 1);
       unsigned char* base = BsRaw + (size_t)buf * kBufB + unit * 16 + (t & 1) * 8;
@@ -271,7 +309,7 @@
   for (int i = 0; i < 16; ++i) acc1[i] = 0.f;
 
   load_a(0);
-  load_b(0);
+  load_b(0, 0);
   __syncthreads();
   store_b(0, 0);
   activate(0);
@@ -282,7 +320,7 @@
     const bool more = k0 + BK < Cin;
     if (more) {
       load_a(k0 + BK);
-      load_b(k0 + BK);
+      load_b(k0 + BK, buf ^ 1);
     }
     __builtin_amdgcn_sched_barrier(0);
     __builtin_amdgcn_s_setprio(MVP_MFMA_PRIO);
@@ -469,6 +507,77 @@
         }
       }
     }
+  }
+}
+
+template <int BN, int BK, bool WT, bool VEC, int ACT, int NS>
+__global__ __launch_bounds__(kMT, (BN == 128 && VEC && WT && NS == 0) ? MVP_MLP_WAVES128 : (NS != 0 && BN == 128) ? 2 : 1) void mlp_fwd_kernel(const float* __restrict__ X, int64_t R, int Cin, int ldx,
+                                                      const float* __restrict__ W, int ldw, int Cout,
+                                                      InAct act, const float* __restrict__ bias, EpiBwd epi,
+                                                      float* __restrict__ Y , double* __restrict__ stat,
+                                                      double* __restrict__ partial) {
+  mlp_tile<BN, BK, WT, VEC, ACT, NS, false>(X, R, Cin, ldx, W, ldw, Cout, act, bias, epi, Y, stat, partial, nullptr, 0);
+}
+
+#ifndef MVP_IMG_WAVES128
+#define MVP_IMG_WAVES128 2
+#endif
+template <int BN, bool WT, int ACT, int NS>
+__global__ __launch_bounds__(kMT, BN == 128 ? MVP_IMG_WAVES128 : 1) void mlp_img_kernel(const float* __restrict__ X, int64_t R, int Cin, int ldx, int Cout, InAct act,
+                                                                   const float* __restrict__ bias, EpiBwd epi, float* __restrict__ Y,
+                                                                   double* __restrict__ stat, double* __restrict__ partial,
+                                                                   const unsigned char* __restrict__ img, int npad) {
+  mlp_tile<BN, 32, WT, true, ACT, NS, true>(X, R, Cin, ldx, nullptr, 0, Cout, act, bias, epi, Y, stat, partial, img, npad);
+}
+
+constexpr int kImgColB = 80;
+__global__ __launch_bounds__(256) void weight_refresh_kernel(const int64_t* __restrict__ slices, int n_slices, const int64_t* __restrict__ images) {
+  if ((int)blockIdx.y < n_slices) {
+    const int64_t* e = slices + (size_t)blockIdx.y * 6;
+    const float* src = reinterpret_cast<const float*>(e[0]);
+    float* dst = reinterpret_cast<float*>(e[1]);
+    const int64_t lds = e[2], ldd = e[3], rows = e[4], cols = e[5];
+    const int64_t total = rows * cols;
+    for (int64_t i = (int64_t)blockIdx.x * 256 + threadIdx.x; i < total; i += (int64_t)gridDim.x * 256) {
+      const int64_t r = i / cols, c = i - r * cols;
+      dst[r * ldd + c] = src[r * lds + c];
+    }
+    return;
+  }
+  const int64_t* e = images + (size_t)(blockIdx.y - n_slices) * 8;
+  const float* src = reinterpret_cast<const float*>(e[0]);
+  unsigned char* dst = reinterpret_cast<unsigned char*>(e[1]);
+  const int64_t lds = e[2];
+  const int rows = (int)e[3], cols = (int)e[4];
+  const bool across = e[5] != 0;
+  const int npad = (int)e[6], kpad = (int)e[7];
+  const int ncol = across ? cols : rows, nk = across ? rows : cols;
+  const int64_t total = (int64_t)(kpad / 32) * 5 * npad;
+  for (int64_t i = (int64_t)blockIdx.x * 256 + threadIdx.x; i < total; i += (int64_t)gridDim.x * 256) {
+    const int c = (int)(i % npad);
+    const int unit = (int)((i / npad) % 5);
+    const int slab = (int)(i / ((int64_t)npad * 5));
+    u32x4 out[3] = {u32x4{0u, 0u, 0u, 0u}, u32x4{0u, 0u, 0u, 0u}, u32x4{0u, 0u, 0u, 0u}};
+    if (unit < 4 && c < ncol) {
+      const int sI = unit >> 1, h = unit & 1;
+      float v[8];
+#pragma unroll
+      for (int p = 0; p < 8; ++p) {
+        const int k = slab * 32 + 16 * sI + 8 * (p >> 2) + 4 * h + (p & 3);
+        v[p] = k < nk ? (across ? src[(size_t)k * lds + c] : src[(size_t)c * lds + k]) : 0.f;
+      }
+#pragma unroll
+      for (int q = 0; q < 4; ++q) {
+        unsigned pc[3];
+        split_pair<3>(v[2 * q], v[2 * q + 1], pc);
+        out[0][q] = pc[0];
+        out[1][q] = pc[1];
+        out[2][q] = pc[2];
+      }
+    }
+#pragma unroll
+    for (int pc = 0; pc < 3; ++pc)
+      *reinterpret_cast<u32x4*>(dst + (((size_t)slab * 3 + pc) * npad + c) * kImgColB + unit * 16) = out[pc];
   }
 }
 
@@ -878,7 +987,7 @@
 
 template <bool WT>
 void launch_mlp(const float* X, int64_t R, int K, int ldx, const float* W, int ldw, int N, InAct act, const float* bias, EpiBwd epi,
-                float* Y, double* stat, double* partial, hipStream_t s) {
+                float* Y, double* stat, double* partial, hipStream_t s, const void* image = nullptr) {
   const unsigned gx = (unsigned)cdiv(R, kBM);
   const bool vec = ldx % 4 == 0 && ldw % 4 == 0 && K % 4 == 0 && N % 4 == 0 && ((uintptr_t)X) % 16 == 0 && ((uintptr_t)W) % 16 == 0 &&
                    K >= 4 && N >= 4;
@@ -907,7 +1016,31 @@
     else if (ns == 3) MVP_MLP_LAUNCH(BN, true, 3);                                                                                 \
     else MVP_MLP_LAUNCH(BN, true, 0);                                                                                              \
   } while (0)
-  if (bn == 32) MVP_MLP_BY_NS(32);
+  if (image && ns != 0) {
+    const unsigned char* img = static_cast<const unsigned char*>(image);
+    const int npad = (int)(cdiv(N, 128) * 128);
+    const dim3 grid(gx, (unsigned)cdiv(N, bn));
+#define MVP_IMG_LAUNCH(BN, ACT_, NS_)                                                                                              \
+  hipLaunchKernelGGL((mlp_img_kernel<BN, WT, ACT_, NS_>), grid, dim3(kMT), 0, s, X, R, K, ldx, N, act, bias, epi, Y, stat, partial, img, npad)
+#define MVP_IMG_BY_ACT(BN, NS_)                                                                                                    \
+  do {                                                                                                                             \
+    if (WT || act.mean == nullptr) MVP_IMG_LAUNCH(BN, 0, NS_);                                                                     \
+    else if (K <= kMaxActCin) MVP_IMG_LAUNCH(BN, (WT ? 0 : 1), NS_);                                                               \
+    else MVP_IMG_LAUNCH(BN, (WT ? 0 : 2), NS_);                                                                                    \
+  } while (0)
+#define MVP_IMG_BY_NS(BN)                                                                                                          \
+  do {                                                                                                                             \
+    if (ns == 1) MVP_IMG_BY_ACT(BN, 1);                                                                                            \
+    else if (ns == 2) MVP_IMG_BY_ACT(BN, 2);                                                                                       \
+    else MVP_IMG_BY_ACT(BN, 3);                                                                                                    \
+  } while (0)
+    if (bn == 32) MVP_IMG_BY_NS(32);
+    else if (bn == 64) MVP_IMG_BY_NS(64);
+    else MVP_IMG_BY_NS(128);
+#undef MVP_IMG_BY_NS
+#undef MVP_IMG_BY_ACT
+#undef MVP_IMG_LAUNCH
+  } else if (bn == 32) MVP_MLP_BY_NS(32);
   else if (bn == 64) MVP_MLP_BY_NS(64);
   else MVP_MLP_BY_NS(128);
 #undef MVP_MLP_BY_NS
@@ -931,7 +1064,7 @@
     if (rc != MVP_EUNSUPPORTED) return rc;
   }
   launch_mlp<false>(X, R, (int)Cin, (int)ldx, W, (int)ldw, (int)Cout, act, bias, EpiBwd{nullptr, nullptr, nullptr, nullptr, nullptr, rel, wrel}, Y, stat,
-                    stat ? partial : nullptr, s);
+                    stat ? partial : nullptr, s, tl_mlp_image);
   if (stat && bn_mean)
     launch_stats_reduce_finalize(partial, partial ? (int64_t)gx : 0, (int)(2 * Cout), stat, fin, s);
   else if (stat && partial)
@@ -1256,7 +1389,7 @@
   if (make_dropout(y_prev ? drop_p : 0.f, drop_seed, R, Cin, 1, &epi.drop) != MVP_OK) return MVP_EINVAL;
   double* st = y_prev ? stat : nullptr;
   const unsigned gx = (unsigned)cdiv(R, kBM);
-  launch_mlp<true>(dY, R, (int)Cout, (int)Cout, W, (int)Cin, (int)Cin, act, nullptr, epi, dZ, st, st ? partial : nullptr, s);
+  launch_mlp<true>(dY, R, (int)Cout, (int)Cout, W, (int)Cin, (int)Cin, act, nullptr, epi, dZ, st, st ? partial : nullptr, s, tl_mlp_image);
   if (st && partial)
     launch_stats_reduce(partial, (int64_t)gx, (int)(2 * Cin), stat, s);
   return mvp_launch_status();
@@ -1274,6 +1407,21 @@
                                            double* stat, double* partial, mvp_stream_t stream) {
   MVP_NONNULL(y_prev);
   return input_grad_impl(dY, R, Cout, W, Cin, y_prev, mean, invstd, gamma, beta, drop_p, drop_seed, dZ, stat, partial, stream);
+}
+
+MVP_API int mvp_refresh_weights_f32(const int64_t* slices, int64_t n_slices, const int64_t* images, int64_t n_images, mvp_stream_t stream) {
+  MVP_REQUIRE(n_slices >= 0 && n_images >= 0 && n_slices + n_images < 65536);
+  if (n_slices + n_images == 0) return MVP_OK;
+  if (n_slices) MVP_NONNULL(slices);
+  if (n_images) MVP_NONNULL(images);
+  hipLaunchKernelGGL(weight_refresh_kernel, dim3(32, (unsigned)(n_slices + n_images)), dim3(256), 0, static_cast<hipStream_t>(stream), slices,
+                     (int)n_slices, images);
+  return mvp_launch_status();
+}
+MVP_API int64_t mvp_mlp_weight_image_bytes(int64_t rows, int64_t cols, int across) {
+  if (rows <= 0 || cols <= 0) return 0;
+  const int64_t n = across ? cols : rows, k = across ? rows : cols;
+  return cdiv(k, 32) * 3 * (cdiv(n, 128) * 128) * kImgColB;
 }
 
 MVP_API int mvp_set_mlp_precision(int terms, int min_width) {
diff --git a/mvpnet_amd/csrc/mlp_common.h b/mvpnet_amd/csrc/mlp_common.h
--- a/mvpnet_amd/csrc/mlp_common.h
+++ b/mvpnet_amd/csrc/mlp_common.h
@@ -7,6 +7,7 @@
 
 extern thread_local int tl_mlp_terms;
 extern thread_local int tl_mlp_terms_bwd;
+extern thread_local const void* tl_mlp_image;
 static inline int mlp_terms() { return tl_mlp_terms >= 0 ? tl_mlp_terms : g_mlp_terms; }
 static inline int mlp_terms_bwd() { return tl_mlp_terms_bwd >= 0 ? tl_mlp_terms_bwd : g_mlp_terms_bwd; }
 static inline int mlp_fwd_pieces() { return mlp_terms() == 1 ? 1 : mlp_terms() == 3 ? 2 : mlp_terms() == 6 ? 3 : 0; }
diff --git a/mvpnet_amd/csrc/mlp_prec.hip b/mvpnet_amd/csrc/mlp_prec.hip
--- a/mvpnet_amd/csrc/mlp_prec.hip
+++ b/mvpnet_amd/csrc/mlp_prec.hip
@@ -59,6 +59,51 @@
                                              const float* mean, const float* invstd, const float* gamma, const float* beta, float drop_p,
                                              uint64_t drop_seed, float* dZ, double* stat, double* partial, int precision, int precision_backward,
                                              mvp_stream_t stream) {
+  MVP_WITH_PRECISION(mvp_mlp_input_grad_dropout_f32(dY, R, Cout, W, Cin, y_prev, mean, invstd, gamma, beta, drop_p, drop_seed, dZ, stat, partial, stream));
+}
+namespace {
+struct ImageArg {
+  const void* old;
+  explicit ImageArg(const void* image) : old(tl_mlp_image) { tl_mlp_image = image; }
+  ~ImageArg() { tl_mlp_image = old; }
+};
+}
+MVP_API int mvp_mlp_forward_img_p_f32(const float* X, int64_t R, int64_t Cin, int64_t ldx, const float* W, int64_t ldw, int64_t Cout,
+                                      const float* act_mean, const float* act_invstd, const float* act_gamma, const float* act_beta,
+                                      const float* bias, float* Y, double* stat, double* partial, const void* image, int precision,
+                                      int precision_backward, mvp_stream_t stream) {
+  ImageArg img(image);
+  MVP_WITH_PRECISION(mvp_mlp_forward_f32(X, R, Cin, ldx, W, ldw, Cout, act_mean, act_invstd, act_gamma, act_beta, bias, Y, stat, partial, stream));
+}
+MVP_API int mvp_mlp_forward_bn_img_p_f32(const float* X, int64_t R, int64_t Cin, int64_t ldx, const float* W, int64_t ldw, int64_t Cout,
+                                         const float* act_mean, const float* act_invstd, const float* act_gamma, const float* act_beta, float* Y,
+                                         double* stat, double* partial, float eps, float momentum, float* mean, float* invstd,
+                                         float* running_mean, float* running_var, int64_t* num_batches_tracked, const void* image,
+                                         int precision, int precision_backward, mvp_stream_t stream) {
+  ImageArg img(image);
+  MVP_WITH_PRECISION(mvp_mlp_forward_bn_f32(X, R, Cin, ldx, W, ldw, Cout, act_mean, act_invstd, act_gamma, act_beta, Y, stat, partial, eps, momentum,
+                                            mean, invstd, running_mean, running_var, num_batches_tracked, stream));
+}
+MVP_API int mvp_mlp_forward_rel_bn_img_p_f32(const float* X, int64_t R, int64_t Cin, int64_t ldx, const float* W, int64_t ldw, int64_t Cout,
+                                             const float* rel, const float* wrel, float* Y, double* stat, double* partial, float eps,
+                                             float momentum, float* mean, float* invstd, float* running_mean, float* running_var,
+                                             int64_t* num_batches_tracked, const void* image, int precision, int precision_backward,
+                                             mvp_stream_t stream) {
+  ImageArg img(image);
+  MVP_WITH_PRECISION(mvp_mlp_forward_rel_bn_f32(X, R, Cin, ldx, W, ldw, Cout, rel, wrel, Y, stat, partial, eps, momentum, mean, invstd, running_mean,
+                                                running_var, num_batches_tracked, stream));
+}
+MVP_API int mvp_mlp_input_grad_img_p_f32(const float* dY, int64_t R, int64_t Cout, const float* W, int64_t Cin, const float* y_prev,
+                                         const float* mean, const float* invstd, const float* gamma, const float* beta, float* dZ, double* stat,
+                                         double* partial, const void* image, int precision, int precision_backward, mvp_stream_t stream) {
+  ImageArg img(image);
+  MVP_WITH_PRECISION(mvp_mlp_input_grad_f32(dY, R, Cout, W, Cin, y_prev, mean, invstd, gamma, beta, dZ, stat, partial, stream));
+}
+MVP_API int mvp_mlp_input_grad_dropout_img_p_f32(const float* dY, int64_t R, int64_t Cout, const float* W, int64_t Cin, const float* y_prev,
+                                                 const float* mean, const float* invstd, const float* gamma, const float* beta, float drop_p,
+                                                 uint64_t drop_seed, float* dZ, double* stat, double* partial, const void* image, int precision,
+                                                 int precision_backward, mvp_stream_t stream) {
+  ImageArg img(image);
   MVP_WITH_PRECISION(mvp_mlp_input_grad_dropout_f32(dY, R, Cout, W, Cin, y_prev, mean, invstd, gamma, beta, drop_p, drop_seed, dZ, stat, partial, stream));
 }
 MVP_API int mvp_mlp_weight_grad_p_f32(const float* dY, const float* X, int64_t R, int64_t Cout, int64_t Cin, int64_t ldx,
diff --git a/mvpnet_amd/optim.py b/mvpnet_amd/optim.py
--- a/mvpnet_amd/optim.py
+++ b/mvpnet_amd/optim.py
@@ -91,5 +91,6 @@
                                                       torch.cuda.current_stream(dev).cuda_stream)
                     if code != 0:
                         L.check(code, 'mvp_adam_step_f32')
+            torch.autograd.graph.increment_version(plist)
             del grads
         return loss
diff --git a/mvpnet_amd/rows.py b/mvpnet_amd/rows.py
--- a/mvpnet_amd/rows.py
+++ b/mvpnet_amd/rows.py
@@ -199,13 +199,12 @@
     def invalidate(self):
         for e in self.entries.values():
             e.version = None
+        weight_images.invalidate()
 
     def refresh(self, dev):
-        if not WeightSlices.ENABLED:
-            return
-        mine = [e for e in self.entries.values() if e.bufs[0].device == dev]
+        mine = [e for e in self.entries.values() if e.bufs[0].device == dev] if WeightSlices.ENABLED else []
         if not mine:
-            return
+            return weight_images.refresh(dev)
         capturing = torch.cuda.is_current_stream_capturing()
         tab = self.tables.get(dev)
         if (tab is None or any(e.weight.data_ptr() != p for e, p in zip(tab[1], tab[2]))) and not capturing:
@@ -218,17 +217,120 @@
                 self.retired.append(tab[0])
             tab = self.tables[dev] = ([torch.tensor(r, dtype=torch.int64).to(dev) for r in rows], mine, [e.weight.data_ptr() for e in mine])
         if tab is None:
-            return
+            return weight_images.refresh(dev)
         stale = [e.version != e.weight._version or e.ptr != e.weight.data_ptr() for e in tab[1]]
-        if not capturing and not any(stale):
+        images = weight_images.pending(dev, capturing)
+        if not capturing and not any(stale) and not (images and images[3]):
             return
         par = tab[1][0].cur ^ 1
-        L.call('mvp_copy_slices_f32', tab[0][par], L.ptr(tab[0][par]), len(tab[1]))
+        if images:
+            L.call('mvp_refresh_weights_f32', tab[0][par], L.ptr(tab[0][par]), len(tab[1]), L.ptr(images[0]), len(images[1]))
+            weight_images.commit(images)
+        else:
+            L.call('mvp_copy_slices_f32', tab[0][par], L.ptr(tab[0][par]), len(tab[1]))
         for e in tab[1]:
             e.cur, e.version, e.ptr = par, e.weight._version, e.weight.data_ptr()
 
 
 weight_slices = WeightSlices()
+
+
+class WeightImages:
+
+    ENABLED = os.environ.get('MVP_WEIGHT_IMAGES', '1') != '0'
+
+    class Entry:
+        __slots__ = ('weight', 'c0', 'cols', 'across', 'npad', 'kpad', 'bufs', 'tabs', 'cur', 'version', 'ptr')
+
+    def __init__(self):
+        self.entries = {}
+        self.tables = {}
+        self.retired = []
+
+    @staticmethod
+    def row(e, par):
+        w2 = e.weight.detach().reshape(e.weight.size(0), -1)
+        return [w2.data_ptr() + 4 * e.c0, e.bufs[par].data_ptr(), w2.stride(0), w2.size(0), e.cols, e.across, e.npad, e.kpad]
+
+    def get(self, weight, across, c0=0, c1=None, k=0):
+        if not WeightImages.ENABLED or weight.dtype != torch.float32:
+            return None
+        base = weight._base if weight._base is not None else weight
+        if base.numel() != weight.numel() or base.data_ptr() != weight.data_ptr() or not base.is_contiguous():
+            return None
+        weight = base
+        rows = weight.size(0)
+        c1 = weight.numel() // rows if c1 is None else c1
+        cols = c1 - c0
+        n, kk = (cols, rows) if across else (rows, cols)
+        npad, kpad = (n + 127) // 128 * 128, (max(kk, k) + 31) // 32 * 32
+        key = (id(weight), c0, c1, across, kpad)
+        e = self.entries.get(key)
+        capturing = torch.cuda.is_current_stream_capturing()
+        if e is None or e.weight is not weight or e.bufs[0].device != weight.device:
+            if capturing:
+                return None
+            e = WeightImages.Entry()
+            e.weight, e.c0, e.cols, e.across, e.npad, e.kpad, e.cur, e.version, e.ptr = weight, c0, cols, int(across), npad, kpad, 0, None, None
+            e.bufs = [torch.empty(kpad // 32 * 3 * npad * 80, dtype=torch.uint8, device=weight.device) for _ in range(2)]
+            e.tabs = None
+            self.entries[key] = e
+            old = self.tables.pop(weight.device, None)
+            if old is not None:
+                self.retired.append(old[0])
+        if e.version != weight._version or e.ptr != weight.data_ptr():
+            if capturing:
+                return None
+            if e.tabs is None or e.ptr != weight.data_ptr():
+                e.tabs = [torch.tensor([self.row(e, par)], dtype=torch.int64).to(weight.device) for par in (0, 1)]
+            e.cur ^= 1
+            L.call('mvp_refresh_weights_f32', weight, None, 0, L.ptr(e.tabs[e.cur]), 1)
+            e.version, e.ptr = weight._version, weight.data_ptr()
+        return e.bufs[e.cur]
+
+    def invalidate(self):
+        for e in self.entries.values():
+            e.version = None
+
+    def pending(self, dev, capturing):
+        if not WeightImages.ENABLED:
+            return None
+        tab = self.tables.get(dev)
+        if (tab is None or any(e.weight.data_ptr() != p for e, p in zip(tab[1], tab[2]))) and not capturing:
+            mine = [e for e in self.entries.values() if e.bufs[0].device == dev]
+            if not mine:
+                return None
+            if tab is not None:
+                self.retired.append(tab[0])
+            tab = self.tables[dev] = ([torch.tensor([self.row(e, par) for e in mine], dtype=torch.int64).to(dev) for par in (0, 1)], mine,
+                                      [e.weight.data_ptr() for e in mine])
+        if tab is None:
+            return None
+        par = tab[1][0].cur ^ 1
+        return tab[0][par], tab[1], par, any(e.version != e.weight._version or e.ptr != e.weight.data_ptr() for e in tab[1])
+
+    def commit(self, pending):
+        for e in pending[1]:
+            e.cur, e.version, e.ptr = pending[2], e.weight._version, e.weight.data_ptr()
+
+    def refresh(self, dev):
+        p = self.pending(dev, torch.cuda.is_current_stream_capturing())
+        if p is not None and (p[3] or torch.cuda.is_current_stream_capturing()):
+            L.call('mvp_refresh_weights_f32', p[0], None, 0, L.ptr(p[0]), len(p[1]))
+            self.commit(p)
+
+
+weight_images = WeightImages()
+
+
+_MLP_STREAM = os.environ.get('MVP_MLP_STREAM', '1') != '0'
+
+
+def _image(weight, across, R=0, cin=0, cout=0, c0=0, c1=None, k=0):
+    if weight is None or not weight.is_cuda or (not across and R >= 32768 and cin <= 128 and cout <= 128 and _MLP_STREAM):
+        return None
+    t = weight_images.get(weight, across, c0, c1, k)
+    return None if t is None else t.data_ptr()
 
 
 DW_SIDE_STREAM = os.environ.get('MVP_DW_SIDE_STREAM', '1') != '0'
@@ -731,6 +833,7 @@
         pool_sum = bool(opts.get('sum', False))
         rel, w0_param = opts.get('rel', (None, None))
         ctx.rel = (rel, w0_param)
+        ctx.w_refs = [params[3 * i] for i in range(nl)]
         ctx.dropout = (float(drop_p), int(drop_seed))
         ys, means, invstds = [], [], []
         act = (None, None, None, None)
@@ -776,10 +879,10 @@
                         invstd = torch.empty(cout, dtype=torch.float32, device=dev)
                         L.call('mvp_mlp_forward_rel_bn_f32', x, L.ptr(x), R, cin_f, cin_f, L.ptr(w), cin, cout, L.ptr(rel), L.ptr(wrel), L.ptr(y),
                                L.ptr(stat), L.ptr(_partial(R, cout, dev)), float(eps), float(mom), L.ptr(mean), L.ptr(invstd), L.ptr(rm), L.ptr(rv),
-                               L.ptr(nbt), prec=prec)
+                               L.ptr(nbt), prec=prec, img=_image(w0_param, 0, c1=cin_f))
                     else:
                         L.call('mvp_mlp_forward_rel_bn_f32', x, L.ptr(x), R, cin_f, cin_f, L.ptr(w), cin, cout, L.ptr(rel), L.ptr(wrel), L.ptr(y),
-                               None, None, 0.0, 0.0, None, None, None, None, None, prec=prec)
+                               None, None, 0.0, 0.0, None, None, None, None, None, prec=prec, img=_image(w0_param, 0, c1=cin_f))
                         mean, invstd = rm, eval_invstd.get(rv, eps)
                     ys.append(y)
                     means.append(mean)
@@ -816,7 +919,7 @@
                     invstd = torch.empty(cout, dtype=torch.float32, device=dev)
                     L.call('mvp_mlp_forward_bn_f32', x, L.ptr(x), R, cin, x.size(1), L.ptr(w), cin, cout, L.ptr(act[0]), L.ptr(act[1]),
                            L.ptr(act[2]), L.ptr(act[3]), L.ptr(y), L.ptr(stat), L.ptr(_partial(R, cout, dev)), float(eps), float(mom),
-                           L.ptr(mean), L.ptr(invstd), L.ptr(rm), L.ptr(rv), L.ptr(nbt), prec=prec)
+                           L.ptr(mean), L.ptr(invstd), L.ptr(rm), L.ptr(rv), L.ptr(nbt), prec=prec, img=_image(w, 0, R, cin, cout))
                     ys.append(y)
                     means.append(mean)
                     invstds.append(invstd)
@@ -824,7 +927,8 @@
                     x = y
                     continue
                 L.call('mvp_mlp_forward_f32', x, L.ptr(x), R, cin, x.size(1), L.ptr(w), cin, cout, L.ptr(act[0]), L.ptr(act[1]),
-                       L.ptr(act[2]), L.ptr(act[3]), None, L.ptr(y), L.ptr(stat), L.ptr(_partial(R, cout, dev) if training else None), prec=prec)
+                       L.ptr(act[2]), L.ptr(act[3]), None, L.ptr(y), L.ptr(stat), L.ptr(_partial(R, cout, dev) if training else None), prec=prec,
+                       img=_image(w, 0, R, cin, cout))
             rm, rv, nbt = bn_buffers[i]
             if training:
                 mean = torch.empty(cout, dtype=torch.float32, device=dev)
@@ -1041,7 +1145,8 @@
                         L.call('mvp_mlp_weight_grad_f32', gcur, *wg_args, prec=ctx.prec)
                 if need_dz:
                     wf = weight_slices.get(w0_param, 0, cin_f, cin_f)
-                    L.call('mvp_mlp_input_grad_f32', gcur, L.ptr(gcur), R, cout, L.ptr(wf), cin_f, None, None, None, None, None, L.ptr(dz), None, None, prec=ctx.prec)
+                    L.call('mvp_mlp_input_grad_f32', gcur, L.ptr(gcur), R, cout, L.ptr(wf), cin_f, None, None, None, None, None, L.ptr(dz), None, None, prec=ctx.prec,
+                           img=_image(w0_param, 1, c1=cin_f))
                     dx0 = dz
                 break
             if wide:
@@ -1082,9 +1187,10 @@
                 if need_dz and i > 0:
                     pm, pi, pg, pb = act
                     L.call('mvp_mlp_input_grad_f32', gcur, L.ptr(gcur), R, cout, L.ptr(w), cin, L.ptr(ys[i - 1]), L.ptr(pm), L.ptr(pi),
-                           L.ptr(pg), L.ptr(pb), L.ptr(dz), L.ptr(stat), L.ptr(_partial(R, cin, dev)), prec=ctx.prec)
+                           L.ptr(pg), L.ptr(pb), L.ptr(dz), L.ptr(stat), L.ptr(_partial(R, cin, dev)), prec=ctx.prec, img=_image(ctx.w_refs[i], 1))
                 elif need_dz:
-                    L.call('mvp_mlp_input_grad_f32', gcur, L.ptr(gcur), R, cout, L.ptr(w), cin, None, None, None, None, None, L.ptr(dz), None, None, prec=ctx.prec)
+                    L.call('mvp_mlp_input_grad_f32', gcur, L.ptr(gcur), R, cout, L.ptr(w), cin, None, None, None, None, None, L.ptr(dz), None, None, prec=ctx.prec,
+                           img=_image(ctx.w_refs[i], 1))
             if i > 0:
                 gcur, pending = dz, stat
             elif need_dz:
@@ -1137,7 +1243,10 @@
         L.require_gpu(x, w, bias)
         cout = w.size(0)
         y = torch.empty((R, cout), dtype=torch.float32, device=x.device)
-        L.call('mvp_mlp_forward_f32', x, L.ptr(x), R, ldx, ldx, L.ptr(w), ldx, cout, None, None, None, None, L.ptr(bias), L.ptr(y), None, None, prec=prec)
+        is_param = w2.is_cuda and w2.dtype == torch.float32
+        L.call('mvp_mlp_forward_f32', x, L.ptr(x), R, ldx, ldx, L.ptr(w), ldx, cout, None, None, None, None, L.ptr(bias), L.ptr(y), None, None, prec=prec,
+               img=_image(w_full if is_param else None, 0, R, ldx, cout, c0, c1, ldx))
+        ctx.w_ref = (w_full if is_param else None, c0, c1)
         ctx.save_for_backward(x, w)
         ctx.has_bias = bias is not None
         ctx.slice = (c0, cin, tuple(w_full.shape))
@@ -1153,6 +1262,7 @@
         cout = w.size(0)
         gy = gy.contiguous()
         gx = gw = gb = None
+        img = _image(ctx.w_ref[0], 1, c0=ctx.w_ref[1], c1=ctx.w_ref[2]) if (ctx.needs_input_grad[0] and cin == ctx.w_ref[2] - ctx.w_ref[1]) else None
         aside = False
         if ctx.needs_input_grad[0]:
             gx = torch.empty_like(x)
@@ -1163,13 +1273,13 @@
                 part = L.ptr(_partial(R, cin, gy.device) if R > 65536 else None)
                 if drop_p > 0:
                     L.call('mvp_mlp_input_grad_dropout_f32', gy, L.ptr(gy), R, cout, L.ptr(w), cin, L.ptr(yp), L.ptr(pm), L.ptr(pi), L.ptr(pg), L.ptr(pb),
-                           drop_p, drop_seed, L.ptr(gx), L.ptr(stat), part, prec=ctx.prec)
+                           drop_p, drop_seed, L.ptr(gx), L.ptr(stat), part, prec=ctx.prec, img=img)
                 else:
                     L.call('mvp_mlp_input_grad_f32', gy, L.ptr(gy), R, cout, L.ptr(w), cin, L.ptr(yp), L.ptr(pm), L.ptr(pi), L.ptr(pg), L.ptr(pb), L.ptr(gx),
-                           L.ptr(stat), part, prec=ctx.prec)
+                           L.ptr(stat), part, prec=ctx.prec, img=img)
                 src.stat = stat
             else:
-                L.call('mvp_mlp_input_grad_f32', gy, L.ptr(gy), R, cout, L.ptr(w), cin, None, None, None, None, None, L.ptr(gx), None, None, prec=ctx.prec)
+                L.call('mvp_mlp_input_grad_f32', gy, L.ptr(gy), R, cout, L.ptr(w), cin, None, None, None, None, None, L.ptr(gx), None, None, prec=ctx.prec, img=img)
         if ctx.needs_input_grad[1]:
             c0, ncol, shape = ctx.slice
             sink = ctx.sink
```

After: 5076 chunks/s, median of 6. Within noise of the previous version (+0.9%).
